# ChenFengYe/motion-latent-diffusion

Hardware: NVIDIA H100
Metric: motions/sec @ 50-step DDIM text-to-motion, batch 256 (higher is better)
Workload: dtype f16x2-split (fp32-equivalent, fp32 accumulate)

## Files before the change

### include/mldb.h

```cpp
#ifndef MLDB_H_
#define MLDB_H_

#include <stdint.h>

#ifdef __cplusplus
extern "C" {
#endif

#define MLDB_OK 0
#define MLDB_ERR_INVALID 1
#define MLDB_ERR_CUDA 2
#define MLDB_ERR_STATE 3
#define MLDB_ERR_UNSUPPORTED 4

#define MLDB_ABI_VERSION 4

typedef struct mldb_handle mldb_handle;

#define MLDB_COND_TEXT 0
#define MLDB_COND_ACTION 1
#define MLDB_ARCH_TRANS_ENC 0
#define MLDB_ARCH_TRANS_DEC 1
#define MLDB_VAE_NONE 0
#define MLDB_VAE_MLD 1
#define MLDB_VAE_ACTOR 2
#define MLDB_SCHED_DDIM 0
#define MLDB_SCHED_DDPM 1
#define MLDB_BETA_SCALED_LINEAR 0
#define MLDB_BETA_LINEAR 1
#define MLDB_BETA_SQUAREDCOS_CAP_V2 2
#define MLDB_DTYPE_F32 0

typedef struct mldb_config {
  int32_t abi_version;
  int32_t cond_kind;
  int32_t arch;
  int32_t latent_dim;
  int32_t n_lat;
  int32_t num_heads;
  int32_t ff_size;
  int32_t num_layers;
  int32_t text_dim;
  int32_t nclasses;
  int32_t nfeats;
  int32_t diffusion_only;
  int32_t flip_sin_to_cos;
  float   freq_shift;
  float   guidance_scale;
  int32_t vae_kind;
  int32_t vae_layers;
  int32_t vae_heads;
  int32_t vae_ff;
  int32_t vae_nfeats;
  int32_t sched_kind;
  int32_t num_train_timesteps;
  double  beta_start;
  double  beta_end;
  int32_t steps_offset;
  int32_t set_alpha_to_one;
  float   eta;
  int32_t njoints;
  int32_t beta_schedule;
  int32_t clip_sample;
} mldb_config;

void mldb_default_config(mldb_config* cfg);

int mldb_create(const mldb_config* cfg, int device, mldb_handle** out);
void mldb_destroy(mldb_handle* h);

int mldb_load_tensor(mldb_handle* h, const char* key, const void* data,
                     const int64_t* shape, int32_t ndim, int32_t dtype);

int mldb_finalize_weights(mldb_handle* h, void* stream);

int mldb_set_mean_std(mldb_handle* h, const float* mean, const float* std, int32_t nfeats);

int mldb_scheduler_table(const mldb_config* cfg, float* alphas_cumprod_out);
int mldb_scheduler_timesteps(const mldb_config* cfg, int32_t n, int64_t* out);

int mldb_scheduler_set_timesteps(mldb_handle* h, int32_t n, int64_t* timesteps_out);

int mldb_scheduler_step(mldb_handle* h, const float* model_output, int64_t timestep,
                        const float* sample, const float* noise, int64_t count,
                        float* prev_sample, void* stream);

int mldb_denoise(mldb_handle* h, const float* sample, int64_t timestep, const void* cond,
                 const int32_t* lengths, int32_t Bx, int32_t S_ctx, int32_t T,
                 float* out, void* stream);

int mldb_diffusion_reverse(mldb_handle* h, const void* cond, const float* init_noise,
                           const float* step_noise, const int32_t* lengths, int32_t B,
                           int32_t S_ctx, int32_t T, float* latents_out, void* stream);

int mldb_vae_decode(mldb_handle* h, const float* z, const int32_t* lengths, int32_t B,
                    int32_t T, float* feats_out, void* stream);

int mldb_vae_encode(mldb_handle* h, const float* feats, const int32_t* lengths, int32_t B,
                    int32_t T, float* mu, float* logvar, void* stream);

int mldb_feats2joints(mldb_handle* h, const float* feats, int32_t B, int32_t T,
                      float* joints_out, void* stream);

int mldb_sample(mldb_handle* h, const void* cond, const float* init_noise,
                const int32_t* lengths, int32_t B, int32_t S_ctx, int32_t T,
                float* latents_out, float* feats_out, float* joints_out, void* stream,
                const float* step_noise);

int mldb_sample_host(mldb_handle* h, const void* cond_host, const float* init_noise_host,
                     const int32_t* lengths_host, int32_t B, int32_t S_ctx, int32_t T,
                     float* joints_host, void* stream, const float* step_noise_host);

int mldb_comm_unique_id(void* out128 );
int mldb_comm_init(mldb_handle* h, const void* unique_id128, int32_t nranks, int32_t rank);
int mldb_comm_attach(mldb_handle* h, void* nccl_comm, int32_t nranks, int32_t rank);
int mldb_comm_info(const mldb_handle* h, int32_t* nranks, int32_t* rank);
int mldb_allgather(mldb_handle* h, const float* local, float* global, int64_t count, void* stream);
int mldb_sample_gather(mldb_handle* h, const void* cond, const float* init_noise, const int32_t* lengths,
                       int32_t B, int32_t S_ctx, int32_t T, float* joints_global, void* stream,
                       const float* step_noise);
int mldb_gather_wait(mldb_handle* h, void* stream);

int mldb_profile_op(mldb_handle* h, const char* op, int32_t B, int32_t S_ctx, int32_t iters,
                    float* avg_ms_out);

int mldb_profile_steps(mldb_handle* h, const void* cond, const float* init_noise, int32_t B, int32_t S_ctx,
                       float* ms_out);

int mldb_debug_timeline(int32_t enable, int64_t* out, int32_t cap, int32_t* count);

int mldb_debug_gemm(mldb_handle* h, const float* A, const float* W, const float* bias, const float* gamma,
                    const float* beta, const float* R, int32_t M, int32_t N, int32_t K, int32_t K1,
                    int32_t act, int32_t use_tc, int32_t split_out, float* out, void* stream);

int mldb_debug_ffn(mldb_handle* h, const float* X, const float* W1, const float* b1, const float* W2,
                   const float* b2, const float* gamma, const float* beta, int32_t M, int32_t d, int32_t ff,
                   int32_t mode, float* out, void* stream);

int mldb_debug_attention(mldb_handle* h, const float* Q, const float* KV, const int32_t* lengths, int32_t kv_prefix,
                         int32_t nseq, int32_t Lq, int32_t Lk, int32_t heads, int32_t hd, int32_t mode, float* out,
                         void* stream);

int mldb_debug_attention_causal(mldb_handle* h, const float* Q, const float* KV, const int32_t* lengths,
                                int32_t kv_prefix, int32_t nseq, int32_t Lq, int32_t Lk, int32_t heads, int32_t hd,
                                int32_t mode, float* out, void* stream);

#define MLDB_TEXT_ABI_VERSION 1
#define MLDB_TEXT_HIDDEN 0
#define MLDB_TEXT_POOLED 1
typedef struct mldb_text_config {
  int32_t abi_version;
  int32_t vocab_size;
  int32_t max_positions;
  int32_t hidden;
  int32_t heads;
  int32_t layers;
  int32_t ff;
  int32_t projection_dim;
  int32_t eos_token_id;
  float   ln_eps;
} mldb_text_config;
void mldb_default_text_config(mldb_text_config* cfg);
int mldb_text_configure(mldb_handle* h, const mldb_text_config* cfg);
int mldb_text_encode(mldb_handle* h, const int64_t* ids, int32_t n, int32_t L, int32_t mode, float* out, void* stream);

#define MLDB_T2M_ABI_VERSION 1
#define MLDB_T2M_TEXT 1
#define MLDB_T2M_MOVEMENT 2
#define MLDB_T2M_MOTION 4
typedef struct mldb_t2m_config {
  int32_t abi_version;
  int32_t parts;
  int32_t dim_word;
  int32_t dim_pos_ohot;
  int32_t dim_text_hidden;
  int32_t dim_coemb_hidden;
  int32_t dim_pose;
  int32_t dim_move_hidden;
  int32_t dim_move_latent;
  int32_t dim_motion_hidden;
  int32_t dim_motion_latent;
} mldb_t2m_config;
void mldb_default_t2m_config(mldb_t2m_config* cfg);
int mldb_t2m_configure(mldb_handle* h, const mldb_t2m_config* cfg);
int mldb_t2m_movement(mldb_handle* h, const float* x, int32_t ld, int32_t B, int32_t T, float* out, void* stream);
int mldb_t2m_motion(mldb_handle* h, const float* x, const int32_t* lengths, int32_t B, int32_t L, float* out,
                    void* stream);
int mldb_t2m_text(mldb_handle* h, const float* word_embs, const float* pos_ohot, const int32_t* lengths, int32_t B,
                  int32_t L, float* out, void* stream);

const char* mldb_last_error(void);
int mldb_abi_version(void);
int64_t mldb_launch_count(const mldb_handle* h);
#define MLDB_KSTAT_GEMM_TC 0
#define MLDB_KSTAT_GEMM_LN_TC 1
#define MLDB_KSTAT_FFN_TC 2
#define MLDB_KSTAT_ATTN_TC 3
#define MLDB_KSTAT_ATTN_MMA 4
#define MLDB_KSTAT_ATTN_SIMT 5
#define MLDB_KSTAT_GEMM_SIMT 6
#define MLDB_KSTAT_LN_SIMT 7
#define MLDB_KSTAT_LN_UNFUSED 8
#define MLDB_KSTAT_MISC 9
#define MLDB_KSTAT_TEXT_LN 10
#define MLDB_KSTAT_GRU_TC 11
#define MLDB_KSTAT_COUNT 12
int mldb_kernel_stats(const mldb_handle* h, int64_t* out, int32_t n);
int mldb_reset_kernel_stats(mldb_handle* h);

int mldb_set_option(mldb_handle* h, const char* name, const char* value);

#ifdef __cplusplus
}
#endif
#endif
```

### mld_b200/_lib.py

```python
from __future__ import annotations

import ctypes as C
import os

_HERE = os.path.dirname(os.path.abspath(__file__))
LIB_PATH = os.path.join(_HERE, "libmldb200.so")

MLDB_ABI_VERSION = 4
COND_TEXT, COND_ACTION = 0, 1
ARCH_TRANS_ENC, ARCH_TRANS_DEC = 0, 1
VAE_NONE, VAE_MLD, VAE_ACTOR = 0, 1, 2
SCHED_DDIM, SCHED_DDPM = 0, 1
BETA_SCHEDULES = {"scaled_linear": 0, "linear": 1, "squaredcos_cap_v2": 2}
DTYPE_F32 = 0
KSTAT_NAMES = ("gemm_tc", "gemm_ln_tc", "ffn_tc", "attn_tc", "attn_mma", "attn_simt", "gemm_simt", "ln_simt",
               "ln_unfused", "misc", "text_ln", "gru_tc")
MLDB_TEXT_ABI_VERSION = 1
TEXT_HIDDEN, TEXT_POOLED = 0, 1
MLDB_T2M_ABI_VERSION = 1
T2M_TEXT, T2M_MOVEMENT, T2M_MOTION = 1, 2, 4


class MldbConfig(C.Structure):
    _fields_ = [
        ("abi_version", C.c_int32),
        ("cond_kind", C.c_int32), ("arch", C.c_int32), ("latent_dim", C.c_int32),
        ("n_lat", C.c_int32), ("num_heads", C.c_int32), ("ff_size", C.c_int32),
        ("num_layers", C.c_int32), ("text_dim", C.c_int32), ("nclasses", C.c_int32),
        ("nfeats", C.c_int32), ("diffusion_only", C.c_int32), ("flip_sin_to_cos", C.c_int32),
        ("freq_shift", C.c_float), ("guidance_scale", C.c_float),
        ("vae_kind", C.c_int32), ("vae_layers", C.c_int32), ("vae_heads", C.c_int32),
        ("vae_ff", C.c_int32), ("vae_nfeats", C.c_int32),
        ("sched_kind", C.c_int32), ("num_train_timesteps", C.c_int32),
        ("beta_start", C.c_double), ("beta_end", C.c_double), ("steps_offset", C.c_int32),
        ("set_alpha_to_one", C.c_int32), ("eta", C.c_float), ("njoints", C.c_int32),
        ("beta_schedule", C.c_int32), ("clip_sample", C.c_int32),
    ]


class MldbTextConfig(C.Structure):
    _fields_ = [
        ("abi_version", C.c_int32), ("vocab_size", C.c_int32), ("max_positions", C.c_int32),
        ("hidden", C.c_int32), ("heads", C.c_int32), ("layers", C.c_int32), ("ff", C.c_int32),
        ("projection_dim", C.c_int32), ("eos_token_id", C.c_int32), ("ln_eps", C.c_float),
    ]


class MldbT2mConfig(C.Structure):
    _fields_ = [
        ("abi_version", C.c_int32), ("parts", C.c_int32), ("dim_word", C.c_int32), ("dim_pos_ohot", C.c_int32),
        ("dim_text_hidden", C.c_int32), ("dim_coemb_hidden", C.c_int32), ("dim_pose", C.c_int32),
        ("dim_move_hidden", C.c_int32), ("dim_move_latent", C.c_int32), ("dim_motion_hidden", C.c_int32),
        ("dim_motion_latent", C.c_int32),
    ]


_P = C.c_void_p
_SIGNATURES = {
    "mldb_default_config": (None, [C.POINTER(MldbConfig)]),
    "mldb_create": (C.c_int, [C.POINTER(MldbConfig), C.c_int, C.POINTER(_P)]),
    "mldb_destroy": (None, [_P]),
    "mldb_load_tensor": (C.c_int, [_P, C.c_char_p, _P, C.POINTER(C.c_int64), C.c_int32, C.c_int32]),
    "mldb_finalize_weights": (C.c_int, [_P, _P]),
    "mldb_set_mean_std": (C.c_int, [_P, _P, _P, C.c_int32]),
    "mldb_scheduler_table": (C.c_int, [C.POINTER(MldbConfig), _P]),
    "mldb_scheduler_timesteps": (C.c_int, [C.POINTER(MldbConfig), C.c_int32, _P]),
    "mldb_scheduler_set_timesteps": (C.c_int, [_P, C.c_int32, _P]),
    "mldb_scheduler_step": (C.c_int, [_P, _P, C.c_int64, _P, _P, C.c_int64, _P, _P]),
    "mldb_denoise": (C.c_int, [_P, _P, C.c_int64, _P, _P, C.c_int32, C.c_int32, C.c_int32, _P, _P]),
    "mldb_diffusion_reverse": (C.c_int, [_P, _P, _P, _P, _P, C.c_int32, C.c_int32, C.c_int32, _P, _P]),
    "mldb_vae_decode": (C.c_int, [_P, _P, _P, C.c_int32, C.c_int32, _P, _P]),
    "mldb_vae_encode": (C.c_int, [_P, _P, _P, C.c_int32, C.c_int32, _P, _P, _P]),
    "mldb_feats2joints": (C.c_int, [_P, _P, C.c_int32, C.c_int32, _P, _P]),
    "mldb_sample": (C.c_int, [_P, _P, _P, _P, C.c_int32, C.c_int32, C.c_int32, _P, _P, _P, _P, _P]),
    "mldb_sample_host": (C.c_int, [_P, _P, _P, _P, C.c_int32, C.c_int32, C.c_int32, _P, _P, _P]),
    "mldb_profile_op": (C.c_int, [_P, C.c_char_p, C.c_int32, C.c_int32, C.c_int32, C.POINTER(C.c_float)]),
    "mldb_profile_steps": (C.c_int, [_P, _P, _P, C.c_int32, C.c_int32, _P]),
    "mldb_debug_timeline": (C.c_int, [C.c_int32, _P, C.c_int32, C.POINTER(C.c_int32)]),
    "mldb_debug_gemm": (C.c_int, [_P, _P, _P, _P, _P, _P, _P, C.c_int32, C.c_int32, C.c_int32, C.c_int32,
                                  C.c_int32, C.c_int32, C.c_int32, _P, _P]),
    "mldb_debug_ffn": (C.c_int, [_P, _P, _P, _P, _P, _P, _P, _P, C.c_int32, C.c_int32, C.c_int32, C.c_int32, _P, _P]),
    "mldb_debug_attention": (C.c_int, [_P, _P, _P, _P, C.c_int32, C.c_int32, C.c_int32, C.c_int32, C.c_int32, C.c_int32,
                                       C.c_int32, _P, _P]),
    "mldb_debug_attention_causal": (C.c_int, [_P, _P, _P, _P, C.c_int32, C.c_int32, C.c_int32, C.c_int32, C.c_int32,
                                              C.c_int32, C.c_int32, _P, _P]),
    "mldb_default_text_config": (None, [C.POINTER(MldbTextConfig)]),
    "mldb_text_configure": (C.c_int, [_P, C.POINTER(MldbTextConfig)]),
    "mldb_text_encode": (C.c_int, [_P, _P, C.c_int32, C.c_int32, C.c_int32, _P, _P]),
    "mldb_default_t2m_config": (None, [C.POINTER(MldbT2mConfig)]),
    "mldb_t2m_configure": (C.c_int, [_P, C.POINTER(MldbT2mConfig)]),
    "mldb_t2m_movement": (C.c_int, [_P, _P, C.c_int32, C.c_int32, C.c_int32, _P, _P]),
    "mldb_t2m_motion": (C.c_int, [_P, _P, _P, C.c_int32, C.c_int32, _P, _P]),
    "mldb_t2m_text": (C.c_int, [_P, _P, _P, _P, C.c_int32, C.c_int32, _P, _P]),
    "mldb_comm_unique_id": (C.c_int, [_P]),
    "mldb_comm_init": (C.c_int, [_P, _P, C.c_int32, C.c_int32]),
    "mldb_comm_attach": (C.c_int, [_P, _P, C.c_int32, C.c_int32]),
    "mldb_comm_info": (C.c_int, [_P, C.POINTER(C.c_int32), C.POINTER(C.c_int32)]),
    "mldb_allgather": (C.c_int, [_P, _P, _P, C.c_int64, _P]),
    "mldb_sample_gather": (C.c_int, [_P, _P, _P, _P, C.c_int32, C.c_int32, C.c_int32, _P, _P, _P]),
    "mldb_gather_wait": (C.c_int, [_P, _P]),
    "mldb_kernel_stats": (C.c_int, [_P, _P, C.c_int32]),
    "mldb_reset_kernel_stats": (C.c_int, [_P]),
    "mldb_last_error": (C.c_char_p, []),
    "mldb_abi_version": (C.c_int, []),
    "mldb_launch_count": (C.c_int64, [_P]),
    "mldb_set_option": (C.c_int, [_P, C.c_char_p, C.c_char_p]),
}

_lib = None


def lib():
    global _lib
    if _lib is None:
        if not os.path.exists(LIB_PATH):
            raise ImportError(
                f"{LIB_PATH} is missing: build it with `python -c 'import __graft_entry__ as g; "
                "g.build()'` (nvcc, sm_90a). mld_b200 has no CPU or PyTorch fallback.")
        l = C.CDLL(LIB_PATH)
        for name, (res, args) in _SIGNATURES.items():
            fn = getattr(l, name)
            fn.restype = res
            fn.argtypes = args
        if l.mldb_abi_version() != MLDB_ABI_VERSION:
            raise ImportError("libmldb200.so ABI version mismatch; rebuild")
        _lib = l
    return _lib


def check(status: int, what: str = "mldb"):
    if status != 0:
        msg = lib().mldb_last_error()
        raise RuntimeError(f"{what} failed (status {status}): {msg.decode() if msg else '?'}")


def default_config() -> MldbConfig:
    cfg = MldbConfig()
    lib().mldb_default_config(C.byref(cfg))
    return cfg


def default_text_config() -> MldbTextConfig:
    cfg = MldbTextConfig()
    lib().mldb_default_text_config(C.byref(cfg))
    return cfg


def default_t2m_config() -> MldbT2mConfig:
    cfg = MldbT2mConfig()
    lib().mldb_default_t2m_config(C.byref(cfg))
    return cfg
```

### mld_b200/csrc/engine.cu

```cuda
#include "engine.h"

#include <math.h>
#include <stdio.h>
#include <string.h>

#include <algorithm>

#include "gemm_tc.h"

static thread_local std::string g_err;
void mldb_set_err(const std::string& s) { g_err = s; }
extern "C" const char* mldb_last_error(void) { return g_err.c_str(); }
extern "C" int mldb_abi_version(void) { return MLDB_ABI_VERSION; }

#define CK(call)                                                                      \
  do {                                                                                \
    cudaError_t e__ = (call);                                                         \
    if (e__ != cudaSuccess) {                                                         \
      char buf__[512];                                                                \
      snprintf(buf__, sizeof buf__, "%s:%d: %s failed: %s", __FILE__, __LINE__, #call, \
               cudaGetErrorString(e__));                                              \
      mldb_set_err(buf__);                                                            \
      return MLDB_ERR_CUDA;                                                           \
    }                                                                                 \
// ... 242 lines not shown
  for (int i = 0; i < nb; ++i) {
    s->skip.emplace_back();
    const std::string lp = p + "linear_blocks." + std::to_string(i) + ".";
    TRY(pack_named(h, lp + "weight", lp + "bias", &s->skip.back()));
  }
  TRY(pack_ln(h, p + "norm.", d, &s->norm));
  return MLDB_OK;
}
static int upload_pe(mldb_handle* h, const std::string& key, float** out, int* rows = nullptr) {
  const RawTensor& t = rt(h, key);
  if (rows) *rows = (int)t.shape[0];
  return upload_f32(h, t.host.data(), t.host.size(), out);
}
static int pack_actor_encoder(mldb_handle* h) {
  const mldb_config& c = h->cfg;
  const int d = c.latent_dim;
  const std::string E = "vae.encoder.";
  StackW* s = &h->venc;
  s->kind = STACK_PLAIN_ENC; s->d = d; s->ff = c.vae_ff; s->heads = c.vae_heads; s->layers = c.vae_layers;
  for (int i = 0; i < c.vae_layers; ++i) {
    const std::string n = E + "seqTransEncoder.layers." + std::to_string(i) + ".";
    s->enc.emplace_back();
    TRY(pack_enc_layer(h, n, d, &s->enc.back()));
    if (i == c.vae_layers - 1) TRY(pack_trimmed_qkv(h, n, d, &s->enc.back()));
  }
  std::vector<float> tok(rt(h, E + "mu_token").host);
  const std::vector<float>& lv = rt(h, E + "logvar_token").host;
  tok.insert(tok.end(), lv.begin(), lv.end());
  TRY(upload_f32(h, tok.data(), tok.size(), &h->global_token));
  TRY(pack_named(h, E + "skel_embedding.weight", E + "skel_embedding.bias", &h->skel_emb, 0, -1, true));
  return upload_pe(h, E + "sequence_pos_encoding.pe", &h->vae_enc_pe, &h->vae_enc_pe_rows);
}

static int check_sched_cfg(const mldb_config& c) {
  if (c.sched_kind != MLDB_SCHED_DDIM && c.sched_kind != MLDB_SCHED_DDPM) FAIL(MLDB_ERR_INVALID, "unknown sched_kind %d", c.sched_kind);
  if (c.beta_schedule != MLDB_BETA_SCALED_LINEAR && c.beta_schedule != MLDB_BETA_LINEAR &&
      c.beta_schedule != MLDB_BETA_SQUAREDCOS_CAP_V2)
    FAIL(MLDB_ERR_INVALID, "unknown beta_schedule %d", c.beta_schedule);
  if (!(c.eta >= 0.0f && c.eta <= 1.0f)) FAIL(MLDB_ERR_INVALID, "eta must lie in [0, 1], got %g", (double)c.eta);
  if (c.num_train_timesteps < 2) FAIL(MLDB_ERR_INVALID, "num_train_timesteps must be >= 2");
  return MLDB_OK;
}

static void build_alphas(const mldb_config& c, std::vector<float>* out) {
  const int T = c.num_train_timesteps;
  out->resize(T);
  const bool scaled = c.beta_schedule == MLDB_BETA_SCALED_LINEAR;
  const float s0 = scaled ? (float)sqrt(c.beta_start) : (float)c.beta_start;
  const float s1 = scaled ? (float)sqrt(c.beta_end) : (float)c.beta_end;
  const float step = (s1 - s0) / (float)(T - 1);
  auto alpha_bar = [](double t) { return pow(cos((t + 0.008) / 1.008 * M_PI / 2), 2.0); };
  double prod = 1.0;
  for (int i = 0; i < T; ++i) {
    float beta;
    if (c.beta_schedule == MLDB_BETA_SQUAREDCOS_CAP_V2) {
      const double t1 = (double)i / T, t2 = (double)(i + 1) / T;
      beta = (float)std::min(1.0 - alpha_bar(t2) / alpha_bar(t1), 0.999);
    } else {
      const float v = (i < T / 2) ? fmaf(step, (float)i, s0) : fmaf(-step, (float)(T - 1 - i), s1);
      beta = scaled ? v * v : v;
    }
    const float alpha = 1.0f - beta;
    prod *= (double)alpha;
    (*out)[i] = (float)prod;
  }
}
extern "C" int mldb_scheduler_table(const mldb_config* cfg, float* alphas_cumprod_out) {
  if (!cfg || !alphas_cumprod_out) FAIL(MLDB_ERR_INVALID, "null argument");
  TRY(check_sched_cfg(*cfg));
  std::vector<float> a;
  build_alphas(*cfg, &a);
  memcpy(alphas_cumprod_out, a.data(), a.size() * sizeof(float));
  return MLDB_OK;
}
extern "C" int mldb_scheduler_timesteps(const mldb_config* cfg, int32_t n, int64_t* out) {
  if (!cfg || !out || n <= 0 || n > cfg->num_train_timesteps) FAIL(MLDB_ERR_INVALID, "bad n");
  const int64_t ratio = cfg->num_train_timesteps / n;
  const int64_t off = cfg->sched_kind == MLDB_SCHED_DDIM ? cfg->steps_offset : 0;
  for (int i = 0; i < n; ++i) out[i] = (int64_t)(n - 1 - i) * ratio + off;
  return MLDB_OK;
}
static StepCoef make_coef(const mldb_handle* h, int64_t t, int n_inference) {
  const mldb_config& c = h->cfg;
  const std::vector<float>& ac = h->alphas_cumprod;
  StepCoef k{};
  const int64_t prev_t = t - c.num_train_timesteps / n_inference;
  const float a_t = ac[t];
  k.c0 = sqrtf(a_t);
  k.c1 = sqrtf(1.0f - a_t);
  k.clip = c.clip_sample ? 1 : 0;
  if (c.sched_kind == MLDB_SCHED_DDIM) {
    const float a_prev = prev_t >= 0 ? ac[prev_t] : (c.set_alpha_to_one ? 1.0f : ac[0]);
    const float variance = ((1.0f - a_prev) / (1.0f - a_t)) * (1.0f - a_t / a_prev);
    const float std_dev = c.eta * sqrtf(variance);
    k.kind = 0;
    k.c2 = sqrtf(a_prev);
    k.c3 = sqrtf(1.0f - a_prev - std_dev * std_dev);
    k.sigma = std_dev;
  } else {
    const float a_prev = prev_t >= 0 ? ac[prev_t] : 1.0f;
    const float bpt = 1.0f - a_t, bpp = 1.0f - a_prev;
    const float cur_alpha = a_t / a_prev, cur_beta = 1.0f - cur_alpha;
    k.kind = 1;
    k.c2 = (sqrtf(a_prev) * cur_beta) / bpt;
    k.c3 = sqrtf(cur_alpha) * bpp / bpt;
    k.sigma = t > 0 ? sqrtf(std::max(bpp / bpt * cur_beta, 1e-20f)) : 0.0f;
  }
  return k;
}

static inline unsigned nblk(int64_t n, int t = 256) { return (unsigned)((n + t - 1) / t); }

static inline ActBuf rows_of(ActBuf b, int64_t row0, int rows) {
  b.hi += row0 * b.cols; b.rows = rows; return b;
}
static inline void kcount(mldb_handle* h, int kind) { h->kstat[kind]++; count_launch(h); }
static void op_gemm(mldb_handle* h, const GemmArgs& g, cudaStream_t st) {
  if (h->use_tc && tc_gemm_supported(h->tc, g)) {
    if (!tc_gemm(h->tc, g, nullptr, st)) h->op_failed = true;
    kcount(h, MLDB_KSTAT_GEMM_TC);
    return;
  }
  simt_gemm(g, st);
  kcount(h, MLDB_KSTAT_GEMM_SIMT);
}
static void op_gemm_ln(mldb_handle* h, GemmArgs g, LnArgs l, float* cf32, cudaStream_t st) {
  if (h->use_tc && tc_gemm_ln_supported(h->tc, g, l)) {
    if (!tc_gemm(h->tc, g, &l, st)) h->op_failed = true;
    kcount(h, MLDB_KSTAT_GEMM_LN_TC);
    return;
  }
  g.out = ActBuf{}; g.out_f32 = cf32; g.ldc = g.w.N;
  op_gemm(h, g, st);
  l.c = cf32; l.ldc = g.w.N;
  simt_ln(l, st);
  kcount(h, h->use_tc ? MLDB_KSTAT_LN_UNFUSED : MLDB_KSTAT_LN_SIMT);
}
static void op_ln(mldb_handle* h, const LnArgs& l, cudaStream_t st) { simt_ln(l, st); kcount(h, MLDB_KSTAT_LN_SIMT); }
static void op_attn(mldb_handle* h, const AttnArgs& a, cudaStream_t st) {
  if (h->use_tc && h->attn_kind == 0 && tc_attention_supported(a)) {
    if (!tc_attention(a, st)) h->op_failed = true;
    kcount(h, MLDB_KSTAT_ATTN_TC);
  } else if (h->use_tc && h->attn_kind <= 1 && mma_attention_supported(a)) {
    mma_attention(a, st);
    kcount(h, MLDB_KSTAT_ATTN_MMA);
  } else {
    if (!simt_attention(a, st)) {
      mldb_set_err("CUDA-core attention: head_dim " + std::to_string(a.hd) + " does not fit shared memory");
      h->op_failed = true;
    }
    kcount(h, MLDB_KSTAT_ATTN_SIMT);
  }
}
static void op_ffn(mldb_handle* h, const GemmArgs& g1, const GemmArgs& g2, const LnArgs& l2, float* cf32, cudaStream_t st) {
  if (h->use_tc && tc_ffn_supported(h->tc, g1, g2, l2)) {
    int k = 0;
    for (int i = 0; i < mldb_handle::MAX_BRANCHES - 1; ++i) if (st == h->br_stream[i]) k = i + 1;
    if (!tc_ffn(h->tc, g1, g2, l2, h->ffn_scratch[k], h->ffn_flags[k], st)) h->op_failed = true;
    kcount(h, MLDB_KSTAT_FFN_TC);
    return;
  }
  op_gemm(h, g1, st);
  op_gemm_ln(h, g2, l2, cf32, st);
}

static int alloc_act(mldb_handle* h, int rows, int cols, ActBuf* out) {
  const int64_t rp = ((int64_t)rows + 127) / 128 * 128;
  __half* p = nullptr;
  TRY(dev_alloc(h, (void**)&p, (size_t)2 * rp * cols * sizeof(__half)));
  CK(cudaMemset(p, 0, (size_t)2 * rp * cols * sizeof(__half)));
  out->hi = p; out->plane_stride = rp * cols; out->rows = rows; out->cols = cols;
  return MLDB_OK;
}
static int alloc_stack_ws(mldb_handle* h, const StackW& sw, int nseq, int L, int Lmem, StackWs* ws,
                          int n_sel = 0) {
  ws->nseq = nseq; ws->L = L; ws->M = nseq * L; ws->d = sw.d; ws->ff = sw.ff; ws->Lmem = Lmem;
  const int M = ws->M, d = sw.d;
  TRY(alloc_act(h, M, d, &ws->x0));
  TRY(alloc_act(h, M, d, &ws->cur[0]));
  TRY(alloc_act(h, M, d, &ws->cur[1]));
  TRY(alloc_act(h, M, d, &ws->x1));
  TRY(alloc_act(h, M, d, &ws->att));
  TRY(alloc_act(h, M, 3 * d, &ws->qkv));
  TRY(alloc_act(h, M, sw.ff, &ws->h));
  const bool enc = sw.kind == STACK_SKIP_ENC || sw.kind == STACK_PLAIN_ENC;
  if (!enc) {
    TRY(alloc_act(h, M, d, &ws->x2));
    TRY(alloc_act(h, M, d, &ws->qc));
    TRY(alloc_act(h, nseq * Lmem, 2 * d, &ws->kvm));
    TRY(alloc_act(h, nseq, d, &ws->vrow));
    TRY(dev_alloc(h, (void**)&ws->cvec, (size_t)nseq * d * sizeof(float)));
  }
  if (sw.kind == STACK_SKIP_ENC || sw.kind == STACK_SKIP_DEC) {
    TRY(alloc_act(h, M, d, &ws->cat));
    const int nb = (sw.layers - 1) / 2;
    ws->ys.resize(nb);
    for (int i = 0; i < nb; ++i) TRY(alloc_act(h, M, d, &ws->ys[i]));
  }
  TRY(dev_alloc(h, (void**)&ws->cf32, (size_t)M * d * sizeof(float)));
  if (enc && n_sel > 0) {
    ws->n_sel = n_sel;
    const int R = nseq * n_sel;
    TRY(alloc_act(h, R, d, &ws->sx));
    TRY(alloc_act(h, R, d, &ws->sq));
    TRY(alloc_act(h, R, d, &ws->satt));
    TRY(alloc_act(h, R, d, &ws->sx1));
    TRY(alloc_act(h, R, sw.ff, &ws->sh));
    TRY(alloc_act(h, R, d, &ws->sout));
  }
  return MLDB_OK;
}

struct SeqInfo {
  const int32_t* lengths = nullptr;
  int kv_prefix = 0;
  int len_mod = 0;
};

static StackWs ws_slice(const StackWs& ws, int s0, int n) {
  StackWs w = ws;
  w.nseq = n; w.M = n * ws.L;
  auto tok = [&](ActBuf b) { return b.hi ? rows_of(b, (int64_t)s0 * ws.L, n * ws.L) : b; };
  auto sel = [&](ActBuf b) { return b.hi ? rows_of(b, (int64_t)s0 * ws.n_sel, n * ws.n_sel) : b; };
  w.x0 = tok(ws.x0); w.cur[0] = tok(ws.cur[0]); w.cur[1] = tok(ws.cur[1]); w.x1 = tok(ws.x1); w.x2 = tok(ws.x2);
  w.att = tok(ws.att); w.qkv = tok(ws.qkv); w.qc = tok(ws.qc); w.h = tok(ws.h); w.cat = tok(ws.cat);
  for (auto& y : w.ys) y = tok(y);
  if (ws.kvm.hi) w.kvm = rows_of(ws.kvm, (int64_t)s0 * ws.Lmem, n * ws.Lmem);
  if (ws.vrow.hi) w.vrow = rows_of(ws.vrow, s0, n);
  if (ws.cvec) w.cvec = ws.cvec + (size_t)s0 * ws.d;
  if (ws.cf32) w.cf32 = ws.cf32 + (size_t)s0 * ws.L * ws.d;
  w.sx = sel(ws.sx); w.sq = sel(ws.sq); w.satt = sel(ws.satt); w.sx1 = sel(ws.sx1); w.sh = sel(ws.sh); w.sout = sel(ws.sout);
  return w;
}
static void out_proj_ln(mldb_handle* h, const LinW& w, const LnW& n, ActBuf att, ActBuf res, ActBuf xout, int M, int d,
                        float* cf32, cudaStream_t st) {
  GemmArgs g; g.a1 = att; g.K1 = d; g.M = M; g.w = w;
  LnArgs l; l.res = res; l.gamma = n.g; l.beta = n.b; l.M = M; l.d = d; l.out = xout;
  op_gemm_ln(h, g, l, cf32, st);
}
static void self_attn_block(mldb_handle* h, const LinW& in_proj, const LinW& out_proj, const LnW& n,
                            ActBuf xin, ActBuf xout, StackWs& ws, const SeqInfo& si, int heads,
                            cudaStream_t st) {
  const int d = ws.d;
  GemmArgs g; g.a1 = xin; g.K1 = d; g.M = ws.M; g.w = in_proj; g.out = ws.qkv;
  op_gemm(h, g, st);
  AttnArgs a; a.q = ws.qkv; a.q_col0 = 0; a.Lq = ws.L; a.kv = ws.qkv; a.k_col0 = d; a.v_col0 = 2 * d;
  a.Lk = ws.L; a.nseq = ws.nseq; a.heads = heads; a.hd = d / heads;
  a.lengths = si.lengths; a.kv_prefix = si.kv_prefix; a.len_mod = si.len_mod; a.seq0 = 0; a.out = ws.att;
  op_attn(h, a, st);
  out_proj_ln(h, out_proj, n, ws.att, xin, xout, ws.M, d, ws.cf32, st);
}
static void ffn_block(mldb_handle* h, const LinW& l1, const LinW& l2, const LnW& n, ActBuf xin,
                      ActBuf xout, StackWs& ws, int act, cudaStream_t st) {
  GemmArgs g; g.a1 = xin; g.K1 = ws.d; g.M = ws.M; g.w = l1; g.act = act; g.out = ws.h;
  GemmArgs g2; g2.a1 = ws.h; g2.K1 = ws.ff; g2.M = ws.M; g2.w = l2;
  LnArgs l; l.res = xin; l.gamma = n.g; l.beta = n.b; l.M = ws.M; l.d = ws.d; l.out = xout;
  op_ffn(h, g, g2, l, ws.cf32, st);
}
static void enc_layer(mldb_handle* h, const StackW& sw, const EncW& w, ActBuf xin, ActBuf xout,
                      StackWs& ws, const SeqInfo& si, cudaStream_t st) {
  self_attn_block(h, w.in_proj, w.out_proj, w.n1, xin, ws.x1, ws, si, sw.heads, st);
  ffn_block(h, w.l1, w.l2, w.n2, ws.x1, xout, ws, ACT_GELU, st);
}
static void dec_layer(mldb_handle* h, const StackW& sw, const DecW& w, ActBuf xin, ActBuf xout,
                      ActBuf mem, StackWs& ws, const SeqInfo& si, cudaStream_t st) {
  const int d = ws.d;
  self_attn_block(h, w.sa_in, w.sa_out, w.n1, xin, ws.x1, ws, si, sw.heads, st);
  if (ws.Lmem == 1) {
    GemmArgs gv; gv.a1 = mem; gv.K1 = d; gv.M = ws.nseq; gv.w = w.ca_v; gv.out = ws.vrow;
    op_gemm(h, gv, st);
    GemmArgs gc; gc.a1 = ws.vrow; gc.K1 = d; gc.M = ws.nseq; gc.w = w.ca_out; gc.out_f32 = ws.cvec; gc.ldc = d;
    op_gemm(h, gc, st);
    LnArgs lc; lc.res = ws.x1; lc.rowvec = ws.cvec; lc.rv_group = ws.L; lc.gamma = w.n2.g; lc.beta = w.n2.b;
    lc.M = ws.M; lc.d = d; lc.out = ws.x2;
    op_ln(h, lc, st);
    ffn_block(h, w.l1, w.l2, w.n3, ws.x2, xout, ws, ACT_GELU, st);
    return;
  }
  GemmArgs gq; gq.a1 = ws.x1; gq.K1 = d; gq.M = ws.M; gq.w = w.ca_q; gq.out = ws.qc;
  op_gemm(h, gq, st);
  GemmArgs gk; gk.a1 = mem; gk.K1 = d; gk.M = ws.nseq * ws.Lmem; gk.w = w.ca_kv; gk.out = ws.kvm;
  op_gemm(h, gk, st);
  AttnArgs a; a.q = ws.qc; a.q_col0 = 0; a.Lq = ws.L; a.kv = ws.kvm; a.k_col0 = 0; a.v_col0 = d;
  a.Lk = ws.Lmem; a.nseq = ws.nseq; a.heads = sw.heads; a.hd = d / sw.heads; a.out = ws.att;
  op_attn(h, a, st);
  out_proj_ln(h, w.ca_out, w.n2, ws.att, ws.x1, ws.x2, ws.M, d, ws.cf32, st);
  ffn_block(h, w.l1, w.l2, w.n3, ws.x2, xout, ws, ACT_GELU, st);
}
static void any_layer(mldb_handle* h, const StackW& sw, int li, ActBuf xin, ActBuf xout, ActBuf mem,
                      StackWs& ws, const SeqInfo& si, cudaStream_t st) {
  if (sw.kind == STACK_SKIP_ENC) enc_layer(h, sw, sw.enc[li], xin, xout, ws, si, st);
  else dec_layer(h, sw, sw.dec[li], xin, xout, mem, ws, si, st);
}
__global__ void k_gather_rows(ActBuf src, ActBuf dst, int L, int n_sel, int nrows_out, int d) {
  pdl_trigger();
  pdl_wait();
  const int64_t idx = (int64_t)blockIdx.x * blockDim.x + threadIdx.x;
  if (idx >= (int64_t)nrows_out * (d / 8)) return;
  const int c = (int)(idx % (d / 8));
  const int r = (int)(idx / (d / 8));
  const int64_t srow = (int64_t)(r / n_sel) * L + r % n_sel;
  const uint4* sh = reinterpret_cast<const uint4*>(src.hi + srow * src.cols) + c;
  const uint4* sl = reinterpret_cast<const uint4*>(src.lo() + srow * src.cols) + c;
  reinterpret_cast<uint4*>(dst.hi + (int64_t)r * dst.cols)[c] = *sh;
  reinterpret_cast<uint4*>(dst.lo() + (int64_t)r * dst.cols)[c] = *sl;
}

static ActBuf enc_layer_selected(mldb_handle* h, const StackW& sw, const EncW& w, ActBuf xin, StackWs& ws,
                                 const SeqInfo& si, cudaStream_t st) {
  const int d = ws.d, R = ws.nseq * ws.n_sel;
  GemmArgs gk; gk.a1 = xin; gk.K1 = d; gk.M = ws.M; gk.w = w.kv_only; gk.out = ws.qkv;
  op_gemm(h, gk, st);
  launch_pdl(k_gather_rows, dim3(nblk((int64_t)R * (d / 8))), dim3(256), 0, st, xin, ws.sx, ws.L, ws.n_sel, R, d);
  kcount(h, MLDB_KSTAT_MISC);
  GemmArgs gq; gq.a1 = ws.sx; gq.K1 = d; gq.M = R; gq.w = w.q_only; gq.out = ws.sq;
  op_gemm(h, gq, st);
  AttnArgs a; a.q = ws.sq; a.q_col0 = 0; a.Lq = ws.n_sel; a.kv = ws.qkv; a.k_col0 = 0; a.v_col0 = d;
  a.Lk = ws.L; a.nseq = ws.nseq; a.heads = sw.heads; a.hd = d / sw.heads; a.lengths = si.lengths;
  a.kv_prefix = si.kv_prefix; a.len_mod = si.len_mod; a.out = ws.satt;
  op_attn(h, a, st);
  out_proj_ln(h, w.out_proj, w.n1, ws.satt, ws.sx, ws.sx1, R, d, ws.cf32, st);
  GemmArgs g1; g1.a1 = ws.sx1; g1.K1 = d; g1.M = R; g1.w = w.l1; g1.act = ACT_GELU; g1.out = ws.sh;
  GemmArgs g2; g2.a1 = ws.sh; g2.K1 = ws.ff; g2.M = R; g2.w = w.l2;
  LnArgs l2; l2.res = ws.sx1; l2.gamma = w.n2.g; l2.beta = w.n2.b; l2.M = R; l2.d = d; l2.out = ws.sout;
  op_ffn(h, g1, g2, l2, ws.cf32, st);
  return ws.sout;
}

static ActBuf run_stack(mldb_handle* h, const StackW& sw, ActBuf x0, ActBuf mem, StackWs& ws,
                        const SeqInfo& si, cudaStream_t st) {
  if (sw.kind == STACK_PLAIN_ENC) {
    ActBuf x = x0;
    for (int i = 0; i + 1 < sw.layers; ++i) {
      enc_layer(h, sw, sw.enc[i], x, ws.cur[i & 1], ws, si, st);
      x = ws.cur[i & 1];
    }
    return enc_layer_selected(h, sw, sw.enc.back(), x, ws, si, st);
  }
  if (sw.kind == STACK_PLAIN_DEC) {
    ActBuf x = x0;
    for (int i = 0; i < sw.layers; ++i) {
      any_layer(h, sw, i, x, ws.cur[i & 1], mem, ws, si, st);
      x = ws.cur[i & 1];
    }
    return x;
  }
  const int nb = (sw.layers - 1) / 2;
  ActBuf x = x0;
  for (int i = 0; i < nb; ++i) {
    any_layer(h, sw, i, x, ws.ys[i], mem, ws, si, st);
    x = ws.ys[i];
  }
  any_layer(h, sw, nb, x, ws.cur[0], mem, ws, si, st);
  x = ws.cur[0];
  for (int i = 0; i < nb; ++i) {
    GemmArgs g; g.a1 = x; g.K1 = sw.d; g.a2 = ws.ys[nb - 1 - i]; g.K2 = sw.d; g.M = ws.M;
    g.w = sw.skip[i]; g.out = ws.cat;
    op_gemm(h, g, st);
    if (i == nb - 1 && sw.kind == STACK_SKIP_ENC && ws.n_sel > 0)
      return enc_layer_selected(h, sw, sw.enc[nb + 1 + i], ws.cat, ws, si, st);
    any_layer(h, sw, nb + 1 + i, ws.cat, ws.cur[(i + 1) & 1], mem, ws, si, st);
    x = ws.cur[(i + 1) & 1];
  }
  return x;
}

extern "C" int mldb_create(const mldb_config* cfg, int device, mldb_handle** out) {
  if (!cfg || !out) FAIL(MLDB_ERR_INVALID, "null argument");
  if (cfg->abi_version != MLDB_ABI_VERSION) FAIL(MLDB_ERR_INVALID, "abi_version mismatch");
  if (cfg->latent_dim % cfg->num_heads || cfg->latent_dim % 32) FAIL(MLDB_ERR_INVALID, "latent_dim must be a multiple of 32 and of num_heads");
  if (cfg->latent_dim > 1024) FAIL(MLDB_ERR_UNSUPPORTED, "latent_dim > 1024");
  for (int heads : {cfg->num_heads, cfg->vae_heads})
    if (heads > 0 && !simt_attention_supported(cfg->latent_dim / heads))
      FAIL(MLDB_ERR_UNSUPPORTED, "head_dim %d is too wide for the attention kernels", cfg->latent_dim / heads);
  if (cfg->arch == MLDB_ARCH_TRANS_ENC && cfg->num_layers > 0 && cfg->num_layers % 2 != 1) FAIL(MLDB_ERR_INVALID, "skip encoder needs an odd layer count");
  if (cfg->arch == MLDB_ARCH_TRANS_ENC && cfg->diffusion_only) FAIL(MLDB_ERR_UNSUPPORTED, "diffusion_only requires arch trans_dec");
  if (cfg->vae_kind == MLDB_VAE_MLD && cfg->vae_layers % 2 != 1) FAIL(MLDB_ERR_INVALID, "MldVae needs an odd layer count");
  TRY(check_sched_cfg(*cfg));
  int ndev = 0;
  CK(cudaGetDeviceCount(&ndev));
  if (device < 0 || device >= ndev) FAIL(MLDB_ERR_INVALID, "no such CUDA device %d (no CPU fallback exists)", device);
  cudaDeviceProp prop;
  CK(cudaGetDeviceProperties(&prop, device));
  if (prop.major != 9) FAIL(MLDB_ERR_UNSUPPORTED, "device %d is sm_%d%d; libmldb200 is sm_90a only", device, prop.major, prop.minor);
  DeviceGuard guard(device);
  mldb_handle* h = new mldb_handle();
  h->cfg = *cfg; h->device = device; h->sm_count = prop.multiProcessorCount;
  build_spec(h);
  build_alphas(h->cfg, &h->alphas_cumprod);
  cudaError_t e = cudaStreamCreateWithFlags(&h->cap_stream, cudaStreamNonBlocking);
  if (e != cudaSuccess) { delete h; FAIL(MLDB_ERR_CUDA, "cudaStreamCreate: %s", cudaGetErrorString(e)); }
  if (!simt_init() || !mma_attention_init()) { delete h; return MLDB_ERR_CUDA; }
  h->tc = tc_create(device);
  if (!h->tc) { delete h; return MLDB_ERR_CUDA; }
  if (!tc_attention_init(device) || !gru_tc_init()) { tc_destroy(h->tc); delete h; return MLDB_ERR_CUDA; }
  const char* env = getenv("MLDB_GEMM");
  if (env && !strcmp(env, "simt")) h->use_tc = false;
  env = getenv("MLDB_GRAPH");
  if (env && !strcmp(env, "0")) h->use_graph = false;
  env = getenv("MLDB_ATTN");
  if (env) h->attn_kind = !strcmp(env, "mma") ? 1 : (!strcmp(env, "simt") ? 2 : 0);
  env = getenv("MLDB_BRANCHES");
  if (env) h->branches = std::min(std::max(atoi(env), 1), (int)mldb_handle::MAX_BRANCHES);
  e = cudaEventCreateWithFlags(&h->ev_fork, cudaEventDisableTiming);
  for (int i = 0; i < mldb_handle::MAX_BRANCHES - 1 && e == cudaSuccess; ++i) {
    e = cudaStreamCreateWithFlags(&h->br_stream[i], cudaStreamNonBlocking);
    if (e == cudaSuccess) e = cudaEventCreateWithFlags(&h->ev_join[i], cudaEventDisableTiming);
  }
  if (e != cudaSuccess) { mldb_destroy(h); FAIL(MLDB_ERR_CUDA, "branch streams: %s", cudaGetErrorString(e)); }
  for (int i = 0; i < mldb_handle::MAX_BRANCHES && e == cudaSuccess; ++i) {
    e = cudaMalloc((void**)&h->ffn_scratch[i], TC_FFN_SCRATCH_BYTES);
    if (e == cudaSuccess) e = cudaMalloc((void**)&h->ffn_flags[i], TC_FFN_FLAG_BYTES);
    if (e == cudaSuccess) e = cudaMemset(h->ffn_flags[i], 0, TC_FFN_FLAG_BYTES);
  }
  if (e != cudaSuccess) { mldb_destroy(h); FAIL(MLDB_ERR_CUDA, "ffn scratch: %s", cudaGetErrorString(e)); }
  env = getenv("MLDB_FFN_SPLIT");
  if (env) tc_set_ffn_split(h->tc, atoi(env) != 0);
  env = getenv("MLDB_FFN_FUSED");
  if (env) tc_set_ffn_fused(h->tc, atoi(env) != 0);
  *out = h;
  return MLDB_OK;
}

extern "C" void mldb_destroy(mldb_handle* h) {
  if (!h) return;
  DeviceGuard guard(h->device);
  cudaDeviceSynchronize();
  for (auto& kv : h->plans) {
    if (kv.second->exec) cudaGraphExecDestroy(kv.second->exec);
    delete kv.second;
  }
  for (void* p : h->allocs) cudaFree(p);
  for (void* p : h->text.ws_allocs) cudaFree(p);
  for (void* p : h->t2m.buf) cudaFree(p);
  if (h->cap_stream) cudaStreamDestroy(h->cap_stream);
  for (int i = 0; i < mldb_handle::MAX_BRANCHES - 1; ++i) {
    if (h->br_stream[i]) cudaStreamDestroy(h->br_stream[i]);
    if (h->ev_join[i]) cudaEventDestroy(h->ev_join[i]);
  }
  if (h->ev_fork) cudaEventDestroy(h->ev_fork);
  for (int i = 0; i < mldb_handle::MAX_BRANCHES; ++i) { cudaFree(h->ffn_scratch[i]); cudaFree(h->ffn_flags[i]); }
  mldb_comm_release(h);
  tc_destroy(h->tc);
  delete h;
}

extern "C" int mldb_set_option(mldb_handle* h, const char* name, const char* value) {
  if (!h || !name || !value) FAIL(MLDB_ERR_INVALID, "null argument");
  if (!strcmp(name, "gemm")) {
    if (!strcmp(value, "tc")) h->use_tc = true;
    else if (!strcmp(value, "simt")) h->use_tc = false;
    else FAIL(MLDB_ERR_INVALID, "gemm must be tc|simt");
  } else if (!strcmp(name, "ffn_fused")) {
    tc_set_ffn_fused(h->tc, atoi(value) != 0);
  } else if (!strcmp(name, "ffn_split")) {
    tc_set_ffn_split(h->tc, atoi(value) != 0);
  } else if (!strcmp(name, "attn")) {
    if (!strcmp(value, "tc")) h->attn_kind = 0;
    else if (!strcmp(value, "mma")) h->attn_kind = 1;
    else if (!strcmp(value, "simt")) h->attn_kind = 2;
    else FAIL(MLDB_ERR_INVALID, "attn must be tc|mma|simt");
  } else if (!strcmp(name, "branches")) {
    h->branches = std::min(std::max(atoi(value), 1), (int)mldb_handle::MAX_BRANCHES);
  } else if (!strcmp(name, "graph")) {
    h->use_graph = strcmp(value, "0") != 0;
  } else if (!strcmp(name, "t2m_chunk")) {
    h->t2m.chunk = std::max(atoi(value), 0);
  } else {
    FAIL(MLDB_ERR_INVALID, "unknown option %s", name);
  }
  for (auto& kv : h->plans) {
    if (kv.second->exec) { cudaGraphExecDestroy(kv.second->exec); kv.second->exec = nullptr; }
  }
  return MLDB_OK;
}

extern "C" int64_t mldb_launch_count(const mldb_handle* h) { return h ? h->launches : 0; }

// ... 911 lines not shown
    return check_ops(h);
  }
  LnArgs l; l.res = x; l.gamma = h->venc.norm.g; l.beta = h->venc.norm.b; l.M = B * G; l.d = d;
  if (p->ws.n_sel == 0) { l.sel_group = G; l.in_group = L; }
  l.out_f32 = p->stage_f32; l.ld_out = d;
  op_ln(h, l, st);
  k_rows_out_permuted<<<nblk((int64_t)B * G * d), 256, 0, st>>>(p->stage_f32, mu, logvar, B, c.n_lat, d);
  kcount(h, MLDB_KSTAT_MISC);
  CK(cudaGetLastError());
  return MLDB_OK;
}

static int run_f2j(mldb_handle* h, const float* feats, int B, int T, float* joints, cudaStream_t st) {
  const mldb_config& c = h->cfg;
  const int F = c.vae_kind != MLDB_VAE_NONE ? c.vae_nfeats : c.nfeats;
  if (!h->mean || h->nstat != F) FAIL(MLDB_ERR_STATE, "call mldb_set_mean_std with %d features first", F);
  if (F < 4 + (c.njoints - 1) * 3) FAIL(MLDB_ERR_UNSUPPORTED, "feats2joints needs the HumanML3D/KIT layout");
  k_feats2joints<<<B, 256, 0, st>>>(feats, h->mean, h->stdv, T, F, c.njoints, joints);
  kcount(h, MLDB_KSTAT_MISC);
  CK(cudaGetLastError());
  return MLDB_OK;
}
extern "C" int mldb_feats2joints(mldb_handle* h, const float* feats, int32_t B, int32_t T,
                                 float* joints_out, void* stream) {
  TRY(check_ready(h, false));
  DeviceGuard guard(h->device);
  if (!feats || !joints_out || B <= 0 || T <= 0) FAIL(MLDB_ERR_INVALID, "bad argument");
  return run_f2j(h, feats, B, T, joints_out, (cudaStream_t)stream);
}

extern "C" int mldb_sample(mldb_handle* h, const void* cond, const float* init_noise,
                           const int32_t* lengths, int32_t B, int32_t S_ctx, int32_t T,
                           float* latents_out, float* feats_out, float* joints_out, void* stream,
                           const float* step_noise) {
  TRY(check_ready(h, true));
  DeviceGuard guard(h->device);
  if (!cond || !init_noise || !lengths || B <= 0 || T <= 0) FAIL(MLDB_ERR_INVALID, "bad argument");
  cudaStream_t st = (cudaStream_t)stream;
  Plan *rp = nullptr, *dp = nullptr;
  TRY(dec_plan(h, B, T, &dp));
  const mldb_config& c = h->cfg;
  float* z = latents_out;
  if (!z) {
    if (!dp->stage_f32) TRY(dev_alloc(h, (void**)&dp->stage_f32, (size_t)B * c.n_lat * c.latent_dim * sizeof(float)));
    z = dp->stage_f32;
  }
  if (c.arch != MLDB_ARCH_TRANS_ENC) FAIL(MLDB_ERR_UNSUPPORTED, "mldb_sample is built for the latent (VAE) models");
  TRY(run_reverse(h, cond, init_noise, step_noise, lengths, B, S_ctx, T, z, st, &rp));
  TRY(run_decode(h, z, lengths, B, T, feats_out, st, &dp));
  if (joints_out) TRY(run_f2j(h, feats_out ? feats_out : dp->feats, B, T, joints_out, st));
  return MLDB_OK;
}

extern "C" int mldb_sample_gather(mldb_handle* h, const void* cond, const float* init_noise,
                                  const int32_t* lengths, int32_t B, int32_t S_ctx, int32_t T,
                                  float* joints_global, void* stream, const float* step_noise) {
  TRY(check_ready(h, true));
  DeviceGuard guard(h->device);
  if (!joints_global) FAIL(MLDB_ERR_INVALID, "bad argument");
  const int64_t count = (int64_t)B * T * h->cfg.njoints * 3;
  cudaStream_t st = (cudaStream_t)stream;
  if (!h->nccl_comm) {
    return mldb_sample(h, cond, init_noise, lengths, B, S_ctx, T, nullptr, nullptr, joints_global, stream, step_noise);
  }
  TRY(mldb_gather_begin(h, st));
  TRY(mldb_sample(h, cond, init_noise, lengths, B, S_ctx, T, nullptr, nullptr, joints_global + h->comm_rank * count, stream,
                  step_noise));
  return mldb_gather_async(h, joints_global, count, st);
}

extern "C" int mldb_sample_host(mldb_handle* h, const void* cond_host, const float* init_noise_host,
                                const int32_t* lengths_host, int32_t B, int32_t S_ctx, int32_t T,
                                float* joints_host, void* stream, const float* step_noise_host) {
  TRY(check_ready(h, true));
  DeviceGuard guard(h->device);
  if (!cond_host || !init_noise_host || !lengths_host || !joints_host || B <= 0 || T <= 0) FAIL(MLDB_ERR_INVALID, "bad argument");
  cudaStream_t st = (cudaStream_t)stream;
  const mldb_config& c = h->cfg;
  Plan* dp = nullptr;
  TRY(dec_plan(h, B, T, &dp));
  const bool cfg_on = c.guidance_scale > 1.0f;
  const int Bx = cfg_on ? 2 * B : B;
  const size_t cond_bytes = c.cond_kind == MLDB_COND_TEXT ? (size_t)Bx * S_ctx * c.text_dim * sizeof(float)
                                                         : (size_t)Bx * sizeof(int64_t);
  const size_t noise_bytes = (size_t)B * c.n_lat * c.latent_dim * sizeof(float);
  if (dp->cond_cap < cond_bytes) {
    TRY(dev_alloc(h, (void**)&dp->cond_f, cond_bytes));
    dp->cond_cap = cond_bytes;
  }
  if (!dp->noise_in) {
    TRY(dev_alloc(h, (void**)&dp->noise_in, noise_bytes));
    TRY(dev_alloc(h, (void**)&dp->cond_i, (size_t)B * sizeof(int32_t)));
  }
  const int world = h->nccl_comm ? h->comm_world : 1;
  const size_t joints_elems = (size_t)B * T * c.njoints * 3;
  if (world > 1 && !dp->joints_all) TRY(dev_alloc(h, (void**)&dp->joints_all, world * joints_elems * sizeof(float)));
  CK(cudaMemcpyAsync(dp->cond_f, cond_host, cond_bytes, cudaMemcpyHostToDevice, st));
  CK(cudaMemcpyAsync(dp->noise_in, init_noise_host, noise_bytes, cudaMemcpyHostToDevice, st));
  CK(cudaMemcpyAsync(dp->cond_i, lengths_host, (size_t)B * sizeof(int32_t), cudaMemcpyHostToDevice, st));
  const float* step_noise = nullptr;
  if (step_noise_host) {
    const size_t n = h->timesteps.size() * (size_t)B * c.n_lat * c.latent_dim;
    if (dp->noise_cap < n) {
      TRY(dev_alloc(h, (void**)&dp->step_noise, n * sizeof(float)));
      dp->noise_cap = n;
    }
    CK(cudaMemcpyAsync(dp->step_noise, step_noise_host, n * sizeof(float), cudaMemcpyHostToDevice, st));
    step_noise = dp->step_noise;
  }
  if (world > 1) {
    TRY(mldb_sample_gather(h, dp->cond_f, dp->noise_in, (const int32_t*)dp->cond_i, B, S_ctx, T, dp->joints_all, stream,
                           step_noise));
    TRY(mldb_gather_wait(h, stream));
    CK(cudaMemcpyAsync(joints_host, dp->joints_all, world * joints_elems * sizeof(float), cudaMemcpyDeviceToHost, st));
    return MLDB_OK;
  }
  TRY(mldb_sample(h, dp->cond_f, dp->noise_in, (const int32_t*)dp->cond_i, B, S_ctx, T, nullptr, nullptr, dp->joints, stream,
                  step_noise));
  CK(cudaMemcpyAsync(joints_host, dp->joints, joints_elems * sizeof(float), cudaMemcpyDeviceToHost, st));
  return MLDB_OK;
}

extern "C" int mldb_profile_op(mldb_handle* h, const char* op, int32_t B, int32_t S_ctx, int32_t iters,
                               float* avg_ms_out) {
  TRY(check_ready(h, false));
  DeviceGuard guard(h->device);
  if (!op || !avg_ms_out || iters <= 0) FAIL(MLDB_ERR_INVALID, "bad argument");
  const mldb_config& c = h->cfg;
  if (c.num_layers == 0 || c.arch != MLDB_ARCH_TRANS_ENC) FAIL(MLDB_ERR_UNSUPPORTED, "needs the trans_enc denoiser");
  const bool cfg_on = c.guidance_scale > 1.0f;
  Plan* p = nullptr;
  TRY(enc_plan(h, 0, B, cfg_on ? 2 * B : B, S_ctx, &p));
  cudaStream_t st = h->cap_stream;
  StackWs& ws = p->ws;
  const EncW& w = h->den.enc[0];
  const int d = ws.d;
  SeqInfo si;
  auto run = [&]() -> int {
    if (!strcmp(op, "qkv")) {
      GemmArgs g; g.a1 = ws.x0; g.K1 = d; g.M = ws.M; g.w = w.in_proj; g.out = ws.qkv; op_gemm(h, g, st);
    } else if (!strcmp(op, "attn")) {
      AttnArgs a; a.q = ws.qkv; a.Lq = ws.L; a.kv = ws.qkv; a.k_col0 = d; a.v_col0 = 2 * d; a.Lk = ws.L;
      a.nseq = ws.nseq; a.heads = c.num_heads; a.hd = d / c.num_heads; a.out = ws.att; op_attn(h, a, st);
    } else if (!strcmp(op, "outproj_ln")) {
      out_proj_ln(h, w.out_proj, w.n1, ws.att, ws.x0, ws.x1, ws.M, d, ws.cf32, st);
    } else if (!strcmp(op, "ffn1")) {
      GemmArgs g; g.a1 = ws.x1; g.K1 = d; g.M = ws.M; g.w = w.l1; g.act = ACT_GELU; g.out = ws.h; op_gemm(h, g, st);
    } else if (!strcmp(op, "ffn2_ln")) {
      GemmArgs g; g.a1 = ws.h; g.K1 = ws.ff; g.M = ws.M; g.w = w.l2;
      LnArgs l; l.res = ws.x1; l.gamma = w.n2.g; l.beta = w.n2.b; l.M = ws.M; l.d = d; l.out = ws.cur[0];
      op_gemm_ln(h, g, l, ws.cf32, st);
    } else if (!strcmp(op, "ffn")) {
      ffn_block(h, w.l1, w.l2, w.n2, ws.x1, ws.cur[0], ws, ACT_GELU, st);
    } else if (!strcmp(op, "layer")) {
      enc_layer(h, h->den, w, ws.x0, ws.cur[0], ws, si, st);
    } else {
      FAIL(MLDB_ERR_INVALID, "unknown op %s", op);
    }
    return MLDB_OK;
  };
  cudaEvent_t e0, e1;
  CK(cudaEventCreate(&e0)); CK(cudaEventCreate(&e1));
  for (int i = 0; i < 3; ++i) TRY(run());
  CK(cudaEventRecord(e0, st));
  for (int i = 0; i < iters; ++i) TRY(run());
  CK(cudaEventRecord(e1, st));
  CK(cudaStreamSynchronize(st));
  float ms = 0.0f;
  CK(cudaEventElapsedTime(&ms, e0, e1));
  cudaEventDestroy(e0); cudaEventDestroy(e1);
  CK(cudaGetLastError());
  *avg_ms_out = ms / (float)iters;
  return MLDB_OK;
}

extern "C" int mldb_profile_steps(mldb_handle* h, const void* cond, const float* init_noise, int32_t B, int32_t S_ctx,
                                  float* ms_out) {
  TRY(check_ready(h, true));
  DeviceGuard guard(h->device);
  if (!cond || !init_noise || !ms_out || B <= 0) FAIL(MLDB_ERR_INVALID, "bad argument");
  const mldb_config& c = h->cfg;
  if (c.num_layers == 0 || c.arch != MLDB_ARCH_TRANS_ENC) FAIL(MLDB_ERR_UNSUPPORTED, "needs the trans_enc denoiser");
  if (c.sched_kind != MLDB_SCHED_DDIM) FAIL(MLDB_ERR_UNSUPPORTED, "step profiling is built for the DDIM loop");
  const bool cfg_on = c.guidance_scale > 1.0f;
  Plan* p = nullptr;
  TRY(enc_plan(h, 0, B, cfg_on ? 2 * B : B, S_ctx, &p));
  cudaStream_t st = h->cap_stream;
  const int d = c.latent_dim, nsteps = (int)h->timesteps.size();
  const int64_t per = (int64_t)c.n_lat * d;
  TRY(place_condition(h, p, cond, st));
  CK(cudaMemcpyAsync(p->latents, init_noise, (size_t)B * per * sizeof(float), cudaMemcpyDeviceToDevice, st));
  std::vector<cudaEvent_t> ev(nsteps + 1);
  for (auto& e : ev) CK(cudaEventCreate(&e));
  CK(cudaEventRecord(ev[0], st));
  for (int i = 0; i < nsteps; ++i) {
    denoiser_pass(h, p, p->latents, B, h->d_tt + (size_t)i * d, p->eps, st);
    launch_pdl(k_cfg_sched, dim3(nblk(B * per)), dim3(256), 0, st, (const float*)p->eps, p->latents, (const float*)nullptr,
               (int64_t)(B * per), cfg_on ? 1 : 0, c.guidance_scale, (const StepCoef*)h->d_coefs, i, (const int*)nullptr);
    kcount(h, MLDB_KSTAT_MISC);
    CK(cudaEventRecord(ev[i + 1], st));
  }
  CK(cudaStreamSynchronize(st));
  for (int i = 0; i < nsteps; ++i) CK(cudaEventElapsedTime(&ms_out[i], ev[i], ev[i + 1]));
  for (auto& e : ev) cudaEventDestroy(e);
  CK(cudaGetLastError());
  return check_ops(h);
}


static void op_text_ln(mldb_handle* h, const TextLnArgs& a, cudaStream_t st) { text_ln(a, st); kcount(h, MLDB_KSTAT_TEXT_LN); }

static int text_workspace(mldb_handle* h, int rows, int seqs) {
  TextW& tw = h->text;
  if (rows <= tw.rows && seqs <= tw.seqs) return MLDB_OK;
  rows = std::max(rows, tw.rows); seqs = std::max(seqs, tw.seqs);
  CK(cudaDeviceSynchronize());
  for (void* p : tw.ws_allocs) cudaFree(p);
  tw.ws_allocs.clear();
  tw.rows = tw.seqs = 0;
  auto alloc = [&](size_t bytes, void** p) -> int {
    CK(cudaMalloc(p, bytes ? bytes : 16));
    tw.ws_allocs.push_back(*p);
    CK(cudaMemset(*p, 0, bytes));
    return MLDB_OK;
  };
  auto act = [&](int r, int cols, ActBuf* out) -> int {
    const int64_t rp = ((int64_t)r + 127) / 128 * 128;
    TRY(alloc((size_t)2 * rp * cols * sizeof(__half), (void**)&out->hi));
    out->plane_stride = rp * cols; out->rows = r; out->cols = cols;
    return MLDB_OK;
  };
  const mldb_text_config& c = tw.cfg;
  TRY(alloc((size_t)rows * c.hidden * sizeof(float), (void**)&tw.x));
  TRY(act(rows, c.hidden, &tw.a));
  TRY(act(rows, 3 * c.hidden, &tw.qkv));
  TRY(act(rows, c.hidden, &tw.att));
  TRY(act(rows, c.ff, &tw.h));
  TRY(act(seqs, c.hidden, &tw.pooled));
  tw.rows = rows; tw.seqs = seqs;
  return MLDB_OK;
}

extern "C" int mldb_text_encode(mldb_handle* h, const int64_t* ids, int32_t n, int32_t L, int32_t mode, float* out,
                                void* stream) {
  if (!h || !ids || !out) FAIL(MLDB_ERR_INVALID, "null argument");
  TextW& tw = h->text;
  if (!tw.on) FAIL(MLDB_ERR_STATE, "the text tower is not configured (mldb_text_configure)");
  if (!h->finalized) FAIL(MLDB_ERR_STATE, "finalize weights first");
  const mldb_text_config& c = tw.cfg;
  if (n < 1 || L < 1 || L > c.max_positions) FAIL(MLDB_ERR_INVALID, "ids must be [n >= 1, 1 <= L <= %d]", c.max_positions);
  if ((int64_t)n * L > (1 << 30)) FAIL(MLDB_ERR_INVALID, "too many tokens");
  if (mode != MLDB_TEXT_HIDDEN && mode != MLDB_TEXT_POOLED) FAIL(MLDB_ERR_INVALID, "mode must be MLDB_TEXT_HIDDEN or MLDB_TEXT_POOLED");
  DeviceGuard guard(h->device);
  cudaStream_t st = (cudaStream_t)stream;
  const int M = n * L, d = c.hidden;
  TRY(text_workspace(h, M, n));
  auto rows = [&](ActBuf b, int r) { b.rows = r; return b; };
  const ActBuf a = rows(tw.a, M), qkv = rows(tw.qkv, M), att = rows(tw.att, M), hid = rows(tw.h, M);
  auto ln = [&](int m, const LnW& w) {
    TextLnArgs l; l.mode = m; l.x = tw.x; l.ids = ids; l.L = L; l.tok = tw.tok; l.pos = tw.pos; l.vocab = c.vocab_size;
    l.eos_id = c.eos_token_id; l.gamma = w.g; l.beta = w.b; l.eps = c.ln_eps; l.M = M; l.d = d; l.out = a;
    return l;
  };
  op_text_ln(h, ln(TEXT_LN_EMBED, tw.layers[0].ln1), st);
  for (int i = 0; i < c.layers; ++i) {
    const TextLayerW& w = tw.layers[i];
    GemmArgs g; g.a1 = a; g.K1 = d; g.M = M; g.w = w.qkv; g.out = qkv; g.wide_n = 1;
    op_gemm(h, g, st);
    AttnArgs at; at.q = qkv; at.q_col0 = 0; at.Lq = L; at.kv = qkv; at.k_col0 = d; at.v_col0 = 2 * d; at.Lk = L;
    at.nseq = n; at.heads = c.heads; at.hd = d / c.heads; at.causal = 1; at.out = att;
    op_attn(h, at, st);
    GemmArgs go; go.a1 = att; go.K1 = d; go.M = M; go.w = w.out; go.out_f32 = tw.x; go.ldc = d; go.res_f32 = tw.x;
    op_gemm(h, go, st);
    op_text_ln(h, ln(TEXT_LN_ROWS, w.ln2), st);
    GemmArgs g1; g1.a1 = a; g1.K1 = d; g1.M = M; g1.w = w.fc1; g1.act = ACT_QUICKGELU; g1.out = hid; g1.wide_n = 1;
    op_gemm(h, g1, st);
    GemmArgs g2; g2.a1 = hid; g2.K1 = c.ff; g2.M = M; g2.w = w.fc2; g2.out_f32 = tw.x; g2.ldc = d; g2.res_f32 = tw.x;
    op_gemm(h, g2, st);
    if (i + 1 < c.layers) op_text_ln(h, ln(TEXT_LN_ROWS, tw.layers[i + 1].ln1), st);
  }
  if (mode == MLDB_TEXT_HIDDEN) {
    TextLnArgs l = ln(TEXT_LN_ROWS, tw.final_ln);
    l.out = ActBuf{}; l.out_f32 = out;
    op_text_ln(h, l, st);
  } else {
    TextLnArgs l = ln(TEXT_LN_EOS, tw.final_ln);
    l.M = n; l.out = rows(tw.pooled, n);
    op_text_ln(h, l, st);
    GemmArgs gp; gp.a1 = l.out; gp.K1 = d; gp.M = n; gp.w = tw.proj; gp.out_f32 = out; gp.ldc = c.projection_dim;
    gp.wide_n = 1;
    op_gemm(h, gp, st);
  }
  CK(cudaGetLastError());
  return check_ops(h);
}

static int t2m_slot(mldb_handle* h, int i, size_t bytes, void** out) {
  T2mW& t = h->t2m;
  if (bytes > t.cap[i]) {
    CK(cudaDeviceSynchronize());
    cudaFree(t.buf[i]);
    t.buf[i] = nullptr; t.cap[i] = 0;
    CK(cudaMalloc(&t.buf[i], bytes));
    CK(cudaMemset(t.buf[i], 0, bytes));
    t.cap[i] = bytes;
  }
// ... 124 lines not shown
}

extern "C" int mldb_t2m_motion(mldb_handle* h, const float* x, const int32_t* lengths, int32_t B, int32_t L, float* out,
                               void* stream) {
  if (!h || !x || !lengths || !out) FAIL(MLDB_ERR_INVALID, "null argument");
  TRY(t2m_ready(h, MLDB_T2M_MOTION, "motion"));
  const mldb_t2m_config& c = h->t2m.cfg;
  if (B < 1 || L < 1 || (int64_t)B * L > (1 << 26)) FAIL(MLDB_ERR_INVALID, "motion encoder input must be [B >= 1, L >= 1, %d], got B=%d L=%d", c.dim_move_latent, B, L);
  DeviceGuard guard(h->device);
  cudaStream_t st = (cudaStream_t)stream;
  const int In = c.dim_move_latent, H = c.dim_motion_hidden;
  const int Bc = t2m_chunk(h, B, gru_bytes_per_seq(L, In + H, H));
  for (int b0 = 0; b0 < B; b0 += Bc) {
    const int n = std::min(Bc, B - b0);
    ActBuf xs, e;
    TRY(t2m_act(h, 0, n * L, In, &xs));
    TRY(t2m_act(h, 2, n * L, H, &e));
    k_f32_to_split_pad<<<nblk((int64_t)n * L * In), 256, 0, st>>>(xs, x + (int64_t)b0 * L * In, In, n * L, In, 1);
    kcount(h, MLDB_KSTAT_MISC);
    GemmArgs g; g.a1 = xs; g.K1 = In; g.M = n * L; g.w = h->t2m.motion_in; g.out = e; g.wide_n = 1;
    op_gemm(h, g, st);
    TRY(gru_forward(h, h->t2m.motion_gru, e, lengths + b0, n, L, out + (int64_t)b0 * c.dim_motion_latent,
                    c.dim_motion_latent, st));
  }
  CK(cudaGetLastError());
  return check_ops(h);
}

extern "C" int mldb_t2m_text(mldb_handle* h, const float* word_embs, const float* pos_ohot, const int32_t* lengths,
                             int32_t B, int32_t L, float* out, void* stream) {
  if (!h || !word_embs || !pos_ohot || !lengths || !out) FAIL(MLDB_ERR_INVALID, "null argument");
  TRY(t2m_ready(h, MLDB_T2M_TEXT, "text"));
  const mldb_t2m_config& c = h->t2m.cfg;
  if (B < 1 || L < 1 || (int64_t)B * L > (1 << 26)) FAIL(MLDB_ERR_INVALID, "text encoder input must be [B >= 1, L >= 1, *], got B=%d L=%d", B, L);
  DeviceGuard guard(h->device);
  cudaStream_t st = (cudaStream_t)stream;
  const int W = c.dim_word, P = c.dim_pos_ohot, H = c.dim_text_hidden;
  const int Bc = t2m_chunk(h, B, gru_bytes_per_seq(L, pad64(P) + 2 * W + pad64(W) + H, H));
  for (int b0 = 0; b0 < B; b0 += Bc) {
    const int n = std::min(Bc, B - b0), M = n * L;
    ActBuf ps, xs, e;
    float* xw = nullptr;
    TRY(t2m_act(h, 0, M, pad64(P), &ps));
    TRY(t2m_slot(h, 7, (size_t)M * W * sizeof(float), (void**)&xw));
    TRY(t2m_act(h, 8, M, pad64(W), &xs));
    TRY(t2m_act(h, 2, M, H, &e));
    k_f32_to_split_pad<<<nblk((int64_t)M * ps.cols), 256, 0, st>>>(ps, pos_ohot + (int64_t)b0 * L * P, P, M, P, 1);
    kcount(h, MLDB_KSTAT_MISC);
    GemmArgs gp; gp.a1 = ps; gp.K1 = ps.cols; gp.M = M; gp.w = h->t2m.pos_emb; gp.out_f32 = xw; gp.ldc = W;
    gp.res_f32 = word_embs + (int64_t)b0 * L * W; gp.wide_n = 1;
    op_gemm(h, gp, st);
    k_f32_to_split_pad<<<nblk((int64_t)M * xs.cols), 256, 0, st>>>(xs, xw, W, M, W, 1);
    kcount(h, MLDB_KSTAT_MISC);
    GemmArgs g; g.a1 = xs; g.K1 = xs.cols; g.M = M; g.w = h->t2m.text_in; g.out = e; g.wide_n = 1;
    op_gemm(h, g, st);
    TRY(gru_forward(h, h->t2m.text_gru, e, lengths + b0, n, L, out + (int64_t)b0 * c.dim_coemb_hidden,
                    c.dim_coemb_hidden, st));
  }
  CK(cudaGetLastError());
  return check_ops(h);
}

extern "C" int mldb_debug_gemm(mldb_handle* h, const float* A, const float* W, const float* bias,
                               const float* gamma, const float* beta, const float* R, int32_t M, int32_t N,
                               int32_t K, int32_t K1, int32_t act, int32_t use_tc, int32_t split_out, float* out,
                               void* stream) {
  if (!h || !A || !W || !out || M <= 0 || N <= 0 || K <= 0) FAIL(MLDB_ERR_INVALID, "bad argument");
  DeviceGuard guard(h->device);
  cudaStream_t st = (cudaStream_t)stream;
  const size_t n_alloc0 = h->allocs.size();
  LinW w;
  TRY(pack_linear(h, W, N, K, bias, &w));
  if (K1 <= 0 || K1 >= K) K1 = K;
  ActBuf a1, a2{}, res{}, o{};
  TRY(alloc_act(h, M, K1, &a1));
  k_rows_to_split<<<nblk((int64_t)M * K1), 256, 0, st>>>(a1, A, K, M, K1, 1 << 30, 0, 0, 0, nullptr);
  if (K1 < K) {
    TRY(alloc_act(h, M, K - K1, &a2));
    k_rows_to_split<<<nblk((int64_t)M * (K - K1)), 256, 0, st>>>(a2, A + K1, K, M, K - K1, 1 << 30, 0, 0, 0, nullptr);
  }
  float *g = nullptr, *b = nullptr, *cf32 = nullptr;
  const bool saved = h->use_tc;
  h->use_tc = use_tc != 0;
  GemmArgs ga; ga.a1 = a1; ga.K1 = K1; ga.a2 = a2; ga.K2 = K - K1; ga.M = M; ga.w = w; ga.act = act; ga.wide_n = 1;
  int rc = MLDB_OK;
  if (gamma) {
    TRY(upload_f32(h, gamma, N, &g));
    TRY(upload_f32(h, beta, N, &b));
    TRY(dev_alloc(h, (void**)&cf32, (size_t)M * N * sizeof(float)));
    TRY(alloc_act(h, M, N, &o));
    if (R) {
      TRY(alloc_act(h, M, N, &res));
      k_rows_to_split<<<nblk((int64_t)M * N), 256, 0, st>>>(res, R, N, M, N, 1 << 30, 0, 0, 0, nullptr);
    }
    LnArgs l; l.res = res; l.gamma = g; l.beta = b; l.M = M; l.d = N; l.out = o;
    op_gemm_ln(h, ga, l, cf32, st);
    k_split_to_f32<<<nblk((int64_t)M * N), 256, 0, st>>>(o, out, (int64_t)M * N);
  } else if (R) {
    ga.res_f32 = R; ga.out_f32 = out; ga.ldc = N;
    op_gemm(h, ga, st);
  } else if (split_out && N % 8 == 0) {
    TRY(alloc_act(h, M, N, &o));
    ga.out = o;
    op_gemm(h, ga, st);
    k_split_to_f32<<<nblk((int64_t)M * N), 256, 0, st>>>(o, out, (int64_t)M * N);
  } else {
    ga.out_f32 = out; ga.ldc = N;
    op_gemm(h, ga, st);
  }
  h->use_tc = saved;
  cudaError_t e = cudaStreamSynchronize(st);
  if (e == cudaSuccess) e = cudaGetLastError();
  while (h->allocs.size() > n_alloc0) { cudaFree(h->allocs.back()); h->allocs.pop_back(); }
  if (e != cudaSuccess) FAIL(MLDB_ERR_CUDA, "debug gemm: %s", cudaGetErrorString(e));
  return rc;
}

extern "C" int mldb_debug_ffn(mldb_handle* h, const float* X, const float* W1, const float* b1, const float* W2,
                              const float* b2, const float* gamma, const float* beta, int32_t M, int32_t d,
                              int32_t ff, int32_t mode, float* out, void* stream) {
  if (!h || !X || !W1 || !W2 || !gamma || !beta || !out || M <= 0 || d <= 0 || ff <= 0)
    FAIL(MLDB_ERR_INVALID, "bad argument");
  DeviceGuard guard(h->device);
  cudaStream_t st = (cudaStream_t)stream;
  const size_t n_alloc0 = h->allocs.size();
  LinW l1, l2;
  LnW n;
  TRY(pack_linear(h, W1, ff, d, b1, &l1));
  TRY(pack_linear(h, W2, d, ff, b2, &l2));
  TRY(upload_f32(h, gamma, d, &n.g));
  TRY(upload_f32(h, beta, d, &n.b));
  StackWs ws;
  ws.M = M; ws.d = d; ws.ff = ff;
  ActBuf x, o;
  TRY(alloc_act(h, M, d, &x));
  TRY(alloc_act(h, M, d, &o));
  TRY(alloc_act(h, M, ff, &ws.h));
  TRY(dev_alloc(h, (void**)&ws.cf32, (size_t)M * d * sizeof(float)));
  k_rows_to_split<<<nblk((int64_t)M * d), 256, 0, st>>>(x, X, d, M, d, 1 << 30, 0, 0, 0, nullptr);
  const bool saved = h->use_tc;
  h->use_tc = mode != 0;
  const int saved_fused = tc_set_ffn_fused(h->tc, mode == 2);
  ffn_block(h, l1, l2, n, x, o, ws, ACT_GELU, st);
  h->use_tc = saved;
  tc_set_ffn_fused(h->tc, saved_fused);
  k_split_to_f32<<<nblk((int64_t)M * d), 256, 0, st>>>(o, out, (int64_t)M * d);
  cudaError_t e = cudaStreamSynchronize(st);
  if (e == cudaSuccess) e = cudaGetLastError();
  while (h->allocs.size() > n_alloc0) { cudaFree(h->allocs.back()); h->allocs.pop_back(); }
  if (e != cudaSuccess) FAIL(MLDB_ERR_CUDA, "debug ffn: %s", cudaGetErrorString(e));
  return MLDB_OK;
}

static int debug_attention(mldb_handle* h, const float* Q, const float* KV, const int32_t* lengths, int32_t kv_prefix,
                           int32_t nseq, int32_t Lq, int32_t Lk, int32_t heads, int32_t hd, int32_t mode, int causal,
                           float* out, void* stream) {
  if (!h || !Q || !out || nseq <= 0 || Lq <= 0 || Lk <= 0 || heads <= 0 || hd <= 0) FAIL(MLDB_ERR_INVALID, "bad argument");
  if (!KV && Lq != Lk) FAIL(MLDB_ERR_INVALID, "a packed QKV input is self-attention: Lq must equal Lk");
  if (causal && KV) FAIL(MLDB_ERR_INVALID, "causal attention is self-attention: pass a packed QKV input (KV == NULL)");
  DeviceGuard guard(h->device);
  cudaStream_t st = (cudaStream_t)stream;
  const size_t n_alloc0 = h->allocs.size();
  const int d = heads * hd, Mq = nseq * Lq, Mk = nseq * Lk;
  ActBuf qb, kvb, o;
  TRY(alloc_act(h, Mq, KV ? d : 3 * d, &qb));
  TRY(alloc_act(h, Mq, d, &o));
  rows_to_split(h, qb, Q, qb.cols, Mq, qb.cols, 1 << 30, 0, 0, 0, nullptr, 0, st);
  AttnArgs a; a.q = qb; a.q_col0 = 0; a.Lq = Lq; a.Lk = Lk;
  if (KV) {
    TRY(alloc_act(h, Mk, 2 * d, &kvb));
    rows_to_split(h, kvb, KV, 2 * d, Mk, 2 * d, 1 << 30, 0, 0, 0, nullptr, 0, st);
    a.kv = kvb; a.k_col0 = 0; a.v_col0 = d;
  } else {
    a.kv = qb; a.k_col0 = d; a.v_col0 = 2 * d;
  }
  a.nseq = nseq; a.heads = heads; a.hd = hd; a.lengths = lengths; a.kv_prefix = kv_prefix; a.out = o;
  a.causal = causal;
  int rc = MLDB_OK;
  if (mode == 0 && simt_attention_supported(hd)) { if (!simt_attention(a, st)) rc = MLDB_ERR_UNSUPPORTED; }
  else if (mode == 1 && mma_attention_supported(a)) mma_attention(a, st);
  else if (mode == 2 && tc_attention_supported(a)) { if (!tc_attention(a, st)) rc = MLDB_ERR_CUDA; }
  else rc = MLDB_ERR_UNSUPPORTED;
  if (rc == MLDB_OK) k_split_to_f32<<<nblk((int64_t)Mq * d), 256, 0, st>>>(o, out, (int64_t)Mq * d);
  cudaError_t e = cudaStreamSynchronize(st);
  if (e == cudaSuccess) e = cudaGetLastError();
  while (h->allocs.size() > n_alloc0) { cudaFree(h->allocs.back()); h->allocs.pop_back(); }
  if (e != cudaSuccess) FAIL(MLDB_ERR_CUDA, "debug attention: %s", cudaGetErrorString(e));
  if (rc == MLDB_ERR_UNSUPPORTED) FAIL(rc, "attention mode %d does not support this shape", mode);
  return rc;
}
extern "C" int mldb_debug_attention(mldb_handle* h, const float* Q, const float* KV, const int32_t* lengths,
                                    int32_t kv_prefix, int32_t nseq, int32_t Lq, int32_t Lk, int32_t heads, int32_t hd,
                                    int32_t mode, float* out, void* stream) {
  return debug_attention(h, Q, KV, lengths, kv_prefix, nseq, Lq, Lk, heads, hd, mode, 0, out, stream);
}
extern "C" int mldb_debug_attention_causal(mldb_handle* h, const float* Q, const float* KV, const int32_t* lengths,
                                           int32_t kv_prefix, int32_t nseq, int32_t Lq, int32_t Lk, int32_t heads,
                                           int32_t hd, int32_t mode, float* out, void* stream) {
  return debug_attention(h, Q, KV, lengths, kv_prefix, nseq, Lq, Lk, heads, hd, mode, 1, out, stream);
}

static long long* g_timeline = nullptr;
namespace tc { long long* mldb_timeline_buffer() { return g_timeline; } }
extern "C" int mldb_debug_timeline(int32_t enable, int64_t* out, int32_t cap, int32_t* count) {
  constexpr int WARPS = 32, CAPW = 512;
  constexpr size_t BYTES = (size_t)WARPS * CAPW * 2 * sizeof(long long);
  if (enable) {
    if (!g_timeline && cudaMalloc((void**)&g_timeline, BYTES) != cudaSuccess) FAIL(MLDB_ERR_CUDA, "timeline buffer");
    CK(cudaMemset(g_timeline, 0, BYTES));
    return MLDB_OK;
  }
  if (!g_timeline) FAIL(MLDB_ERR_STATE, "no timeline is being recorded");
  if (!out || !count || cap <= 0) FAIL(MLDB_ERR_INVALID, "bad argument");
  CK(cudaDeviceSynchronize());
  std::vector<long long> hbuf((size_t)WARPS * CAPW * 2);
  CK(cudaMemcpy(hbuf.data(), g_timeline, BYTES, cudaMemcpyDeviceToHost));
  int n = 0;
  for (int w = 0; w < WARPS; ++w)
    for (int i = 0; i < CAPW && n < cap; ++i) {
      const long long tag = hbuf[((size_t)w * CAPW + i) * 2], clk = hbuf[((size_t)w * CAPW + i) * 2 + 1];
      if (clk == 0) break;
      out[2 * n] = tag | ((long long)w << 16);
      out[2 * n + 1] = clk;
      ++n;
    }
  *count = n;
  cudaFree(g_timeline);
  g_timeline = nullptr;
  return MLDB_OK;
}

extern "C" int mldb_kernel_stats(const mldb_handle* h, int64_t* out, int32_t n) {
  if (!h || !out || n <= 0) FAIL(MLDB_ERR_INVALID, "bad argument");
  for (int i = 0; i < n; ++i) out[i] = i < MLDB_KSTAT_COUNT ? h->kstat[i] : 0;
  return MLDB_OK;
}
extern "C" int mldb_reset_kernel_stats(mldb_handle* h) {
  if (!h) FAIL(MLDB_ERR_INVALID, "null handle");
  for (int i = 0; i < MLDB_KSTAT_COUNT; ++i) h->kstat[i] = 0;
  return MLDB_OK;
}
```

### mld_b200/csrc/gemm_tc.cu

```cuda
#include "gemm_tc.h"

#include <algorithm>

#include "tc_common.cuh"

namespace {
using namespace tc;

constexpr int BM = 128, BK = 64;
constexpr int NUM_THREADS = 384;
constexpr int MMA_THREADS = 256;
constexpr int CONSUMER_WARPS = 8;
constexpr int MAX_N = 1024;
constexpr int MAX_N_WIDE = 4096;

struct TcParams {
  int M, N, kblocks, kb1;
  int m_tiles, n_tiles;
  float inv_scale;
  const float* bias;
  const float* addtab;
  int act;
  __half* out_hi; __half* out_lo; int ld_out, out_col0;
  float* out_f32; int ldc;
  const float* res_f32;
  int in_group, out_group, out_off;
  const int32_t* zero_lengths;
  const __half* res_hi; const __half* res_lo; int ld_res;
  const float* gamma; const float* beta;
  long long* tl;
};

enum { EPI_FAST = 0, EPI_LN = 1, EPI_GENERIC = 2, EPI_RES = 3, EPI_F32 = 4 };

template <int BN>
struct TileCfg {
  static constexpr int A_BYTES = BM * BK * 2;
  static constexpr int W_BYTES = BN * BK * 2;
  static constexpr int STAGE_BYTES = 2 * A_BYTES + 2 * W_BYTES;
  static constexpr int STAGES = BN == 256 ? 2 : 3;
  static constexpr int SMEM_BYTES = STAGES * STAGE_BYTES + 256 + 1024;
  static_assert(SMEM_BYTES <= 232448, "shared memory budget");
};

__device__ __forceinline__ void store_split2(__half* hi, __half* lo, int64_t o, float x0, float x1) {
  uint32_t h, l;
  split2(x0, x1, h, l);
  *reinterpret_cast<uint32_t*>(hi + o) = h;
  *reinterpret_cast<uint32_t*>(lo + o) = l;
}

template <int ACT, int N>
__device__ __forceinline__ void fast_group(const float (&d)[N], int j, float sc, float2 b, float (&x)[4]) {
  x[0] = fmaf(d[4 * j], sc, b.x); x[1] = fmaf(d[4 * j + 1], sc, b.y);
  x[2] = fmaf(d[4 * j + 2], sc, b.x); x[3] = fmaf(d[4 * j + 3], sc, b.y);
#pragma unroll
  for (int e = 0; e < 4; ++e) {
    if (ACT == ACT_GELU) x[e] = gelu_fast(x[e]);
    if (ACT == ACT_QUICKGELU) x[e] = quick_gelu_f(x[e]);
    if (ACT == ACT_LEAKY) x[e] = apply_act(x[e], ACT_LEAKY);
  }
}

__device__ __forceinline__ void quad_transpose(uint32_t (&v)[4], int l) {
  const bool b2 = l & 2, b1 = l & 1;
  uint32_t r0 = __shfl_xor_sync(0xffffffffu, b2 ? v[0] : v[2], 2), r1 = __shfl_xor_sync(0xffffffffu, b2 ? v[1] : v[3], 2);
  if (b2) { v[0] = r0; v[1] = r1; } else { v[2] = r0; v[3] = r1; }
  r0 = __shfl_xor_sync(0xffffffffu, b1 ? v[0] : v[1], 1); r1 = __shfl_xor_sync(0xffffffffu, b1 ? v[2] : v[3], 1);
  if (b1) { v[0] = r0; v[2] = r1; } else { v[1] = r0; v[3] = r1; }
}

template <class Load>
__device__ __forceinline__ void ring_produce(int& q_next, int total, int need, const uint64_t* bar_empty, int stages,
                                             Load&& load) {
  while (q_next < total) {
    const uint32_t bar = smem_u32(&bar_empty[q_next % stages]), par = (((uint32_t)(q_next / stages)) & 1u) ^ 1u;
    if (q_next <= need) mbar_wait(bar, par);
    else if (!__shfl_sync(0xffffffffu, (int)mbar_test(bar, par), 0)) break;
    load(q_next++);
  }
}

__device__ __forceinline__ void ln_epilogue(float (&d)[128], float sc, const float* bias, const __half* res_hi,
                                            const __half* res_lo, int ld_res, const float* gamma, const float* beta,
                                            __half* out_hi, __half* out_lo, int ld_out, int r_lo, int M, int cp) {
  const bool ok0 = r_lo < M, ok1 = r_lo + 8 < M;
  float s0 = 0.0f, s1 = 0.0f;
#pragma unroll
  for (int j = 0; j < 32; ++j) {
    const int n = 8 * j + cp;
    const float2 b = bias ? __ldg(reinterpret_cast<const float2*>(bias + n)) : make_float2(0.0f, 0.0f);
    float x0 = fmaf(d[4 * j], sc, b.x), x1 = fmaf(d[4 * j + 1], sc, b.y);
    float x2 = fmaf(d[4 * j + 2], sc, b.x), x3 = fmaf(d[4 * j + 3], sc, b.y);
    if (res_hi) {
      if (ok0) {
        const int64_t o = (int64_t)r_lo * ld_res + n;
        const float2 h = __half22float2(*reinterpret_cast<const __half2*>(res_hi + o));
        const float2 l = __half22float2(*reinterpret_cast<const __half2*>(res_lo + o));
        x0 = (x0 + h.x) + l.x; x1 = (x1 + h.y) + l.y;
      }
      if (ok1) {
        const int64_t o = (int64_t)(r_lo + 8) * ld_res + n;
        const float2 h = __half22float2(*reinterpret_cast<const __half2*>(res_hi + o));
        const float2 l = __half22float2(*reinterpret_cast<const __half2*>(res_lo + o));
        x2 = (x2 + h.x) + l.x; x3 = (x3 + h.y) + l.y;
      }
    }
    d[4 * j] = x0; d[4 * j + 1] = x1; d[4 * j + 2] = x2; d[4 * j + 3] = x3;
    s0 += x0 + x1; s1 += x2 + x3;
  }
  const float mean0 = quad_sum(s0) * (1.0f / 256), mean1 = quad_sum(s1) * (1.0f / 256);
  float q0 = 0.0f, q1 = 0.0f;
#pragma unroll
  for (int j = 0; j < 32; ++j) {
    const float a0 = d[4 * j] - mean0, a1 = d[4 * j + 1] - mean0, a2 = d[4 * j + 2] - mean1, a3 = d[4 * j + 3] - mean1;
    d[4 * j] = a0; d[4 * j + 1] = a1; d[4 * j + 2] = a2; d[4 * j + 3] = a3;
    q0 = fmaf(a0, a0, fmaf(a1, a1, q0));
    q1 = fmaf(a2, a2, fmaf(a3, a3, q1));
  }
  const float rstd0 = rsqrtf(quad_sum(q0) * (1.0f / 256) + 1e-5f), rstd1 = rsqrtf(quad_sum(q1) * (1.0f / 256) + 1e-5f);
#pragma unroll
  for (int j = 0; j < 32; ++j) {
    const int n = 8 * j + cp;
    const float2 g = __ldg(reinterpret_cast<const float2*>(gamma + n)), be = __ldg(reinterpret_cast<const float2*>(beta + n));
    if (ok0)
      store_split2(out_hi, out_lo, (int64_t)r_lo * ld_out + n, fmaf(d[4 * j] * rstd0, g.x, be.x),
                   fmaf(d[4 * j + 1] * rstd0, g.y, be.y));
    if (ok1)
      store_split2(out_hi, out_lo, (int64_t)(r_lo + 8) * ld_out + n, fmaf(d[4 * j + 2] * rstd1, g.x, be.x),
                   fmaf(d[4 * j + 3] * rstd1, g.y, be.y));
  }
}

template <int BN, int EPI, int ACT = ACT_NONE>
__global__ void __launch_bounds__(NUM_THREADS, 1)
k_gemm_tc(const __grid_constant__ CUtensorMap tmA1h, const __grid_constant__ CUtensorMap tmA1l,
          const __grid_constant__ CUtensorMap tmA2h, const __grid_constant__ CUtensorMap tmA2l,
          const __grid_constant__ CUtensorMap tmWh, const __grid_constant__ CUtensorMap tmWl, const TcParams p) {
  static_assert(EPI != EPI_LN || BN == 256, "the LayerNorm epilogue covers a full 256-wide row");
  using Cfg = TileCfg<BN>;
  constexpr int STAGES = Cfg::STAGES;
  extern __shared__ uint8_t smem_raw[];
  uint8_t* smem = smem_raw + smem_pad1024(smem_raw);
  uint64_t* bar_full = reinterpret_cast<uint64_t*>(smem + STAGES * Cfg::STAGE_BYTES);
  uint64_t* bar_empty = bar_full + STAGES;

  const int warp = __shfl_sync(0xffffffffu, (int)(threadIdx.x >> 5), 0), lane = threadIdx.x & 31;
  int tl_n = 0;
  tl_event(p.tl, tl_n, 40);
  const int ntiles = p.m_tiles * p.n_tiles;
  const int nlocal = (ntiles - (int)blockIdx.x + (int)gridDim.x - 1) / (int)gridDim.x;
  auto decode = [&](int j, int& m0, int& n0) {
    const int t = (int)blockIdx.x + j * (int)gridDim.x;
    m0 = (t / p.n_tiles) * BM;
    n0 = (t % p.n_tiles) * BN;
  };

  if (threadIdx.x == 0) {
    for (int s = 0; s < STAGES; ++s) {
      mbar_init(smem_u32(&bar_full[s]), 1);
      mbar_init(smem_u32(&bar_empty[s]), CONSUMER_WARPS);
    }
    asm volatile("fence.mbarrier_init.release.cluster;" ::: "memory");
    tma_prefetch_desc(&tmA1h); tma_prefetch_desc(&tmA1l); tma_prefetch_desc(&tmWh); tma_prefetch_desc(&tmWl);
  }
  pdl_trigger();
  __syncthreads();
  pdl_wait();
  tl_event(p.tl, tl_n, 41);

  if (warp < 4) {
    reg_dec<40>();
    if (warp != 0) return;
    int kbg = 0;
    for (int j = 0; j < nlocal; ++j) {
      int m0, n0;
      decode(j, m0, n0);
      tl_event(p.tl, tl_n, 1, j);
      for (int kb = 0; kb < p.kblocks; ++kb, ++kbg) {
        const int s = kbg % STAGES;
        mbar_wait(smem_u32(&bar_empty[s]), (((uint32_t)(kbg / STAGES)) & 1u) ^ 1u);
        if (elect_one()) {
          if (kb == 0 && j + 1 < nlocal) {
            int m1, n1;
            decode(j + 1, m1, n1);
            if (m1 != m0) {
              for (int k2 = 0; k2 < p.kblocks; ++k2) {
                if (k2 < p.kb1) { tma_prefetch_2d(&tmA1h, k2 * BK, m1); tma_prefetch_2d(&tmA1l, k2 * BK, m1); }
                else { tma_prefetch_2d(&tmA2h, (k2 - p.kb1) * BK, m1); tma_prefetch_2d(&tmA2l, (k2 - p.kb1) * BK, m1); }
              }
            }
          }
          const uint32_t full = smem_u32(&bar_full[s]);
          mbar_expect_tx(full, Cfg::STAGE_BYTES);
          const uint32_t sAh = smem_u32(smem + s * Cfg::STAGE_BYTES), sAl = sAh + Cfg::A_BYTES;
          const uint32_t sWh = sAl + Cfg::A_BYTES, sWl = sWh + Cfg::W_BYTES;
          if (kb < p.kb1) {
            tma_load_2d(sAh, &tmA1h, full, kb * BK, m0);
            tma_load_2d(sAl, &tmA1l, full, kb * BK, m0);
          } else {
            tma_load_2d(sAh, &tmA2h, full, (kb - p.kb1) * BK, m0);
            tma_load_2d(sAl, &tmA2l, full, (kb - p.kb1) * BK, m0);
          }
          tma_load_2d(sWh, &tmWh, full, kb * BK, n0);
          tma_load_2d(sWl, &tmWl, full, kb * BK, n0);
        }
        __syncwarp();
      }
    }
    return;
  }
  reg_inc<232>();
  const int cw = (warp >> 2) - 1;
  const int cp = 2 * (lane & 3);
  float d[BN / 2];
  int kbg = 0;
  for (int it = 0; it < nlocal; ++it) {
    int m0, n0;
    decode(it, m0, n0);
    tl_event(p.tl, tl_n, 2, it);
    for (int kb = 0; kb < p.kblocks; ++kb, ++kbg) {
      const int s = kbg % STAGES;
      mbar_wait(smem_u32(&bar_full[s]), ((uint32_t)(kbg / STAGES)) & 1u);
      const uint32_t sAh = smem_u32(smem + s * Cfg::STAGE_BYTES) + cw * (64 * 128), sAl = sAh + Cfg::A_BYTES;
      const uint32_t sWh = smem_u32(smem + s * Cfg::STAGE_BYTES) + 2 * Cfg::A_BYTES, sWl = sWh + Cfg::W_BYTES;
      wg_fence();
      kblock_ss<BN>(d, sAh, sAl, sWh, sWl, kb == 0);
      wg_commit();
      if (kb > 0) {
        wg_wait<1>();
        if (lane == 0) mbar_arrive(smem_u32(&bar_empty[(kbg - 1) % STAGES]));
      }
    }
    wg_wait<0>();
    acc_fence(d);
    if (lane == 0) mbar_arrive(smem_u32(&bar_empty[(kbg - 1) % STAGES]));
    tl_event(p.tl, tl_n, 4, it);

    const int r_lo = m0 + cw * 64 + (warp & 3) * 16 + (lane >> 2);
    if constexpr (EPI == EPI_LN) {
      ln_epilogue(d, p.inv_scale, p.bias, p.res_hi, p.res_lo, p.ld_res, p.gamma, p.beta, p.out_hi, p.out_lo, p.ld_out,
                  r_lo, p.M, cp);
    } else if constexpr (EPI == EPI_FAST) {
      const bool ok0 = r_lo < p.M, ok1 = r_lo + 8 < p.M;
      const int64_t o0 = (int64_t)r_lo * p.ld_out + p.out_col0 + n0 + cp, o1 = o0 + (int64_t)8 * p.ld_out;
#pragma unroll
      for (int j = 0; j < BN / 8; ++j) {
        float x[4];
        fast_group<ACT>(d, j, p.inv_scale, __ldg(reinterpret_cast<const float2*>(p.bias + n0 + 8 * j + cp)), x);
        if (ok0) store_split2(p.out_hi, p.out_lo, o0 + 8 * j, x[0], x[1]);
        if (ok1) store_split2(p.out_hi, p.out_lo, o1 + 8 * j, x[2], x[3]);
      }
    } else if constexpr (EPI == EPI_RES) {
      const float sc = p.inv_scale;
#pragma unroll
      for (int j = 0; j < BN / 8; ++j) {
        const int n = n0 + 8 * j + cp;
        if (n >= p.N) continue;
        const float2 b = p.bias ? __ldg(reinterpret_cast<const float2*>(p.bias + n)) : make_float2(0.0f, 0.0f);
#pragma unroll
        for (int h = 0; h < 2; ++h) {
          if (r_lo + 8 * h >= p.M) continue;
          const int64_t o = (int64_t)(r_lo + 8 * h) * p.ldc + n;
          const float2 r = *reinterpret_cast<const float2*>(p.res_f32 + o);
          *reinterpret_cast<float2*>(p.out_f32 + o) =
              make_float2(fmaf(d[4 * j + 2 * h], sc, b.x) + r.x, fmaf(d[4 * j + 2 * h + 1], sc, b.y) + r.y);
        }
      }
    } else if constexpr (EPI == EPI_F32) {
      const float sc = p.inv_scale;
#pragma unroll
      for (int j = 0; j < BN / 8; ++j) {
        const int n = n0 + 8 * j + cp;
        if (n >= p.N) continue;
        const float2 b = p.bias ? __ldg(reinterpret_cast<const float2*>(p.bias + n)) : make_float2(0.0f, 0.0f);
#pragma unroll
        for (int h = 0; h < 2; ++h) {
          if (r_lo + 8 * h >= p.M) continue;
          const float x0 = apply_act(fmaf(d[4 * j + 2 * h], sc, b.x), ACT), x1 = apply_act(fmaf(d[4 * j + 2 * h + 1], sc, b.y), ACT);
          *reinterpret_cast<float2*>(p.out_f32 + (int64_t)(r_lo + 8 * h) * p.ldc + n) = make_float2(x0, x1);
        }
      }
    } else {
#pragma unroll
      for (int h = 0; h < 2; ++h) {
        const int m = r_lo + 8 * h;
        if (m >= p.M) continue;
        int seq = 0, pos = m;
        if (p.in_group < p.M) { seq = m / p.in_group; pos = m - seq * p.in_group; }
        const int64_t orow = (int64_t)seq * p.out_group + p.out_off + pos;
        const bool zero = p.zero_lengths != nullptr && pos >= p.zero_lengths[seq];
        const float* tab = p.addtab ? p.addtab + (int64_t)(p.out_off + pos) * p.N : nullptr;
#pragma unroll
        for (int j = 0; j < BN / 8; ++j) {
#pragma unroll
          for (int e = 0; e < 2; ++e) {
            const int n = n0 + 8 * j + cp + e;
            if (n >= p.N) continue;
            float x = d[4 * j + 2 * h + e] * p.inv_scale + (p.bias ? p.bias[n] : 0.0f);
            if (tab) x += tab[n];
            x = zero ? 0.0f : apply_act(x, p.act);
            if (p.out_hi) {
              __half hh, ll;
              split_f32(x, hh, ll);
              const int64_t o = orow * p.ld_out + p.out_col0 + n;
              p.out_hi[o] = hh; p.out_lo[o] = ll;
            }
            if (p.out_f32) p.out_f32[orow * p.ldc + n] = x;
          }
        }
      }
    }
    tl_event(p.tl, tl_n, 5, it);
  }
  tl_event(p.tl, tl_n, 42);
}

struct FfnParams {
  int M, m_tiles, n_chunks;
  int full, left, parts;
  float* scratch;
  int* flags;
  int reverse;
  long long* tl;
  float inv_s1, inv_s2;
  const float* b1; const float* b2; const float* gamma; const float* beta;
  const __half* res_hi; const __half* res_lo; int ld_res;
  __half* out_hi; __half* out_lo; int ld_out;
};
struct FfnCfg {
  static constexpr int CHUNK = 64;
  static constexpr int X_BYTES = 2 * 4 * BM * 128;
  static constexpr int STAGE_BYTES = 32768, STAGES = 3;
  static constexpr int SMEM_BYTES = X_BYTES + STAGES * STAGE_BYTES + 256 + 1024;
  static_assert(SMEM_BYTES <= 232448, "shared memory budget");
};

__global__ void __launch_bounds__(MMA_THREADS, 1)
k_ffn_tc(const __grid_constant__ CUtensorMap tmXh, const __grid_constant__ CUtensorMap tmXl,
         const __grid_constant__ CUtensorMap tmW1h, const __grid_constant__ CUtensorMap tmW1l,
         const __grid_constant__ CUtensorMap tmW2h, const __grid_constant__ CUtensorMap tmW2l, const FfnParams p) {
  using Cfg = FfnCfg;
  constexpr int STAGES = Cfg::STAGES;
  extern __shared__ uint8_t smem_raw[];
  uint8_t* smem = smem_raw + smem_pad1024(smem_raw);
  uint8_t* ring = smem + Cfg::X_BYTES;
  uint64_t* bar_full = reinterpret_cast<uint64_t*>(ring + STAGES * Cfg::STAGE_BYTES);
  uint64_t* bar_empty = bar_full + STAGES;
  uint64_t* bar_xfull = bar_empty + STAGES;
  uint64_t* bar_xempty = bar_xfull + 1;

  const int warp = __shfl_sync(0xffffffffu, (int)(threadIdx.x >> 5), 0), lane = threadIdx.x & 31;
  int tl_n = 0;
  tl_event(p.tl, tl_n, 40);
  const int ncta = (int)gridDim.x, cid = (int)blockIdx.x;
  const int NC = p.n_chunks;
  struct Item { int mt, c0, c1, mode, piece0; };
  auto rev = [&](int t) { return p.reverse ? p.m_tiles - 1 - t : t; };
  const int nlocal = p.full + (cid < p.left * p.parts ? 1 : 0);
  auto item = [&](int j) -> Item {
    if (j < p.full) return Item{rev(cid + j * ncta), 0, NC, 0, 0};
    const int t = cid / p.parts, part = cid - t * p.parts;
    const int c0 = (part * NC + p.parts - 1) / p.parts, c1 = ((part + 1) * NC + p.parts - 1) / p.parts;
    const int slot0 = t * (p.parts - 1);
    return Item{rev(p.full * ncta + t), c0, c1, p.parts == 1 ? 0 : (part == p.parts - 1 ? 2 : 1),
                p.parts == 1 ? 0 : slot0 + (part == p.parts - 1 ? 0 : part)};
  };
  const int per_tile = 4 * NC;
  int total = p.full * per_tile;
  if (nlocal > p.full) {
    const Item it = item(p.full);
    total += 4 * (it.c1 - it.c0);
  }

  if (threadIdx.x == 0) {
    for (int s = 0; s < STAGES; ++s) {
      mbar_init(smem_u32(&bar_full[s]), 1);
      mbar_init(smem_u32(&bar_empty[s]), CONSUMER_WARPS);
    }
    mbar_init(smem_u32(bar_xfull), 1);
    mbar_init(smem_u32(bar_xempty), CONSUMER_WARPS);
    asm volatile("fence.mbarrier_init.release.cluster;" ::: "memory");
    tma_prefetch_desc(&tmXh); tma_prefetch_desc(&tmXl); tma_prefetch_desc(&tmW1h);
    tma_prefetch_desc(&tmW1l); tma_prefetch_desc(&tmW2h); tma_prefetch_desc(&tmW2l);
  }
  pdl_trigger();
  __syncthreads();
  pdl_wait();
  tl_event(p.tl, tl_n, 41);

  int q_next = 0, x_next = 0;
  auto load_slot = [&](int q) {
    const int j = min(q / per_tile, p.full);
    const Item it = item(j);
    const int r = q - j * per_tile, c = it.c0 + (r >> 2), k = r & 3;
    if (elect_one()) {
      const uint32_t full = smem_u32(&bar_full[q % STAGES]);
      const uint32_t dst = smem_u32(ring + (q % STAGES) * Cfg::STAGE_BYTES);
      mbar_expect_tx(full, Cfg::STAGE_BYTES);
      if (k < 2) {
        for (int kk = 0; kk < 2; ++kk) {
          tma_load_2d(dst + kk * 8192, &tmW1h, full, (2 * k + kk) * BK, c * Cfg::CHUNK);
          tma_load_2d(dst + 16384 + kk * 8192, &tmW1l, full, (2 * k + kk) * BK, c * Cfg::CHUNK);
        }
      } else {
        tma_load_2d(dst, k == 3 ? &tmW2l : &tmW2h, full, c * Cfg::CHUNK, 0);
      }
    }
    __syncwarp();
  };
  auto load_x = [&](int j) {
    if (elect_one()) {
      const int m0 = item(j).mt * BM;
      const uint32_t full = smem_u32(bar_xfull);
      mbar_expect_tx(full, Cfg::X_BYTES);
      for (int kb = 0; kb < 4; ++kb) {
        tma_load_2d(smem_u32(smem + kb * 16384), &tmXh, full, kb * BK, m0);
        tma_load_2d(smem_u32(smem + 65536 + kb * 16384), &tmXl, full, kb * BK, m0);
      }
      if (j + 1 < nlocal) {
        const int m1 = item(j + 1).mt * BM;
        for (int k2 = 0; k2 < 4; ++k2) { tma_prefetch_2d(&tmXh, k2 * BK, m1); tma_prefetch_2d(&tmXl, k2 * BK, m1); }
      }
    }
    __syncwarp();
  };
  auto produce = [&](int need) {
    ring_produce(q_next, total, need, bar_empty, STAGES, load_slot);
    if (x_next < nlocal && __shfl_sync(0xffffffffu, (int)mbar_test(smem_u32(bar_xempty), ((uint32_t)x_next & 1u) ^ 1u), 0))
      load_x(x_next++);
  };
  auto produce_x = [&](int j) {
    while (x_next <= j) {
      mbar_wait(smem_u32(bar_xempty), ((uint32_t)x_next & 1u) ^ 1u);
      load_x(x_next++);
    }
  };

  const int cw = warp >> 2;
  const int cp = 2 * (lane & 3);
  const uint32_t sX = smem_u32(smem) + cw * (64 * 128);
  float acc2[128];
  float acc1[32];
  uint32_t hh[4][4], hl[4][4];
  int rc = 0;
  auto slot_full = [&](int r) { mbar_wait(smem_u32(&bar_full[r % STAGES]), ((uint32_t)(r / STAGES)) & 1u); };
  auto slot_free = [&](int r) { if (lane == 0) mbar_arrive(smem_u32(&bar_empty[r % STAGES])); };
  for (int j = 0; j < nlocal; ++j) {
    const Item it = item(j);
    const int m0 = it.mt * BM;
    if (warp == 0) produce_x(j);
    mbar_wait(smem_u32(bar_xfull), (uint32_t)j & 1u);
    tl_event(p.tl, tl_n, 2, j);
    int pend = -1;
    for (int c = it.c0; c < it.c1; ++c) {
#pragma unroll
      for (int half = 0; half < 2; ++half) {
        if (warp == 0) produce(rc + half);
        slot_full(rc + half);
        tl_event(p.tl, tl_n, 10 + half, c);
        const uint32_t w = smem_u32(ring + ((rc + half) % STAGES) * Cfg::STAGE_BYTES);
        wg_fence();
#pragma unroll
        for (int k = 0; k < 2; ++k) {
          const uint32_t xh = sX + (2 * half + k) * 16384;
          kblock_ss<64>(acc1, xh, xh + 65536, w + k * 8192, w + 16384 + k * 8192, half == 0 && k == 0);
        }
        wg_commit();
      }
      wg_wait<0>();
      acc_fence(acc1);
      tl_event(p.tl, tl_n, 13, c);
      if (pend >= 0) slot_free(pend);
      slot_free(rc); slot_free(rc + 1);
      rc += 2;
      if (c == it.c1 - 1 && lane == 0) mbar_arrive(smem_u32(bar_xempty));
      if (warp == 0) produce(-1);
#pragma unroll
      for (int ks = 0; ks < 4; ++ks) {
#pragma unroll
        for (int g = 0; g < 2; ++g) {
          const int jj = 2 * ks + g, n = c * Cfg::CHUNK + 8 * jj + cp;
          const float2 b = p.b1 ? __ldg(reinterpret_cast<const float2*>(p.b1 + n)) : make_float2(0.0f, 0.0f);
          split2(gelu_fast(fmaf(acc1[4 * jj], p.inv_s1, b.x)), gelu_fast(fmaf(acc1[4 * jj + 1], p.inv_s1, b.y)),
                 hh[ks][2 * g], hl[ks][2 * g]);
          split2(gelu_fast(fmaf(acc1[4 * jj + 2], p.inv_s1, b.x)), gelu_fast(fmaf(acc1[4 * jj + 3], p.inv_s1, b.y)),
                 hh[ks][2 * g + 1], hl[ks][2 * g + 1]);
        }
      }
      tl_event(p.tl, tl_n, 14, c);
      if (warp == 0) produce(rc);
      slot_full(rc);
      tl_event(p.tl, tl_n, 12, c);
      wg_fence();
      {
        const uint64_t wd = make_desc(smem_u32(ring + (rc % STAGES) * Cfg::STAGE_BYTES));
#pragma unroll
        for (int ks = 0; ks < 4; ++ks) {
          wgmma_rs_n256(acc2, hl[ks], wd + 2 * ks, (c == it.c0 && ks == 0) ? 0u : 1u);
          wgmma_rs_n256(acc2, hh[ks], wd + 2 * ks, 1u);
        }
      }
      wg_commit();
      if (warp == 0) produce(rc + 1);
      slot_full(rc + 1);
      {
        const uint64_t wd = make_desc(smem_u32(ring + ((rc + 1) % STAGES) * Cfg::STAGE_BYTES));
#pragma unroll
        for (int ks = 0; ks < 4; ++ks) wgmma_rs_n256(acc2, hh[ks], wd + 2 * ks, 1u);
      }
      wg_commit();
      wg_wait<1>();
      slot_free(rc);
      pend = rc + 1;
      rc += 2;
      if (warp == 0) produce(-1);
    }
    wg_wait<0>();
    acc_fence(acc2);
    if (pend >= 0) slot_free(pend);
    if (warp == 0) produce(-1);
    tl_event(p.tl, tl_n, 4, j);
    const int rl = cw * 64 + (warp & 3) * 16 + (lane >> 2);
    if (it.mode == 1) {
      float* const dst = p.scratch + (size_t)it.piece0 * (BM * 256);
#pragma unroll
      for (int jj = 0; jj < 32; ++jj) {
        *reinterpret_cast<float2*>(dst + rl * 256 + 8 * jj + cp) = make_float2(acc2[4 * jj], acc2[4 * jj + 1]);
        *reinterpret_cast<float2*>(dst + (rl + 8) * 256 + 8 * jj + cp) = make_float2(acc2[4 * jj + 2], acc2[4 * jj + 3]);
      }
      __threadfence();
      named_bar_sync(1, MMA_THREADS);
      if (threadIdx.x == 0) asm volatile("st.release.gpu.global.u32 [%0], %1;" ::"l"(p.flags + it.piece0), "r"(1) : "memory");
      continue;
    }
    const int nparts = it.mode == 2 ? p.parts - 1 : 0;
    if (nparts > 0) {
      if (lane == 0) {
        for (int pp = 0; pp < nparts; ++pp) {
          const int* f = p.flags + it.piece0 + pp;
          uint32_t v = 0;
          long long t_end = clock64() + 4000000000ll;
          do {
            asm volatile("ld.acquire.gpu.global.u32 %0, [%1];" : "=r"(v) : "l"(f) : "memory");
            if (v == 0 && clock64() > t_end) __trap();
          } while (v == 0);
        }
      }
      __syncwarp();
      for (int pp = 0; pp < nparts; ++pp) {
        const float* src = p.scratch + (size_t)(it.piece0 + pp) * (BM * 256);
#pragma unroll
        for (int jj = 0; jj < 32; ++jj) {
          const float2 a = __ldcg(reinterpret_cast<const float2*>(src + rl * 256 + 8 * jj + cp));
          const float2 b = __ldcg(reinterpret_cast<const float2*>(src + (rl + 8) * 256 + 8 * jj + cp));
          acc2[4 * jj] += a.x; acc2[4 * jj + 1] += a.y; acc2[4 * jj + 2] += b.x; acc2[4 * jj + 3] += b.y;
        }
      }
      named_bar_sync(1, MMA_THREADS);
      if (threadIdx.x == 0)
        for (int pp = 0; pp < nparts; ++pp) p.flags[it.piece0 + pp] = 0;
    }
    ln_epilogue(acc2, p.inv_s2, p.b2, p.res_hi, p.res_lo, p.ld_res, p.gamma, p.beta, p.out_hi, p.out_lo, p.ld_out,
                m0 + rl, p.M, cp);
    tl_event(p.tl, tl_n, 5, j);
  }
  tl_event(p.tl, tl_n, 42);
}

struct ProjParams {
  int M, n_chunks, items;
  float inv_scale;
  const float* bias;
  __half* out_hi; __half* out_lo; int ld_out, out_col0;
  long long* tl;
};
struct ProjCfg {
  static constexpr int CHUNK = 128;
  static constexpr int A_BYTES = 2 * 4 * BM * 128;
  static constexpr int STAGE_BYTES = 2 * CHUNK * 128, STAGES = 3;
  static constexpr int SMEM_BYTES = A_BYTES + STAGES * STAGE_BYTES + 256 + 1024;
  static_assert(SMEM_BYTES <= 232448, "shared memory budget");
};

template <int ACT>
__global__ void __launch_bounds__(MMA_THREADS, 1)
k_proj_tc(const __grid_constant__ CUtensorMap tmAh, const __grid_constant__ CUtensorMap tmAl,
          const __grid_constant__ CUtensorMap tmWh, const __grid_constant__ CUtensorMap tmWl, const ProjParams p) {
  using Cfg = ProjCfg;
  constexpr int STAGES = Cfg::STAGES;
  extern __shared__ uint8_t smem_raw[];
  uint8_t* smem = smem_raw + smem_pad1024(smem_raw);
  uint8_t* ring = smem + Cfg::A_BYTES;
  uint64_t* bar_full = reinterpret_cast<uint64_t*>(ring + STAGES * Cfg::STAGE_BYTES);
  uint64_t* bar_empty = bar_full + STAGES;
  uint64_t* bar_afull = bar_empty + STAGES;
  uint64_t* bar_aempty = bar_afull + 4;

  const int warp = __shfl_sync(0xffffffffu, (int)(threadIdx.x >> 5), 0), lane = threadIdx.x & 31;
  int tl_n = 0;
  tl_event(p.tl, tl_n, 40);
  const int NC = p.n_chunks;
  const int t0 = (int)((long long)blockIdx.x * p.items / gridDim.x);
  const int n = (int)((long long)(blockIdx.x + 1) * p.items / gridDim.x) - t0;
  const int mt0 = t0 / NC, ntiles = (t0 + n - 1) / NC - mt0 + 1;
  auto tile_of = [&](int i) { return (t0 + i) / NC - mt0; };
  auto first_of_tile = [&](int i) { return i == 0 || (t0 + i) % NC == 0; };
  auto last_of_tile = [&](int i) { return i == n - 1 || (t0 + i + 1) % NC == 0; };

  if (threadIdx.x == 0) {
    for (int s = 0; s < STAGES; ++s) {
      mbar_init(smem_u32(&bar_full[s]), 1);
      mbar_init(smem_u32(&bar_empty[s]), CONSUMER_WARPS);
    }
    for (int k = 0; k < 4; ++k) {
      mbar_init(smem_u32(&bar_afull[k]), 1);
      mbar_init(smem_u32(&bar_aempty[k]), CONSUMER_WARPS);
    }
    asm volatile("fence.mbarrier_init.release.cluster;" ::: "memory");
    tma_prefetch_desc(&tmAh); tma_prefetch_desc(&tmAl); tma_prefetch_desc(&tmWh); tma_prefetch_desc(&tmWl);
  }
  pdl_trigger();
  __syncthreads();
  pdl_wait();
  tl_event(p.tl, tl_n, 41);

  int q_next = 0, a_next = 0;
  auto load_w = [&](int q) {
    if (elect_one()) {
      const int c = (t0 + (q >> 2)) % NC, k = q & 3;
      const uint32_t full = smem_u32(&bar_full[q % STAGES]);
      const uint32_t dst = smem_u32(ring + (q % STAGES) * Cfg::STAGE_BYTES);
      mbar_expect_tx(full, Cfg::STAGE_BYTES);
      tma_load_2d(dst, &tmWh, full, k * BK, c * Cfg::CHUNK);
      tma_load_2d(dst + Cfg::STAGE_BYTES / 2, &tmWl, full, k * BK, c * Cfg::CHUNK);
    }
    __syncwarp();
  };
  auto load_a = [&](int a) {
    if (elect_one()) {
      const int j = a >> 2, k = a & 3, m0 = (mt0 + j) * BM;
      const uint32_t full = smem_u32(&bar_afull[k]);
      mbar_expect_tx(full, 2 * BM * 128);
      tma_load_2d(smem_u32(smem + k * 16384), &tmAh, full, k * BK, m0);
      tma_load_2d(smem_u32(smem + 65536 + k * 16384), &tmAl, full, k * BK, m0);
      if (k == 0 && j + 1 < ntiles)
        for (int k2 = 0; k2 < 4; ++k2) { tma_prefetch_2d(&tmAh, k2 * BK, m0 + BM); tma_prefetch_2d(&tmAl, k2 * BK, m0 + BM); }
    }
    __syncwarp();
  };
  auto produce = [&](int need_w, int need_a) {
    ring_produce(a_next, 4 * ntiles, need_a, bar_aempty, 4, load_a);
    ring_produce(q_next, 4 * n, need_w, bar_empty, STAGES, load_w);
  };

  const int cw = warp >> 2;
  const int cp = 2 * (lane & 3);
  const uint32_t sA = smem_u32(smem) + cw * (64 * 128);
  float acc0[64], acc1[64];
  auto retire = [&](int q) {
    if (lane == 0) {
      mbar_arrive(smem_u32(&bar_empty[q % STAGES]));
      if (last_of_tile(q >> 2)) mbar_arrive(smem_u32(&bar_aempty[q & 3]));
    }
  };
  auto epilogue = [&](const float (&d)[64], int i) {
    const int t = t0 + i, r_lo = (t / NC) * BM + cw * 64 + (warp & 3) * 16 + (lane >> 2), n0 = (t % NC) * Cfg::CHUNK;
    const int l = lane & 3;
    const bool ok0 = r_lo < p.M, ok1 = r_lo + 8 < p.M;
    const int64_t o0 = (int64_t)r_lo * p.ld_out + p.out_col0 + n0 + 8 * l, o1 = o0 + (int64_t)8 * p.ld_out;
    tl_event(p.tl, tl_n, 52, i);
#pragma unroll
    for (int jb = 0; jb < Cfg::CHUNK / 32; ++jb) {
      uint32_t h0[4], l0[4], h1[4], l1[4];
#pragma unroll
      for (int g = 0; g < 4; ++g) {
        const int j = 4 * jb + g;
        float x[4];
        fast_group<ACT>(d, j, p.inv_scale, __ldg(reinterpret_cast<const float2*>(p.bias + n0 + 8 * j + cp)), x);
        split2(x[0], x[1], h0[g], l0[g]);
        split2(x[2], x[3], h1[g], l1[g]);
      }
      quad_transpose(h0, l); quad_transpose(l0, l); quad_transpose(h1, l); quad_transpose(l1, l);
      if (ok0) {
        *reinterpret_cast<uint4*>(p.out_hi + o0 + 32 * jb) = make_uint4(h0[0], h0[1], h0[2], h0[3]);
        *reinterpret_cast<uint4*>(p.out_lo + o0 + 32 * jb) = make_uint4(l0[0], l0[1], l0[2], l0[3]);
      }
      if (ok1) {
        *reinterpret_cast<uint4*>(p.out_hi + o1 + 32 * jb) = make_uint4(h1[0], h1[1], h1[2], h1[3]);
        *reinterpret_cast<uint4*>(p.out_lo + o1 + 32 * jb) = make_uint4(l1[0], l1[1], l1[2], l1[3]);
      }
    }
    tl_event(p.tl, tl_n, 53, i);
  };
  auto step = [&](int i, float (&cur)[64], float (&prev)[64]) {
    const bool fresh = first_of_tile(i);
    const int j = tile_of(i);
    tl_event(p.tl, tl_n, 50, i);
#pragma unroll
    for (int k = 0; k < 4; ++k) {
      const int q = 4 * i + k;
      if (warp == 0) produce(q, fresh ? 4 * j + k : -1);
      if (fresh) {
        mbar_wait(smem_u32(&bar_afull[k]), (uint32_t)j & 1u);
        if (k == 0) tl_event(p.tl, tl_n, 51, j);
      }
      mbar_wait(smem_u32(&bar_full[q % STAGES]), ((uint32_t)(q / STAGES)) & 1u);
      const uint32_t w = smem_u32(ring + (q % STAGES) * Cfg::STAGE_BYTES), a = sA + k * 16384;
      wg_fence();
      kblock_ss<128>(cur, a, a + 65536, w, w + Cfg::STAGE_BYTES / 2, k == 0);
      wg_commit();
      if (k == 2) {
        if (warp == 0) produce(q + 1, -1);
        if (i > 0) epilogue(prev, i - 1);
      }
      if (q > 0) {
        wg_wait<1>();
        retire(q - 1);
// ... 24 lines not shown
  int sm_count = 132;
  int ffn_fused = 1;
  int ffn_split = 1;
};

TcCtx* tc_create(int device) {
  if (!tc::tmap_encoder()) return nullptr;
  TcCtx* c = new TcCtx();
  c->device = device;
  cudaDeviceGetAttribute(&c->sm_count, cudaDevAttrMultiProcessorCount, device);
  bool ok = true;
  auto opt_in = [&](auto kernel, int bytes) { ok = ok && smem_opt_in(kernel, bytes, "k_gemm_tc"); };
  opt_in(k_gemm_tc<256, EPI_FAST>, TileCfg<256>::SMEM_BYTES); opt_in(k_gemm_tc<128, EPI_FAST>, TileCfg<128>::SMEM_BYTES);
  opt_in(k_gemm_tc<256, EPI_FAST, ACT_GELU>, TileCfg<256>::SMEM_BYTES); opt_in(k_gemm_tc<128, EPI_FAST, ACT_GELU>, TileCfg<128>::SMEM_BYTES);
  opt_in(k_gemm_tc<256, EPI_GENERIC>, TileCfg<256>::SMEM_BYTES); opt_in(k_gemm_tc<128, EPI_GENERIC>, TileCfg<128>::SMEM_BYTES);
  opt_in(k_gemm_tc<256, EPI_FAST, ACT_QUICKGELU>, TileCfg<256>::SMEM_BYTES);
  opt_in(k_gemm_tc<128, EPI_FAST, ACT_QUICKGELU>, TileCfg<128>::SMEM_BYTES);
  opt_in(k_gemm_tc<256, EPI_RES>, TileCfg<256>::SMEM_BYTES); opt_in(k_gemm_tc<128, EPI_RES>, TileCfg<128>::SMEM_BYTES);
  opt_in(k_gemm_tc<256, EPI_LN>, TileCfg<256>::SMEM_BYTES);
  opt_in(k_gemm_tc<256, EPI_FAST, ACT_LEAKY>, TileCfg<256>::SMEM_BYTES); opt_in(k_gemm_tc<128, EPI_FAST, ACT_LEAKY>, TileCfg<128>::SMEM_BYTES);
  opt_in(k_gemm_tc<256, EPI_F32>, TileCfg<256>::SMEM_BYTES); opt_in(k_gemm_tc<128, EPI_F32>, TileCfg<128>::SMEM_BYTES);
  opt_in(k_gemm_tc<256, EPI_F32, ACT_LEAKY>, TileCfg<256>::SMEM_BYTES); opt_in(k_gemm_tc<128, EPI_F32, ACT_LEAKY>, TileCfg<128>::SMEM_BYTES);
  opt_in(k_ffn_tc, FfnCfg::SMEM_BYTES);
  opt_in(k_proj_tc<ACT_NONE>, ProjCfg::SMEM_BYTES); opt_in(k_proj_tc<ACT_GELU>, ProjCfg::SMEM_BYTES);
  opt_in(k_proj_tc<ACT_QUICKGELU>, ProjCfg::SMEM_BYTES); opt_in(k_proj_tc<ACT_LEAKY>, ProjCfg::SMEM_BYTES);
  if (!ok) {
    delete c;
    return nullptr;
  }
  return c;
}
void tc_destroy(TcCtx* c) { delete c; }

static int pick_bn(const GemmArgs& g) { return (g.w.N % 256 == 0) ? 256 : 128; }

bool tc_gemm_supported(const TcCtx* c, const GemmArgs& g) {
  if (!c) return false;
  if (g.a_kind != A_SPLIT || g.M < 1 || g.w.N > (g.wide_n ? MAX_N_WIDE : MAX_N)) return false;
  if (g.K1 <= 0 || g.K1 % BK || g.K2 % BK || g.a1.cols != g.K1) return false;
  if (g.K2 > 0 && g.a2.cols != g.K2) return false;
  if (g.w.K != g.K1 + g.K2) return false;
  if (((uintptr_t)g.a1.hi & 15) || ((uintptr_t)g.w.w & 15)) return false;
  if (g.out.hi && ((g.out.cols % 8) || (g.out_col0 % 8))) return false;
  if (g.res_f32 && (!g.out_f32 || g.out.hi || g.act != ACT_NONE || g.addtab || g.zero_lengths || g.in_group < g.M ||
                    g.out_group != 0 || g.out_off != 0 || (g.w.N % 2) || (g.ldc % 2) || ((uintptr_t)g.out_f32 & 7) ||
                    ((uintptr_t)g.res_f32 & 7)))
    return false;
  return true;
}

bool tc_gemm_ln_supported(const TcCtx* c, const GemmArgs& g, const LnArgs& l) {
  if (!tc_gemm_supported(c, g)) return false;
  if (g.w.N != 256 || l.d != 256 || g.act != ACT_NONE) return false;
  if (l.in_group != 0 || l.c != nullptr || l.out_f32 != nullptr || !l.out.hi) return false;
  if (l.out.cols != 256 || (l.res.hi && l.res.cols != 256)) return false;
  if (l.gamma2 || l.rowvec) return false;
  if (g.addtab || g.zero_lengths || g.in_group < g.M || g.out_group != 0 || g.out_off != 0) return false;
  return true;
}

static void fill_params(const GemmArgs& g, const LnArgs* ln, int bn, TcParams* out) {
  TcParams p{};
  p.M = g.M; p.N = g.w.N; p.kblocks = g.w.K / BK; p.kb1 = g.K1 / BK;
  p.inv_scale = g.w.inv_scale; p.bias = g.w.bias; p.addtab = g.addtab; p.act = g.act;
  p.in_group = g.in_group; p.out_group = g.out_group; p.out_off = g.out_off; p.zero_lengths = g.zero_lengths;
  if (ln) {
    p.out_hi = ln->out.hi; p.out_lo = ln->out.lo(); p.ld_out = ln->out.cols; p.out_col0 = 0;
    p.res_hi = ln->res.hi; p.res_lo = ln->res.hi ? ln->res.lo() : nullptr; p.ld_res = ln->res.cols;
    p.gamma = ln->gamma; p.beta = ln->beta;
  } else {
    p.out_hi = g.out.hi; p.out_lo = g.out.hi ? g.out.lo() : nullptr; p.ld_out = g.out.cols; p.out_col0 = g.out_col0;
    p.out_f32 = g.out_f32; p.ldc = g.ldc; p.res_f32 = g.res_f32;
  }
  p.m_tiles = (g.M + BM - 1) / BM;
  p.n_tiles = (g.w.N + bn - 1) / bn;
  p.tl = tc::mldb_timeline_buffer();
  *out = p;
}

static bool tc_proj(TcCtx* c, const GemmArgs& g, cudaStream_t st) {
  CUtensorMap mAh, mAl, mWh, mWl;
  const bool ok = make_map(&mAh, g.a1.hi, g.M, g.K1, BM) && make_map(&mAl, g.a1.lo(), g.M, g.K1, BM) &&
                  make_map(&mWh, g.w.w, g.w.N, g.w.K, ProjCfg::CHUNK) &&
                  make_map(&mWl, g.w.w + g.w.plane_stride, g.w.N, g.w.K, ProjCfg::CHUNK);
  if (!ok) return false;
  ProjParams p{};
  p.M = g.M; p.n_chunks = g.w.N / ProjCfg::CHUNK; p.items = (g.M + BM - 1) / BM * p.n_chunks;
  p.inv_scale = g.w.inv_scale; p.bias = g.w.bias;
  p.out_hi = g.out.hi; p.out_lo = g.out.lo(); p.ld_out = g.out.cols; p.out_col0 = g.out_col0;
  p.tl = tc::mldb_timeline_buffer();
  const dim3 grid(p.items < c->sm_count ? p.items : c->sm_count);
  switch (g.act) {
    case ACT_GELU: launch_pdl(k_proj_tc<ACT_GELU>, grid, dim3(MMA_THREADS), ProjCfg::SMEM_BYTES, st, mAh, mAl, mWh, mWl, p); break;
    case ACT_QUICKGELU: launch_pdl(k_proj_tc<ACT_QUICKGELU>, grid, dim3(MMA_THREADS), ProjCfg::SMEM_BYTES, st, mAh, mAl, mWh, mWl, p); break;
    case ACT_LEAKY: launch_pdl(k_proj_tc<ACT_LEAKY>, grid, dim3(MMA_THREADS), ProjCfg::SMEM_BYTES, st, mAh, mAl, mWh, mWl, p); break;
    default: launch_pdl(k_proj_tc<ACT_NONE>, grid, dim3(MMA_THREADS), ProjCfg::SMEM_BYTES, st, mAh, mAl, mWh, mWl, p); break;
  }
  return true;
}

bool tc_gemm(TcCtx* c, const GemmArgs& g, const LnArgs* ln, cudaStream_t st) {
  const int bn = ln ? 256 : pick_bn(g);
  const bool fast = !ln && g.out.hi && !g.out_f32 && !g.addtab && !g.zero_lengths && g.in_group >= g.M &&
                    g.out_group == 0 && g.out_off == 0 && g.w.N % bn == 0 && g.w.bias != nullptr &&
                    (g.act == ACT_NONE || g.act == ACT_GELU || g.act == ACT_QUICKGELU || g.act == ACT_LEAKY);
  if (fast && g.K1 == 256 && g.K2 == 0 && ((uintptr_t)g.out.hi & 15) == 0 && ((uintptr_t)g.out.lo() & 15) == 0)
    return tc_proj(c, g, st);
  CUtensorMap mA1h, mA1l, mA2h, mA2l, mWh, mWl;
  bool ok = make_map(&mA1h, g.a1.hi, g.M, g.K1, BM) && make_map(&mA1l, g.a1.lo(), g.M, g.K1, BM);
  if (g.K2 > 0) ok = ok && make_map(&mA2h, g.a2.hi, g.M, g.K2, BM) && make_map(&mA2l, g.a2.lo(), g.M, g.K2, BM);
  else { mA2h = mA1h; mA2l = mA1l; }
  ok = ok && make_map(&mWh, g.w.w, g.w.N, g.w.K, bn) && make_map(&mWl, g.w.w + g.w.plane_stride, g.w.N, g.w.K, bn);
  if (!ok) return false;
  TcParams p;
  fill_params(g, ln, bn, &p);
  const bool f32 = !ln && g.vec_f32 && !g.out.hi && g.out_f32 && !g.res_f32 && !g.addtab && !g.zero_lengths &&
                   g.in_group >= g.M && g.out_group == 0 && g.out_off == 0 && g.w.N % 2 == 0 && g.ldc % 2 == 0 &&
                   ((uintptr_t)g.out_f32 & 7) == 0 && (g.act == ACT_NONE || g.act == ACT_LEAKY);
  const int ntiles = p.m_tiles * p.n_tiles;
  dim3 grid(ntiles < c->sm_count ? ntiles : c->sm_count);
#define MLDB_LAUNCH(BN_, ...)                                                                                      \
  launch_pdl(k_gemm_tc<BN_, __VA_ARGS__>, grid, dim3(NUM_THREADS), TileCfg<BN_>::SMEM_BYTES, st, mA1h, mA1l, mA2h, \
             mA2l, mWh, mWl, p)
#define MLDB_LAUNCH_SHAPE(...)                                                       \
  do {                                                                               \
    if (bn == 256) MLDB_LAUNCH(256, __VA_ARGS__); else MLDB_LAUNCH(128, __VA_ARGS__); \
  } while (0)
  if (ln)                             MLDB_LAUNCH(256, EPI_LN);
  else if (g.res_f32)                 MLDB_LAUNCH_SHAPE(EPI_RES);
  else if (fast && g.act == ACT_GELU) MLDB_LAUNCH_SHAPE(EPI_FAST, ACT_GELU);
  else if (fast && g.act == ACT_QUICKGELU) MLDB_LAUNCH_SHAPE(EPI_FAST, ACT_QUICKGELU);
  else if (fast && g.act == ACT_LEAKY) MLDB_LAUNCH_SHAPE(EPI_FAST, ACT_LEAKY);
  else if (f32 && g.act == ACT_LEAKY) MLDB_LAUNCH_SHAPE(EPI_F32, ACT_LEAKY);
  else if (f32)                       MLDB_LAUNCH_SHAPE(EPI_F32);
  else if (fast)                      MLDB_LAUNCH_SHAPE(EPI_FAST);
  else                                MLDB_LAUNCH_SHAPE(EPI_GENERIC);
#undef MLDB_LAUNCH_SHAPE
#undef MLDB_LAUNCH
  return true;
}

int tc_set_ffn_split(TcCtx* c, int on) {
  if (!c) return 0;
  const int old = c->ffn_split;
  c->ffn_split = on;
  return old;
}
int tc_set_ffn_fused(TcCtx* c, int on) {
  if (!c) return 0;
  const int old = c->ffn_fused;
  c->ffn_fused = on;
  return old;
}
bool tc_ffn_supported(const TcCtx* c, const GemmArgs& g1, const GemmArgs& g2, const LnArgs& l2) {
  if (!c || !c->ffn_fused) return false;
  if (!tc_gemm_supported(c, g1) || !tc_gemm_ln_supported(c, g2, l2)) return false;
  if (g1.K1 != 256 || g1.K2 > 0 || g2.K2 > 0 || g1.M != g2.M) return false;
  if (g1.w.N % FfnCfg::CHUNK || g1.w.N > MAX_N || g1.w.N != g2.K1) return false;
  if (g1.act != ACT_GELU || g1.out_f32 || g1.addtab || g1.zero_lengths) return false;
  if (g1.in_group < g1.M || g1.out_group != 0 || g1.out_off != 0) return false;
  return true;
}
bool tc_ffn(TcCtx* c, const GemmArgs& g1, const GemmArgs& g2, const LnArgs& l2, float* scratch, int* flags, cudaStream_t st) {
  CUtensorMap mXh, mXl, mW1h, mW1l, mW2h, mW2l;
  const int m_tiles = (g1.M + BM - 1) / BM;
  const bool ok = make_map(&mXh, g1.a1.hi, g1.M, g1.K1, BM) && make_map(&mXl, g1.a1.lo(), g1.M, g1.K1, BM) &&
                  make_map(&mW1h, g1.w.w, g1.w.N, g1.w.K, FfnCfg::CHUNK) &&
                  make_map(&mW1l, g1.w.w + g1.w.plane_stride, g1.w.N, g1.w.K, FfnCfg::CHUNK) &&
                  make_map(&mW2h, g2.w.w, g2.w.N, g2.w.K, 256) &&
                  make_map(&mW2l, g2.w.w + g2.w.plane_stride, g2.w.N, g2.w.K, 256);
  if (!ok) return false;
  FfnParams p{};
  p.M = g1.M; p.m_tiles = m_tiles; p.n_chunks = g1.w.N / FfnCfg::CHUNK;
  p.tl = tc::mldb_timeline_buffer();
  p.inv_s1 = g1.w.inv_scale; p.inv_s2 = g2.w.inv_scale;
  p.b1 = g1.w.bias; p.b2 = g2.w.bias; p.gamma = l2.gamma; p.beta = l2.beta;
  p.res_hi = l2.res.hi; p.res_lo = l2.res.hi ? l2.res.lo() : nullptr; p.ld_res = l2.res.cols;
  p.out_hi = l2.out.hi; p.out_lo = l2.out.lo(); p.ld_out = l2.out.cols;
  const int ncta_max = c->sm_count;
  p.full = m_tiles / ncta_max; p.left = m_tiles % ncta_max; p.parts = 1;
  p.scratch = scratch; p.flags = flags;
  if (p.left > 0 && scratch && flags && c->ffn_split) {
    const int parts = std::min(p.n_chunks, ncta_max / p.left);
    if (parts >= 2 && (size_t)p.left * (parts - 1) * (BM * 256 * 4) <= TC_FFN_SCRATCH_BYTES) p.parts = parts;
  }
  const int ncta = p.full > 0 ? ncta_max : p.left * p.parts;
  p.reverse = tc::snake_order();
  launch_pdl(k_ffn_tc, dim3(ncta), dim3(MMA_THREADS), FfnCfg::SMEM_BYTES, st, mXh, mXl, mW1h, mW1l, mW2h, mW2l, p);
  return true;
}
```

### mld_b200/csrc/gemm_tc.h

```cpp
#pragma once
#include "ops.cuh"

struct TcCtx;
TcCtx* tc_create(int device);
void tc_destroy(TcCtx* c);
bool tc_gemm_supported(const TcCtx* c, const GemmArgs& g);
bool tc_gemm_ln_supported(const TcCtx* c, const GemmArgs& g, const LnArgs& l);
bool tc_gemm(TcCtx* c, const GemmArgs& g, const LnArgs* ln, cudaStream_t st);
bool tc_ffn_supported(const TcCtx* c, const GemmArgs& g1, const GemmArgs& g2, const LnArgs& l2);
constexpr size_t TC_FFN_SCRATCH_BYTES = (size_t)160 * 128 * 256 * 4, TC_FFN_FLAG_BYTES = 160 * 4;
bool tc_ffn(TcCtx* c, const GemmArgs& g1, const GemmArgs& g2, const LnArgs& l2, float* scratch, int* flags, cudaStream_t st);
int tc_set_ffn_split(TcCtx* c, int on);
int tc_set_ffn_fused(TcCtx* c, int on);
```

### mld_b200/csrc/tc_common.cuh

```cuda
#pragma once
#include <cuda.h>
#include <stdio.h>
#include <stdlib.h>
#include <string.h>

#include <string>

#include "common.cuh"

namespace tc {

__device__ __forceinline__ uint32_t smem_u32(const void* p) { return (uint32_t)__cvta_generic_to_shared(p); }
__device__ __forceinline__ uint32_t smem_pad1024(const void* raw) { return (1024u - (smem_u32(raw) & 1023u)) & 1023u; }

__device__ __forceinline__ void mbar_init(uint32_t bar, uint32_t count) {
  asm volatile("mbarrier.init.shared::cta.b64 [%0], %1;" ::"r"(bar), "r"(count) : "memory");
}
__device__ __forceinline__ void mbar_expect_tx(uint32_t bar, uint32_t bytes) {
  asm volatile("mbarrier.arrive.expect_tx.shared::cta.b64 _, [%0], %1;" ::"r"(bar), "r"(bytes) : "memory");
}
__device__ __forceinline__ void mbar_arrive(uint32_t bar) {
  asm volatile("mbarrier.arrive.shared::cta.b64 _, [%0];" ::"r"(bar) : "memory");
}
__device__ __forceinline__ void mbar_wait(uint32_t bar, uint32_t parity) {
  uint32_t done = 0, spins = 0;
  long long t0 = 0;
  do {
    asm volatile(
        "{\n\t.reg .pred p;\n\t"
        "mbarrier.try_wait.parity.shared::cta.b64 p, [%1], %2;\n\t"
        "selp.u32 %0, 1, 0, p;\n\t}"
        : "=r"(done)
        : "r"(bar), "r"(parity)
        : "memory");
    if (!done && (++spins & 1023u) == 0) {
      const long long now = clock64();
      if (t0 == 0) t0 = now;
      else if (now - t0 > 4000000000ll) __trap();
    }
  } while (!done);
}
__device__ __forceinline__ bool mbar_test(uint32_t bar, uint32_t parity) {
  uint32_t done;
  asm volatile(
      "{\n\t.reg .pred p;\n\t"
      "mbarrier.test_wait.parity.shared::cta.b64 p, [%1], %2;\n\t"
      "selp.u32 %0, 1, 0, p;\n\t}"
      : "=r"(done)
      : "r"(bar), "r"(parity)
      : "memory");
  return done != 0;
}

__device__ __forceinline__ void tma_load_2d(uint32_t dst, const CUtensorMap* map, uint32_t bar, int c0, int c1) {
  asm volatile(
      "cp.async.bulk.tensor.2d.shared::cluster.global.mbarrier::complete_tx::bytes [%0], [%1, {%3, %4}], [%2];"
      ::"r"(dst), "l"(reinterpret_cast<uint64_t>(map)), "r"(bar), "r"(c0), "r"(c1)
      : "memory");
}
__device__ __forceinline__ void tma_load_3d(uint32_t dst, const CUtensorMap* map, uint32_t bar, int c0, int c1, int c2) {
  asm volatile(
      "cp.async.bulk.tensor.3d.shared::cluster.global.mbarrier::complete_tx::bytes [%0], [%1, {%3, %4, %5}], [%2];"
      ::"r"(dst), "l"(reinterpret_cast<uint64_t>(map)), "r"(bar), "r"(c0), "r"(c1), "r"(c2)
      : "memory");
}
__device__ __forceinline__ void tma_prefetch_2d(const CUtensorMap* map, int c0, int c1) {
  asm volatile("cp.async.bulk.prefetch.tensor.2d.L2.global.tile [%0, {%1, %2}];"
               ::"l"(reinterpret_cast<uint64_t>(map)), "r"(c0), "r"(c1) : "memory");
}
__device__ __forceinline__ void tma_prefetch_desc(const CUtensorMap* map) {
  asm volatile("prefetch.tensormap [%0];" ::"l"(reinterpret_cast<uint64_t>(map)) : "memory");
}

__device__ __forceinline__ bool elect_one() {
  uint32_t pred;
  asm volatile("{\n\t.reg .pred p;\n\telect.sync _|p, 0xffffffff;\n\tselp.u32 %0, 1, 0, p;\n\t}" : "=r"(pred));
  return pred != 0;
}

template <int N> __device__ __forceinline__ void reg_dec() { asm volatile("setmaxnreg.dec.sync.aligned.u32 %0;" ::"n"(N)); }
template <int N> __device__ __forceinline__ void reg_inc() { asm volatile("setmaxnreg.inc.sync.aligned.u32 %0;" ::"n"(N)); }
__device__ __forceinline__ void named_bar_sync(int id, int threads) {
  asm volatile("bar.sync %0, %1;" ::"r"(id), "r"(threads) : "memory");
}

__device__ __forceinline__ void wg_fence() { asm volatile("wgmma.fence.sync.aligned;" ::: "memory"); }
__device__ __forceinline__ void wg_commit() { asm volatile("wgmma.commit_group.sync.aligned;" ::: "memory"); }
template <int N> __device__ __forceinline__ void wg_wait() { asm volatile("wgmma.wait_group.sync.aligned %0;" ::"n"(N) : "memory"); }

template <int N> __device__ __forceinline__ void acc_fence(float (&d)[N]) {
#pragma unroll
  for (int i = 0; i < N; ++i) asm volatile("" : "+f"(d[i])::"memory");
}

__device__ __forceinline__ uint64_t make_desc(uint32_t saddr) {
  return (uint64_t)((saddr >> 4) & 0x3FFF) | ((uint64_t)1 << 16) | ((uint64_t)(1024 >> 4) << 32) | ((uint64_t)1 << 62);
}
__device__ __forceinline__ void wgmma_ss_n256(float (&d)[128], uint64_t adesc, uint64_t bdesc, uint32_t acc) {
  asm volatile(
      "{\n\t.reg .pred p;\n\t"
      "setp.ne.b32 p, %130, 0;\n\t"
      "wgmma.mma_async.sync.aligned.m64n256k16.f32.f16.f16 "
      "{%0, %1, %2, %3, %4, %5, %6, %7, %8, %9, %10, %11, %12, %13, %14, %15, "
      "%16, %17, %18, %19, %20, %21, %22, %23, %24, %25, %26, %27, %28, %29, %30, %31, "
      "%32, %33, %34, %35, %36, %37, %38, %39, %40, %41, %42, %43, %44, %45, %46, %47, "
      "%48, %49, %50, %51, %52, %53, %54, %55, %56, %57, %58, %59, %60, %61, %62, %63, "
      "%64, %65, %66, %67, %68, %69, %70, %71, %72, %73, %74, %75, %76, %77, %78, %79, "
      "%80, %81, %82, %83, %84, %85, %86, %87, %88, %89, %90, %91, %92, %93, %94, %95, "
      "%96, %97, %98, %99, %100, %101, %102, %103, %104, %105, %106, %107, %108, %109, %110, %111, "
      "%112, %113, %114, %115, %116, %117, %118, %119, %120, %121, %122, %123, %124, %125, %126, %127}, "
      "%128, %129, p, 1, 1, 0, 0;\n\t}"
      : "+f"(d[0]), "+f"(d[1]), "+f"(d[2]), "+f"(d[3]), "+f"(d[4]), "+f"(d[5]), "+f"(d[6]), "+f"(d[7]),
        "+f"(d[8]), "+f"(d[9]), "+f"(d[10]), "+f"(d[11]), "+f"(d[12]), "+f"(d[13]), "+f"(d[14]), "+f"(d[15]),
        "+f"(d[16]), "+f"(d[17]), "+f"(d[18]), "+f"(d[19]), "+f"(d[20]), "+f"(d[21]), "+f"(d[22]), "+f"(d[23]),
        "+f"(d[24]), "+f"(d[25]), "+f"(d[26]), "+f"(d[27]), "+f"(d[28]), "+f"(d[29]), "+f"(d[30]), "+f"(d[31]),
        "+f"(d[32]), "+f"(d[33]), "+f"(d[34]), "+f"(d[35]), "+f"(d[36]), "+f"(d[37]), "+f"(d[38]), "+f"(d[39]),
        "+f"(d[40]), "+f"(d[41]), "+f"(d[42]), "+f"(d[43]), "+f"(d[44]), "+f"(d[45]), "+f"(d[46]), "+f"(d[47]),
        "+f"(d[48]), "+f"(d[49]), "+f"(d[50]), "+f"(d[51]), "+f"(d[52]), "+f"(d[53]), "+f"(d[54]), "+f"(d[55]),
        "+f"(d[56]), "+f"(d[57]), "+f"(d[58]), "+f"(d[59]), "+f"(d[60]), "+f"(d[61]), "+f"(d[62]), "+f"(d[63]),
        "+f"(d[64]), "+f"(d[65]), "+f"(d[66]), "+f"(d[67]), "+f"(d[68]), "+f"(d[69]), "+f"(d[70]), "+f"(d[71]),
        "+f"(d[72]), "+f"(d[73]), "+f"(d[74]), "+f"(d[75]), "+f"(d[76]), "+f"(d[77]), "+f"(d[78]), "+f"(d[79]),
        "+f"(d[80]), "+f"(d[81]), "+f"(d[82]), "+f"(d[83]), "+f"(d[84]), "+f"(d[85]), "+f"(d[86]), "+f"(d[87]),
        "+f"(d[88]), "+f"(d[89]), "+f"(d[90]), "+f"(d[91]), "+f"(d[92]), "+f"(d[93]), "+f"(d[94]), "+f"(d[95]),
        "+f"(d[96]), "+f"(d[97]), "+f"(d[98]), "+f"(d[99]), "+f"(d[100]), "+f"(d[101]), "+f"(d[102]), "+f"(d[103]),
        "+f"(d[104]), "+f"(d[105]), "+f"(d[106]), "+f"(d[107]), "+f"(d[108]), "+f"(d[109]), "+f"(d[110]), "+f"(d[111]),
        "+f"(d[112]), "+f"(d[113]), "+f"(d[114]), "+f"(d[115]), "+f"(d[116]), "+f"(d[117]), "+f"(d[118]), "+f"(d[119]),
        "+f"(d[120]), "+f"(d[121]), "+f"(d[122]), "+f"(d[123]), "+f"(d[124]), "+f"(d[125]), "+f"(d[126]), "+f"(d[127])
      : "l"(adesc), "l"(bdesc), "r"(acc)
      : "memory");
}
__device__ __forceinline__ void wgmma_ss_n128(float (&d)[64], uint64_t adesc, uint64_t bdesc, uint32_t acc) {
  asm volatile(
      "{\n\t.reg .pred p;\n\t"
      "setp.ne.b32 p, %66, 0;\n\t"
      "wgmma.mma_async.sync.aligned.m64n128k16.f32.f16.f16 "
      "{%0, %1, %2, %3, %4, %5, %6, %7, %8, %9, %10, %11, %12, %13, %14, %15, "
      "%16, %17, %18, %19, %20, %21, %22, %23, %24, %25, %26, %27, %28, %29, %30, %31, "
      "%32, %33, %34, %35, %36, %37, %38, %39, %40, %41, %42, %43, %44, %45, %46, %47, "
      "%48, %49, %50, %51, %52, %53, %54, %55, %56, %57, %58, %59, %60, %61, %62, %63}, "
      "%64, %65, p, 1, 1, 0, 0;\n\t}"
      : "+f"(d[0]), "+f"(d[1]), "+f"(d[2]), "+f"(d[3]), "+f"(d[4]), "+f"(d[5]), "+f"(d[6]), "+f"(d[7]),
        "+f"(d[8]), "+f"(d[9]), "+f"(d[10]), "+f"(d[11]), "+f"(d[12]), "+f"(d[13]), "+f"(d[14]), "+f"(d[15]),
        "+f"(d[16]), "+f"(d[17]), "+f"(d[18]), "+f"(d[19]), "+f"(d[20]), "+f"(d[21]), "+f"(d[22]), "+f"(d[23]),
        "+f"(d[24]), "+f"(d[25]), "+f"(d[26]), "+f"(d[27]), "+f"(d[28]), "+f"(d[29]), "+f"(d[30]), "+f"(d[31]),
        "+f"(d[32]), "+f"(d[33]), "+f"(d[34]), "+f"(d[35]), "+f"(d[36]), "+f"(d[37]), "+f"(d[38]), "+f"(d[39]),
        "+f"(d[40]), "+f"(d[41]), "+f"(d[42]), "+f"(d[43]), "+f"(d[44]), "+f"(d[45]), "+f"(d[46]), "+f"(d[47]),
        "+f"(d[48]), "+f"(d[49]), "+f"(d[50]), "+f"(d[51]), "+f"(d[52]), "+f"(d[53]), "+f"(d[54]), "+f"(d[55]),
        "+f"(d[56]), "+f"(d[57]), "+f"(d[58]), "+f"(d[59]), "+f"(d[60]), "+f"(d[61]), "+f"(d[62]), "+f"(d[63])
      : "l"(adesc), "l"(bdesc), "r"(acc)
      : "memory");
}
__device__ __forceinline__ void wgmma_ss_n96(float (&d)[48], uint64_t adesc, uint64_t bdesc, uint32_t acc) {
  asm volatile(
      "{\n\t.reg .pred p;\n\t"
      "setp.ne.b32 p, %50, 0;\n\t"
      "wgmma.mma_async.sync.aligned.m64n96k16.f32.f16.f16 "
      "{%0, %1, %2, %3, %4, %5, %6, %7, %8, %9, %10, %11, %12, %13, %14, %15, "
      "%16, %17, %18, %19, %20, %21, %22, %23, %24, %25, %26, %27, %28, %29, %30, %31, "
      "%32, %33, %34, %35, %36, %37, %38, %39, %40, %41, %42, %43, %44, %45, %46, %47}, "
      "%48, %49, p, 1, 1, 0, 0;\n\t}"
      : "+f"(d[0]), "+f"(d[1]), "+f"(d[2]), "+f"(d[3]), "+f"(d[4]), "+f"(d[5]), "+f"(d[6]), "+f"(d[7]),
        "+f"(d[8]), "+f"(d[9]), "+f"(d[10]), "+f"(d[11]), "+f"(d[12]), "+f"(d[13]), "+f"(d[14]), "+f"(d[15]),
        "+f"(d[16]), "+f"(d[17]), "+f"(d[18]), "+f"(d[19]), "+f"(d[20]), "+f"(d[21]), "+f"(d[22]), "+f"(d[23]),
        "+f"(d[24]), "+f"(d[25]), "+f"(d[26]), "+f"(d[27]), "+f"(d[28]), "+f"(d[29]), "+f"(d[30]), "+f"(d[31]),
        "+f"(d[32]), "+f"(d[33]), "+f"(d[34]), "+f"(d[35]), "+f"(d[36]), "+f"(d[37]), "+f"(d[38]), "+f"(d[39]),
        "+f"(d[40]), "+f"(d[41]), "+f"(d[42]), "+f"(d[43]), "+f"(d[44]), "+f"(d[45]), "+f"(d[46]), "+f"(d[47])
      : "l"(adesc), "l"(bdesc), "r"(acc)
      : "memory");
}
__device__ __forceinline__ void wgmma_ss_n64(float (&d)[32], uint64_t adesc, uint64_t bdesc, uint32_t acc) {
  asm volatile(
      "{\n\t.reg .pred p;\n\t"
      "setp.ne.b32 p, %34, 0;\n\t"
      "wgmma.mma_async.sync.aligned.m64n64k16.f32.f16.f16 "
      "{%0, %1, %2, %3, %4, %5, %6, %7, %8, %9, %10, %11, %12, %13, %14, %15, "
      "%16, %17, %18, %19, %20, %21, %22, %23, %24, %25, %26, %27, %28, %29, %30, %31}, "
      "%32, %33, p, 1, 1, 0, 0;\n\t}"
      : "+f"(d[0]), "+f"(d[1]), "+f"(d[2]), "+f"(d[3]), "+f"(d[4]), "+f"(d[5]), "+f"(d[6]), "+f"(d[7]),
        "+f"(d[8]), "+f"(d[9]), "+f"(d[10]), "+f"(d[11]), "+f"(d[12]), "+f"(d[13]), "+f"(d[14]), "+f"(d[15]),
        "+f"(d[16]), "+f"(d[17]), "+f"(d[18]), "+f"(d[19]), "+f"(d[20]), "+f"(d[21]), "+f"(d[22]), "+f"(d[23]),
        "+f"(d[24]), "+f"(d[25]), "+f"(d[26]), "+f"(d[27]), "+f"(d[28]), "+f"(d[29]), "+f"(d[30]), "+f"(d[31])
      : "l"(adesc), "l"(bdesc), "r"(acc)
      : "memory");
}
__device__ __forceinline__ void wgmma_rs_n256(float (&d)[128], const uint32_t (&a)[4], uint64_t bdesc, uint32_t acc) {
  asm volatile(
      "{\n\t.reg .pred p;\n\t"
      "setp.ne.b32 p, %133, 0;\n\t"
      "wgmma.mma_async.sync.aligned.m64n256k16.f32.f16.f16 "
      "{%0, %1, %2, %3, %4, %5, %6, %7, %8, %9, %10, %11, %12, %13, %14, %15, "
      "%16, %17, %18, %19, %20, %21, %22, %23, %24, %25, %26, %27, %28, %29, %30, %31, "
      "%32, %33, %34, %35, %36, %37, %38, %39, %40, %41, %42, %43, %44, %45, %46, %47, "
      "%48, %49, %50, %51, %52, %53, %54, %55, %56, %57, %58, %59, %60, %61, %62, %63, "
      "%64, %65, %66, %67, %68, %69, %70, %71, %72, %73, %74, %75, %76, %77, %78, %79, "
      "%80, %81, %82, %83, %84, %85, %86, %87, %88, %89, %90, %91, %92, %93, %94, %95, "
      "%96, %97, %98, %99, %100, %101, %102, %103, %104, %105, %106, %107, %108, %109, %110, %111, "
      "%112, %113, %114, %115, %116, %117, %118, %119, %120, %121, %122, %123, %124, %125, %126, %127}, "
      "{%128, %129, %130, %131}, %132, p, 1, 1, 0;\n\t}"
      : "+f"(d[0]), "+f"(d[1]), "+f"(d[2]), "+f"(d[3]), "+f"(d[4]), "+f"(d[5]), "+f"(d[6]), "+f"(d[7]),
        "+f"(d[8]), "+f"(d[9]), "+f"(d[10]), "+f"(d[11]), "+f"(d[12]), "+f"(d[13]), "+f"(d[14]), "+f"(d[15]),
        "+f"(d[16]), "+f"(d[17]), "+f"(d[18]), "+f"(d[19]), "+f"(d[20]), "+f"(d[21]), "+f"(d[22]), "+f"(d[23]),
        "+f"(d[24]), "+f"(d[25]), "+f"(d[26]), "+f"(d[27]), "+f"(d[28]), "+f"(d[29]), "+f"(d[30]), "+f"(d[31]),
        "+f"(d[32]), "+f"(d[33]), "+f"(d[34]), "+f"(d[35]), "+f"(d[36]), "+f"(d[37]), "+f"(d[38]), "+f"(d[39]),
        "+f"(d[40]), "+f"(d[41]), "+f"(d[42]), "+f"(d[43]), "+f"(d[44]), "+f"(d[45]), "+f"(d[46]), "+f"(d[47]),
        "+f"(d[48]), "+f"(d[49]), "+f"(d[50]), "+f"(d[51]), "+f"(d[52]), "+f"(d[53]), "+f"(d[54]), "+f"(d[55]),
        "+f"(d[56]), "+f"(d[57]), "+f"(d[58]), "+f"(d[59]), "+f"(d[60]), "+f"(d[61]), "+f"(d[62]), "+f"(d[63]),
        "+f"(d[64]), "+f"(d[65]), "+f"(d[66]), "+f"(d[67]), "+f"(d[68]), "+f"(d[69]), "+f"(d[70]), "+f"(d[71]),
        "+f"(d[72]), "+f"(d[73]), "+f"(d[74]), "+f"(d[75]), "+f"(d[76]), "+f"(d[77]), "+f"(d[78]), "+f"(d[79]),
        "+f"(d[80]), "+f"(d[81]), "+f"(d[82]), "+f"(d[83]), "+f"(d[84]), "+f"(d[85]), "+f"(d[86]), "+f"(d[87]),
        "+f"(d[88]), "+f"(d[89]), "+f"(d[90]), "+f"(d[91]), "+f"(d[92]), "+f"(d[93]), "+f"(d[94]), "+f"(d[95]),
        "+f"(d[96]), "+f"(d[97]), "+f"(d[98]), "+f"(d[99]), "+f"(d[100]), "+f"(d[101]), "+f"(d[102]), "+f"(d[103]),
        "+f"(d[104]), "+f"(d[105]), "+f"(d[106]), "+f"(d[107]), "+f"(d[108]), "+f"(d[109]), "+f"(d[110]), "+f"(d[111]),
        "+f"(d[112]), "+f"(d[113]), "+f"(d[114]), "+f"(d[115]), "+f"(d[116]), "+f"(d[117]), "+f"(d[118]), "+f"(d[119]),
        "+f"(d[120]), "+f"(d[121]), "+f"(d[122]), "+f"(d[123]), "+f"(d[124]), "+f"(d[125]), "+f"(d[126]), "+f"(d[127])
      : "r"(a[0]), "r"(a[1]), "r"(a[2]), "r"(a[3]), "l"(bdesc), "r"(acc)
      : "memory");
}
__device__ __forceinline__ void wgmma_rs_n64_tb(float (&d)[32], const uint32_t (&a)[4], uint64_t bdesc, uint32_t acc) {
  asm volatile(
      "{\n\t.reg .pred p;\n\t"
      "setp.ne.b32 p, %37, 0;\n\t"
      "wgmma.mma_async.sync.aligned.m64n64k16.f32.f16.f16 "
      "{%0, %1, %2, %3, %4, %5, %6, %7, %8, %9, %10, %11, %12, %13, %14, %15, "
      "%16, %17, %18, %19, %20, %21, %22, %23, %24, %25, %26, %27, %28, %29, %30, %31}, "
      "{%32, %33, %34, %35}, %36, p, 1, 1, 1;\n\t}"
// ... 106 lines not shown
```

### mld_b200/engine.py

```python
from __future__ import annotations

import ctypes as C
from typing import Dict, Optional, Sequence

import torch

from . import _lib
from ._lib import MldbConfig, check


def _ptr(t: Optional[torch.Tensor]):
    return None if t is None else C.c_void_p(t.data_ptr())


def _f32c(t: torch.Tensor, device) -> torch.Tensor:
    return t.to(device=device, dtype=torch.float32).contiguous()


class Engine:

    def __init__(self, cfg: MldbConfig, device: int | torch.device = 0):
        self._h = None
        self.lib = _lib.lib()
        if not torch.cuda.is_available():
            raise RuntimeError("mld_b200 needs a CUDA device (sm_90a); there is no CPU fallback")
        dev = torch.device(device) if not isinstance(device, int) else torch.device("cuda", device)
        self.device = dev
        self.cfg = cfg
        h = C.c_void_p()
        check(self.lib.mldb_create(C.byref(cfg), dev.index or 0, C.byref(h)), "mldb_create")
        self._h = h
        self.timesteps: Optional[torch.Tensor] = None

    def __del__(self):
        try:
            if self._h is not None:
                self.lib.mldb_destroy(self._h)
                self._h = None
        except Exception:
            pass

    def load_state_dict(self, sd: Dict[str, torch.Tensor], prefix: str = ""):
        for k, v in sd.items():
            t = v.detach().to(dtype=torch.float32).contiguous()
            shape = (C.c_int64 * t.dim())(*t.shape)
            check(self.lib.mldb_load_tensor(self._h, (prefix + k).encode(), _ptr(t), shape, t.dim(),
                                            _lib.DTYPE_F32), f"mldb_load_tensor({prefix + k})")

    def finalize(self):
        check(self.lib.mldb_finalize_weights(self._h, None), "mldb_finalize_weights")

    def set_mean_std(self, mean: torch.Tensor, std: torch.Tensor):
        m = mean.detach().float().contiguous().cpu()
        s = std.detach().float().contiguous().cpu()
        check(self.lib.mldb_set_mean_std(self._h, _ptr(m), _ptr(s), m.numel()), "mldb_set_mean_std")

    def set_option(self, name: str, value: str):
        check(self.lib.mldb_set_option(self._h, name.encode(), value.encode()), "mldb_set_option")

    def profile_op(self, op: str, B: int, S_ctx: int, iters: int = 20) -> float:
        ms = C.c_float()
        check(self.lib.mldb_profile_op(self._h, op.encode(), B, S_ctx, iters, C.byref(ms)), "mldb_profile_op")
        return float(ms.value)

    def profile_steps(self, cond: torch.Tensor, init_noise: torch.Tensor):
        c, z0 = self._cond(cond), _f32c(init_noise, self.device)
        B = z0.shape[0]
        self._check_latent(z0, B, "init_noise")
        self._check_cond(c, 2 * B if self.cfg_on else B)
        S = c.shape[1] if c.dim() == 3 else 1
        n = 0 if self.timesteps is None else len(self.timesteps)
        ms = (C.c_float * n)()
        check(self.lib.mldb_profile_steps(self._h, _ptr(c), _ptr(z0), B, S, ms), "mldb_profile_steps")
        return [float(v) for v in ms]

    def debug_gemm(self, A, W, bias=None, gamma=None, beta=None, R=None, K1=0, act=0, use_tc=True, split_out=False,
                   in_place=False):
        A = _f32c(A, self.device)
        Wc = W.detach().float().contiguous().cpu()
        host = [None if t is None else t.detach().float().contiguous().cpu() for t in (bias, gamma, beta)]
        Rd = None if R is None else _f32c(R, self.device)
        M, K = A.shape
        N = Wc.shape[0]
        out = torch.empty((M, N), dtype=torch.float32, device=self.device)
        if in_place:
            if Rd is None or gamma is not None:
                raise ValueError("in_place needs R and no gamma (the residual-add epilogue)")
            out = Rd = Rd.clone()
        check(self.lib.mldb_debug_gemm(self._h, _ptr(A), _ptr(Wc), _ptr(host[0]), _ptr(host[1]), _ptr(host[2]),
                                       _ptr(Rd), M, N, K, K1, act, int(use_tc), int(split_out), _ptr(out), self._stream()),
              "mldb_debug_gemm")
        return out

    def debug_ffn(self, X, W1, b1, W2, b2, gamma, beta, mode=2):
        X = _f32c(X, self.device)
        host = [t.detach().float().contiguous().cpu() for t in (W1, b1, W2, b2, gamma, beta)]
        M, d = X.shape
        ff = host[0].shape[0]
        out = torch.empty((M, d), dtype=torch.float32, device=self.device)
        check(self.lib.mldb_debug_ffn(self._h, _ptr(X), *[_ptr(t) for t in host], M, d, ff, int(mode), _ptr(out),
                                      self._stream()), "mldb_debug_ffn")
        return out

    def debug_attention(self, q, nseq, Lq, heads, lengths=None, mode=2, kv=None, Lk=None, kv_prefix=0,
                        causal=False):
        q = _f32c(q, self.device)
        kvd = None if kv is None else _f32c(kv, self.device)
        d = q.shape[1] // 3 if kv is None else q.shape[1]
        Lk = Lq if Lk is None else Lk
        if q.shape[0] != nseq * Lq or (kvd is not None and tuple(kvd.shape) != (nseq * Lk, 2 * d)):
            raise ValueError("debug_attention: shape mismatch")
        ln = None if lengths is None else torch.as_tensor(lengths, dtype=torch.int32, device=self.device).contiguous()
        out = torch.empty((nseq * Lq, d), dtype=torch.float32, device=self.device)
        fn = self.lib.mldb_debug_attention_causal if causal else self.lib.mldb_debug_attention
        check(fn(self._h, _ptr(q), _ptr(kvd), _ptr(ln), int(kv_prefix), nseq, Lq, Lk, heads, d // heads, int(mode),
                 _ptr(out), self._stream()), "mldb_debug_attention")
        return out

    def text_configure(self, tcfg):
        check(self.lib.mldb_text_configure(self._h, C.byref(tcfg)), "mldb_text_configure")
        self.text_cfg = tcfg

    def text_encode(self, ids: torch.Tensor, mode: int = _lib.TEXT_POOLED) -> torch.Tensor:
        tc = getattr(self, "text_cfg", None)
        if tc is None:
            raise RuntimeError("text_configure() was not called before finalize()")
        if ids.dim() != 2 or ids.shape[0] < 1 or not 1 <= ids.shape[1] <= tc.max_positions:
            raise ValueError(f"ids must be [n, L] with 1 <= L <= {tc.max_positions}, got {tuple(ids.shape)}")
        if ids.numel() and (int(ids.min()) < 0 or int(ids.max()) >= tc.vocab_size):
            raise ValueError(f"token ids must lie in [0, {tc.vocab_size})")
        d_ids = ids.to(device=self.device, dtype=torch.int64).contiguous()
        n, L = d_ids.shape
        shape = (n, L, tc.hidden) if mode == _lib.TEXT_HIDDEN else (n, tc.projection_dim)
        out = torch.empty(shape, dtype=torch.float32, device=self.device)
        check(self.lib.mldb_text_encode(self._h, _ptr(d_ids), n, L, int(mode), _ptr(out), self._stream()),
              "mldb_text_encode")
        return out

    def t2m_configure(self, tcfg):
        check(self.lib.mldb_t2m_configure(self._h, C.byref(tcfg)), "mldb_t2m_configure")
        self.t2m_cfg = tcfg

    def _t2m(self, part: int, name: str):
        tc = getattr(self, "t2m_cfg", None)
        if tc is None or not tc.parts & part:
            raise RuntimeError(f"the T2M {name} encoder was not configured (t2m_configure) before finalize()")
        return tc

    def _t2m_lengths(self, lengths, B: int, L: int) -> torch.Tensor:
        ln = torch.as_tensor(lengths).reshape(-1)
        if ln.numel() != B:
            raise ValueError(f"lengths must hold {B} values, got {ln.numel()}")
        if ln.dtype.is_floating_point or ln.dtype == torch.bool:
            raise ValueError("lengths must be integers")
        if B and (int(ln.min()) < 1 or int(ln.max()) > L):
            raise ValueError(f"lengths must lie in [1, {L}]")
        return ln.to(device=self.device, dtype=torch.int32).contiguous()

    def t2m_movement(self, x: torch.Tensor) -> torch.Tensor:
        tc = self._t2m(_lib.T2M_MOVEMENT, "movement")
        if x.dim() != 3 or x.shape[2] != tc.dim_pose or x.shape[0] < 1 or x.shape[1] < 4:
            raise ValueError(f"x must be [B >= 1, T >= 4, {tc.dim_pose}], got {tuple(x.shape)}")
        x = x.to(device=self.device, dtype=torch.float32)
        if x.stride(2) != 1 or x.stride(0) != x.shape[1] * x.stride(1):
            x = x.contiguous()
        B, T = x.shape[:2]
        out = torch.empty((B, T // 2 // 2, tc.dim_move_latent), dtype=torch.float32, device=self.device)
        check(self.lib.mldb_t2m_movement(self._h, _ptr(x), x.stride(1), B, T, _ptr(out), self._stream()),
              "mldb_t2m_movement")
        return out

    def t2m_motion(self, x: torch.Tensor, lengths) -> torch.Tensor:
        tc = self._t2m(_lib.T2M_MOTION, "motion")
        if x.dim() != 3 or x.shape[2] != tc.dim_move_latent or x.shape[0] < 1 or x.shape[1] < 1:
            raise ValueError(f"x must be [B >= 1, L >= 1, {tc.dim_move_latent}], got {tuple(x.shape)}")
        xd = _f32c(x, self.device)
        B, L = xd.shape[:2]
        ln = self._t2m_lengths(lengths, B, L)
        out = torch.empty((B, tc.dim_motion_latent), dtype=torch.float32, device=self.device)
        check(self.lib.mldb_t2m_motion(self._h, _ptr(xd), _ptr(ln), B, L, _ptr(out), self._stream()), "mldb_t2m_motion")
        return out

    def t2m_text(self, word_embs: torch.Tensor, pos_ohot: torch.Tensor, lengths) -> torch.Tensor:
        tc = self._t2m(_lib.T2M_TEXT, "text")
        if word_embs.dim() != 3 or word_embs.shape[2] != tc.dim_word or word_embs.shape[0] < 1 or word_embs.shape[1] < 1:
            raise ValueError(f"word_embs must be [B >= 1, L >= 1, {tc.dim_word}], got {tuple(word_embs.shape)}")
        if tuple(pos_ohot.shape) != (*word_embs.shape[:2], tc.dim_pos_ohot):
            raise ValueError(f"pos_ohot must be [{word_embs.shape[0]}, {word_embs.shape[1]}, {tc.dim_pos_ohot}], "
                             f"got {tuple(pos_ohot.shape)}")
        w, p = _f32c(word_embs, self.device), _f32c(pos_ohot, self.device)
        B, L = w.shape[:2]
        ln = self._t2m_lengths(lengths, B, L)
        out = torch.empty((B, tc.dim_coemb_hidden), dtype=torch.float32, device=self.device)
        check(self.lib.mldb_t2m_text(self._h, _ptr(w), _ptr(p), _ptr(ln), B, L, _ptr(out), self._stream()),
              "mldb_t2m_text")
        return out

    def kernel_stats(self, reset: bool = False) -> Dict[str, int]:
        arr = (C.c_int64 * len(_lib.KSTAT_NAMES))()
        check(self.lib.mldb_kernel_stats(self._h, arr, len(_lib.KSTAT_NAMES)), "mldb_kernel_stats")
        if reset:
            check(self.lib.mldb_reset_kernel_stats(self._h), "mldb_reset_kernel_stats")
        return {k: int(v) for k, v in zip(_lib.KSTAT_NAMES, arr)}

    @property
    def launch_count(self) -> int:
        return int(self.lib.mldb_launch_count(self._h))

    def _stream(self):
        return C.c_void_p(torch.cuda.current_stream(self.device).cuda_stream)

    def set_timesteps(self, n: int) -> torch.Tensor:
        ts = torch.empty(n, dtype=torch.int64)
        check(self.lib.mldb_scheduler_set_timesteps(self._h, n, _ptr(ts)), "mldb_scheduler_set_timesteps")
        self.timesteps = ts
        return ts

    def scheduler_step(self, model_output: torch.Tensor, timestep: int, sample: torch.Tensor,
                       noise: Optional[torch.Tensor] = None) -> torch.Tensor:
        mo, sa = _f32c(model_output, self.device), _f32c(sample, self.device)
        nz = None if noise is None else _f32c(noise, self.device)
        out = torch.empty_like(sa)
        check(self.lib.mldb_scheduler_step(self._h, _ptr(mo), int(timestep), _ptr(sa), _ptr(nz),
                                           sa.numel(), _ptr(out), self._stream()), "mldb_scheduler_step")
        return out

    @property
    def cfg_on(self) -> bool:
        return self.cfg.guidance_scale > 1.0

    def _check_cond(self, c: torch.Tensor, Bx: int):
        if self.cfg.cond_kind == _lib.COND_TEXT:
            if c.dim() != 3 or c.shape[0] != Bx or c.shape[2] != self.cfg.text_dim or c.shape[1] < 1:
                raise ValueError(f"condition must be [{Bx}, S, {self.cfg.text_dim}] (uncond half first when guidance "
                                 f"is on), got {tuple(c.shape)}")
        elif c.numel() != Bx:
            raise ValueError(f"action condition must hold {Bx} class ids ([{Bx}, 1]), got {tuple(c.shape)}")

    def _check_latent(self, x: torch.Tensor, rows: int, what: str):
        cfg = self.cfg
        want = (rows, x.shape[1], cfg.nfeats) if cfg.diffusion_only else (rows, cfg.n_lat, cfg.latent_dim)
        if x.dim() != 3 or tuple(x.shape) != want:
            raise ValueError(f"{what} must be {list(want)}, got {tuple(x.shape)}")

    def _check_lengths(self, ln: Optional[torch.Tensor], B: int, T: Optional[int] = None):
        if ln is None:
            return
        if ln.numel() != B:
            raise ValueError(f"lengths must have {B} entries, got {ln.numel()}")
        if T is not None and not isinstance(T, bool):
            host = ln if ln.device.type == "cpu" else None
            if host is not None and (int(host.max()) > T or int(host.min()) < 1):
                raise ValueError(f"lengths must lie in [1, {T}]")

# ... 228 lines not shown
```

Measured before the change: 813.5.

## Fuse attention out-projection and LayerNorm into the tensor-core FFN kernel

Adds a transformer-layer 'tail' path that folds the attention out-projection GEMM, its residual LayerNorm, the two FFN GEMMs and the final LayerNorm into one persistent wgmma kernel. The first LayerNorm now runs in place on the shared-memory X tile, and the output is written back with a TMA bulk store. The fused path is taken only for small M (at most two 128-row tiles) unless forced. The aim is to remove one kernel launch and a global round trip of the intermediate activation per layer, at the cost of more register pressure and extra TMA descriptors. A debug entry point and profiling ops are added alongside.

```diff
diff --git a/include/mldb.h b/include/mldb.h
--- a/include/mldb.h
+++ b/include/mldb.h
@@ -137,6 +137,11 @@
                    const float* b2, const float* gamma, const float* beta, int32_t M, int32_t d, int32_t ff,
                    int32_t mode, float* out, void* stream);
 
+int mldb_debug_tail(mldb_handle* h, const float* att, const float* X, const float* Wo, const float* bo,
+                    const float* gamma1, const float* beta1, const float* W1, const float* b1, const float* W2,
+                    const float* b2, const float* gamma2, const float* beta2, int32_t M, int32_t d, int32_t ff,
+                    int32_t mode, int32_t out_rows, float* out, void* stream);
+
 int mldb_debug_attention(mldb_handle* h, const float* Q, const float* KV, const int32_t* lengths, int32_t kv_prefix,
                          int32_t nseq, int32_t Lq, int32_t Lk, int32_t heads, int32_t hd, int32_t mode, float* out,
                          void* stream);
diff --git a/mld_b200/_lib.py b/mld_b200/_lib.py
--- a/mld_b200/_lib.py
+++ b/mld_b200/_lib.py
@@ -80,6 +80,7 @@
     "mldb_debug_gemm": (C.c_int, [_P, _P, _P, _P, _P, _P, _P, C.c_int32, C.c_int32, C.c_int32, C.c_int32,
                                   C.c_int32, C.c_int32, C.c_int32, _P, _P]),
     "mldb_debug_ffn": (C.c_int, [_P, _P, _P, _P, _P, _P, _P, _P, C.c_int32, C.c_int32, C.c_int32, C.c_int32, _P, _P]),
+    "mldb_debug_tail": (C.c_int, [_P] * 13 + [C.c_int32] * 5 + [_P, _P]),
     "mldb_debug_attention": (C.c_int, [_P, _P, _P, _P, C.c_int32, C.c_int32, C.c_int32, C.c_int32, C.c_int32, C.c_int32,
                                        C.c_int32, _P, _P]),
     "mldb_debug_attention_causal": (C.c_int, [_P, _P, _P, _P, C.c_int32, C.c_int32, C.c_int32, C.c_int32, C.c_int32,
diff --git a/mld_b200/csrc/engine.cu b/mld_b200/csrc/engine.cu
--- a/mld_b200/csrc/engine.cu
+++ b/mld_b200/csrc/engine.cu
@@ -418,16 +418,39 @@
     kcount(h, MLDB_KSTAT_ATTN_SIMT);
   }
 }
+static int ffn_scratch_slot(const mldb_handle* h, cudaStream_t st) {
+  int k = 0;
+  for (int i = 0; i < mldb_handle::MAX_BRANCHES - 1; ++i) if (st == h->br_stream[i]) k = i + 1;
+  return k;
+}
 static void op_ffn(mldb_handle* h, const GemmArgs& g1, const GemmArgs& g2, const LnArgs& l2, float* cf32, cudaStream_t st) {
   if (h->use_tc && tc_ffn_supported(h->tc, g1, g2, l2)) {
-    int k = 0;
-    for (int i = 0; i < mldb_handle::MAX_BRANCHES - 1; ++i) if (st == h->br_stream[i]) k = i + 1;
+    const int k = ffn_scratch_slot(h, st);
     if (!tc_ffn(h->tc, g1, g2, l2, h->ffn_scratch[k], h->ffn_flags[k], st)) h->op_failed = true;
     kcount(h, MLDB_KSTAT_FFN_TC);
     return;
   }
   op_gemm(h, g1, st);
   op_gemm_ln(h, g2, l2, cf32, st);
+}
+static void op_tail(mldb_handle* h, const LinW& wo, const LnW& n1, const LinW& l1, const LinW& l2, const LnW& n2,
+                    ActBuf att, ActBuf x, ActBuf x1, ActBuf hbuf, ActBuf xout, int M, int d, int ff, float* cf32,
+                    cudaStream_t st, int fuse = 1) {
+  GemmArgs go; go.a1 = att; go.K1 = d; go.M = M; go.w = wo;
+  LnArgs ln1; ln1.res = x; ln1.gamma = n1.g; ln1.beta = n1.b; ln1.M = M; ln1.d = d; ln1.out = x1;
+  GemmArgs g1; g1.a1 = x1; g1.K1 = d; g1.M = M; g1.w = l1; g1.act = ACT_GELU; g1.out = hbuf;
+  GemmArgs g2; g2.a1 = hbuf; g2.K1 = ff; g2.M = M; g2.w = l2;
+  LnArgs ln2; ln2.res = x1; ln2.gamma = n2.g; ln2.beta = n2.b; ln2.M = M; ln2.d = d; ln2.out = xout;
+  constexpr int FUSE_MAX_TILES = 2;
+  const bool small = (M + 127) / 128 <= FUSE_MAX_TILES;
+  if (fuse && (fuse == 2 || small) && h->use_tc && tc_tail_supported(h->tc, go, ln1, g1, g2, ln2)) {
+    const int k = ffn_scratch_slot(h, st);
+    if (!tc_tail(h->tc, go, ln1, g1, g2, ln2, h->ffn_scratch[k], h->ffn_flags[k], st)) h->op_failed = true;
+    kcount(h, MLDB_KSTAT_FFN_TC);
+    return;
+  }
+  op_gemm_ln(h, go, ln1, cf32, st);
+  op_ffn(h, g1, g2, ln2, cf32, st);
 }
 
 static int alloc_act(mldb_handle* h, int rows, int cols, ActBuf* out) {
@@ -504,9 +527,8 @@
   LnArgs l; l.res = res; l.gamma = n.g; l.beta = n.b; l.M = M; l.d = d; l.out = xout;
   op_gemm_ln(h, g, l, cf32, st);
 }
-static void self_attn_block(mldb_handle* h, const LinW& in_proj, const LinW& out_proj, const LnW& n,
-                            ActBuf xin, ActBuf xout, StackWs& ws, const SeqInfo& si, int heads,
-                            cudaStream_t st) {
+static void self_attn(mldb_handle* h, const LinW& in_proj, ActBuf xin, StackWs& ws, const SeqInfo& si, int heads,
+                      cudaStream_t st) {
   const int d = ws.d;
   GemmArgs g; g.a1 = xin; g.K1 = d; g.M = ws.M; g.w = in_proj; g.out = ws.qkv;
   op_gemm(h, g, st);
@@ -514,7 +536,12 @@
   a.Lk = ws.L; a.nseq = ws.nseq; a.heads = heads; a.hd = d / heads;
   a.lengths = si.lengths; a.kv_prefix = si.kv_prefix; a.len_mod = si.len_mod; a.seq0 = 0; a.out = ws.att;
   op_attn(h, a, st);
-  out_proj_ln(h, out_proj, n, ws.att, xin, xout, ws.M, d, ws.cf32, st);
+}
+static void self_attn_block(mldb_handle* h, const LinW& in_proj, const LinW& out_proj, const LnW& n,
+                            ActBuf xin, ActBuf xout, StackWs& ws, const SeqInfo& si, int heads,
+                            cudaStream_t st) {
+  self_attn(h, in_proj, xin, ws, si, heads, st);
+  out_proj_ln(h, out_proj, n, ws.att, xin, xout, ws.M, ws.d, ws.cf32, st);
 }
 static void ffn_block(mldb_handle* h, const LinW& l1, const LinW& l2, const LnW& n, ActBuf xin,
                       ActBuf xout, StackWs& ws, int act, cudaStream_t st) {
@@ -525,8 +552,8 @@
 }
 static void enc_layer(mldb_handle* h, const StackW& sw, const EncW& w, ActBuf xin, ActBuf xout,
                       StackWs& ws, const SeqInfo& si, cudaStream_t st) {
-  self_attn_block(h, w.in_proj, w.out_proj, w.n1, xin, ws.x1, ws, si, sw.heads, st);
-  ffn_block(h, w.l1, w.l2, w.n2, ws.x1, xout, ws, ACT_GELU, st);
+  self_attn(h, w.in_proj, xin, ws, si, sw.heads, st);
+  op_tail(h, w.out_proj, w.n1, w.l1, w.l2, w.n2, ws.att, xin, ws.x1, ws.h, xout, ws.M, ws.d, ws.ff, ws.cf32, st);
 }
 static void dec_layer(mldb_handle* h, const StackW& sw, const DecW& w, ActBuf xin, ActBuf xout,
                       ActBuf mem, StackWs& ws, const SeqInfo& si, cudaStream_t st) {
@@ -585,11 +612,7 @@
   a.Lk = ws.L; a.nseq = ws.nseq; a.heads = sw.heads; a.hd = d / sw.heads; a.lengths = si.lengths;
   a.kv_prefix = si.kv_prefix; a.len_mod = si.len_mod; a.out = ws.satt;
   op_attn(h, a, st);
-  out_proj_ln(h, w.out_proj, w.n1, ws.satt, ws.sx, ws.sx1, R, d, ws.cf32, st);
-  GemmArgs g1; g1.a1 = ws.sx1; g1.K1 = d; g1.M = R; g1.w = w.l1; g1.act = ACT_GELU; g1.out = ws.sh;
-  GemmArgs g2; g2.a1 = ws.sh; g2.K1 = ws.ff; g2.M = R; g2.w = w.l2;
-  LnArgs l2; l2.res = ws.sx1; l2.gamma = w.n2.g; l2.beta = w.n2.b; l2.M = R; l2.d = d; l2.out = ws.sout;
-  op_ffn(h, g1, g2, l2, ws.cf32, st);
+  op_tail(h, w.out_proj, w.n1, w.l1, w.l2, w.n2, ws.satt, ws.sx, ws.sx1, ws.sh, ws.sout, R, d, ws.ff, ws.cf32, st);
   return ws.sout;
 }
 
@@ -1807,6 +1830,10 @@
       op_gemm_ln(h, g, l, ws.cf32, st);
     } else if (!strcmp(op, "ffn")) {
       ffn_block(h, w.l1, w.l2, w.n2, ws.x1, ws.cur[0], ws, ACT_GELU, st);
+    } else if (!strcmp(op, "tail")) {
+      op_tail(h, w.out_proj, w.n1, w.l1, w.l2, w.n2, ws.att, ws.x0, ws.x1, ws.h, ws.cur[0], ws.M, d, ws.ff, ws.cf32, st);
+    } else if (!strcmp(op, "tail_fused")) {
+      op_tail(h, w.out_proj, w.n1, w.l1, w.l2, w.n2, ws.att, ws.x0, ws.x1, ws.h, ws.cur[0], ws.M, d, ws.ff, ws.cf32, st, 2);
     } else if (!strcmp(op, "layer")) {
       enc_layer(h, h->den, w, ws.x0, ws.cur[0], ws, si, st);
     } else {
@@ -2237,6 +2264,50 @@
   return MLDB_OK;
 }
 
+extern "C" int mldb_debug_tail(mldb_handle* h, const float* att, const float* X, const float* Wo, const float* bo,
+                               const float* gamma1, const float* beta1, const float* W1, const float* b1,
+                               const float* W2, const float* b2, const float* gamma2, const float* beta2, int32_t M,
+                               int32_t d, int32_t ff, int32_t mode, int32_t out_rows, float* out, void* stream) {
+  if (!h || !att || !X || !Wo || !gamma1 || !beta1 || !W1 || !W2 || !gamma2 || !beta2 || !out || M <= 0 || d <= 0 ||
+      ff <= 0 || out_rows < M)
+    FAIL(MLDB_ERR_INVALID, "bad argument");
+  DeviceGuard guard(h->device);
+  cudaStream_t st = (cudaStream_t)stream;
+  const size_t n_alloc0 = h->allocs.size();
+  LinW wo, l1, l2;
+  LnW n1, n2;
+  TRY(pack_linear(h, Wo, d, d, bo, &wo));
+  TRY(pack_linear(h, W1, ff, d, b1, &l1));
+  TRY(pack_linear(h, W2, d, ff, b2, &l2));
+  TRY(upload_f32(h, gamma1, d, &n1.g));
+  TRY(upload_f32(h, beta1, d, &n1.b));
+  TRY(upload_f32(h, gamma2, d, &n2.g));
+  TRY(upload_f32(h, beta2, d, &n2.b));
+  ActBuf a, x, x1, hb, o;
+  float* cf32 = nullptr;
+  TRY(alloc_act(h, M, d, &a));
+  TRY(alloc_act(h, M, d, &x));
+  TRY(alloc_act(h, M, d, &x1));
+  TRY(alloc_act(h, M, ff, &hb));
+  TRY(alloc_act(h, out_rows, d, &o));
+  TRY(dev_alloc(h, (void**)&cf32, (size_t)M * d * sizeof(float)));
+  k_rows_to_split<<<nblk((int64_t)out_rows * d), 256, 0, st>>>(o, out, d, out_rows, d, 1 << 30, 0, 0, 0, nullptr);
+  k_rows_to_split<<<nblk((int64_t)M * d), 256, 0, st>>>(a, att, d, M, d, 1 << 30, 0, 0, 0, nullptr);
+  k_rows_to_split<<<nblk((int64_t)M * d), 256, 0, st>>>(x, X, d, M, d, 1 << 30, 0, 0, 0, nullptr);
+  const bool saved = h->use_tc;
+  h->use_tc = mode != 0;
+  const int saved_fused = tc_set_ffn_fused(h->tc, 1);
+  op_tail(h, wo, n1, l1, l2, n2, a, x, x1, hb, o, M, d, ff, cf32, st, mode == 2 ? 2 : 0);
+  h->use_tc = saved;
+  tc_set_ffn_fused(h->tc, saved_fused);
+  k_split_to_f32<<<nblk((int64_t)out_rows * d), 256, 0, st>>>(o, out, (int64_t)out_rows * d);
+  cudaError_t e = cudaStreamSynchronize(st);
+  if (e == cudaSuccess) e = cudaGetLastError();
+  while (h->allocs.size() > n_alloc0) { cudaFree(h->allocs.back()); h->allocs.pop_back(); }
+  if (e != cudaSuccess) FAIL(MLDB_ERR_CUDA, "debug tail: %s", cudaGetErrorString(e));
+  return MLDB_OK;
+}
+
 static int debug_attention(mldb_handle* h, const float* Q, const float* KV, const int32_t* lengths, int32_t kv_prefix,
                            int32_t nseq, int32_t Lq, int32_t Lk, int32_t heads, int32_t hd, int32_t mode, int causal,
                            float* out, void* stream) {
diff --git a/mld_b200/csrc/gemm_tc.cu b/mld_b200/csrc/gemm_tc.cu
--- a/mld_b200/csrc/gemm_tc.cu
+++ b/mld_b200/csrc/gemm_tc.cu
@@ -81,33 +81,19 @@
   }
 }
 
-__device__ __forceinline__ void ln_epilogue(float (&d)[128], float sc, const float* bias, const __half* res_hi,
-                                            const __half* res_lo, int ld_res, const float* gamma, const float* beta,
-                                            __half* out_hi, __half* out_lo, int ld_out, int r_lo, int M, int cp) {
-  const bool ok0 = r_lo < M, ok1 = r_lo + 8 < M;
+template <class Res, class Out>
+__device__ __forceinline__ void ln_rows(float (&d)[128], float sc, const float* bias, const float* gamma,
+                                        const float* beta, int cp, Res&& res, Out&& out) {
   float s0 = 0.0f, s1 = 0.0f;
 #pragma unroll
   for (int j = 0; j < 32; ++j) {
     const int n = 8 * j + cp;
     const float2 b = bias ? __ldg(reinterpret_cast<const float2*>(bias + n)) : make_float2(0.0f, 0.0f);
-    float x0 = fmaf(d[4 * j], sc, b.x), x1 = fmaf(d[4 * j + 1], sc, b.y);
-    float x2 = fmaf(d[4 * j + 2], sc, b.x), x3 = fmaf(d[4 * j + 3], sc, b.y);
-    if (res_hi) {
-      if (ok0) {
-        const int64_t o = (int64_t)r_lo * ld_res + n;
-        const float2 h = __half22float2(*reinterpret_cast<const __half2*>(res_hi + o));
-        const float2 l = __half22float2(*reinterpret_cast<const __half2*>(res_lo + o));
-        x0 = (x0 + h.x) + l.x; x1 = (x1 + h.y) + l.y;
-      }
-      if (ok1) {
-        const int64_t o = (int64_t)(r_lo + 8) * ld_res + n;
-        const float2 h = __half22float2(*reinterpret_cast<const __half2*>(res_hi + o));
-        const float2 l = __half22float2(*reinterpret_cast<const __half2*>(res_lo + o));
-        x2 = (x2 + h.x) + l.x; x3 = (x3 + h.y) + l.y;
-      }
-    }
-    d[4 * j] = x0; d[4 * j + 1] = x1; d[4 * j + 2] = x2; d[4 * j + 3] = x3;
-    s0 += x0 + x1; s1 += x2 + x3;
+    float x[4] = {fmaf(d[4 * j], sc, b.x), fmaf(d[4 * j + 1], sc, b.y), fmaf(d[4 * j + 2], sc, b.x),
+                  fmaf(d[4 * j + 3], sc, b.y)};
+    res(j, x);
+    d[4 * j] = x[0]; d[4 * j + 1] = x[1]; d[4 * j + 2] = x[2]; d[4 * j + 3] = x[3];
+    s0 += x[0] + x[1]; s1 += x[2] + x[3];
   }
   const float mean0 = quad_sum(s0) * (1.0f / 256), mean1 = quad_sum(s1) * (1.0f / 256);
   float q0 = 0.0f, q1 = 0.0f;
@@ -123,13 +109,64 @@
   for (int j = 0; j < 32; ++j) {
     const int n = 8 * j + cp;
     const float2 g = __ldg(reinterpret_cast<const float2*>(gamma + n)), be = __ldg(reinterpret_cast<const float2*>(beta + n));
-    if (ok0)
-      store_split2(out_hi, out_lo, (int64_t)r_lo * ld_out + n, fmaf(d[4 * j] * rstd0, g.x, be.x),
-                   fmaf(d[4 * j + 1] * rstd0, g.y, be.y));
-    if (ok1)
-      store_split2(out_hi, out_lo, (int64_t)(r_lo + 8) * ld_out + n, fmaf(d[4 * j + 2] * rstd1, g.x, be.x),
-                   fmaf(d[4 * j + 3] * rstd1, g.y, be.y));
-  }
+    const float y[4] = {fmaf(d[4 * j] * rstd0, g.x, be.x), fmaf(d[4 * j + 1] * rstd0, g.y, be.y),
+                        fmaf(d[4 * j + 2] * rstd1, g.x, be.x), fmaf(d[4 * j + 3] * rstd1, g.y, be.y)};
+    out(j, y);
+  }
+}
+
+__device__ __forceinline__ void ln_epilogue(float (&d)[128], float sc, const float* bias, const __half* res_hi,
+                                            const __half* res_lo, int ld_res, const float* gamma, const float* beta,
+                                            __half* out_hi, __half* out_lo, int ld_out, int r_lo, int M, int cp) {
+  const bool ok0 = r_lo < M, ok1 = r_lo + 8 < M;
+  ln_rows(d, sc, bias, gamma, beta, cp,
+          [&](int j, float (&x)[4]) {
+            if (!res_hi) return;
+            const int n = 8 * j + cp;
+            if (ok0) {
+              const int64_t o = (int64_t)r_lo * ld_res + n;
+              const float2 h = __half22float2(*reinterpret_cast<const __half2*>(res_hi + o));
+              const float2 l = __half22float2(*reinterpret_cast<const __half2*>(res_lo + o));
+              x[0] = (x[0] + h.x) + l.x; x[1] = (x[1] + h.y) + l.y;
+            }
+            if (ok1) {
+              const int64_t o = (int64_t)(r_lo + 8) * ld_res + n;
+              const float2 h = __half22float2(*reinterpret_cast<const __half2*>(res_hi + o));
+              const float2 l = __half22float2(*reinterpret_cast<const __half2*>(res_lo + o));
+              x[2] = (x[2] + h.x) + l.x; x[3] = (x[3] + h.y) + l.y;
+            }
+          },
+          [&](int j, const float (&y)[4]) {
+            const int n = 8 * j + cp;
+            if (ok0) store_split2(out_hi, out_lo, (int64_t)r_lo * ld_out + n, y[0], y[1]);
+            if (ok1) store_split2(out_hi, out_lo, (int64_t)(r_lo + 8) * ld_out + n, y[2], y[3]);
+          });
+}
+
+__device__ __forceinline__ void ln_tile(float (&d)[128], float sc, const float* bias, const float* gamma,
+                                        const float* beta, uint8_t* tile, int rl, int lane, int cp) {
+  uint8_t* const row0 = tile + rl * 128 + cp * 2;
+  const int sw = lane >> 2;
+  auto at = [&](int j, int h, int plane) {
+    return reinterpret_cast<__half2*>(row0 + plane * 65536 + h * 1024 + (j >> 3) * 16384 + (((j & 7) ^ sw) << 4));
+  };
+  ln_rows(d, sc, bias, gamma, beta, cp,
+          [&](int j, float (&x)[4]) {
+#pragma unroll
+            for (int h = 0; h < 2; ++h) {
+              const float2 hi = __half22float2(*at(j, h, 0)), lo = __half22float2(*at(j, h, 1));
+              x[2 * h] = (x[2 * h] + hi.x) + lo.x; x[2 * h + 1] = (x[2 * h + 1] + hi.y) + lo.y;
+            }
+          },
+          [&](int j, const float (&y)[4]) {
+#pragma unroll
+            for (int h = 0; h < 2; ++h) {
+              uint32_t hi, lo;
+              split2(y[2 * h], y[2 * h + 1], hi, lo);
+              *reinterpret_cast<uint32_t*>(at(j, h, 0)) = hi;
+              *reinterpret_cast<uint32_t*>(at(j, h, 1)) = lo;
+            }
+          });
 }
 
 template <int BN, int EPI, int ACT = ACT_NONE>
@@ -322,11 +359,11 @@
   float* scratch;
   int* flags;
   int reverse;
+  int prefix;
   long long* tl;
-  float inv_s1, inv_s2;
+  float inv_s0, inv_s1, inv_s2;
+  const float* b0; const float* gamma1; const float* beta1;
   const float* b1; const float* b2; const float* gamma; const float* beta;
-  const __half* res_hi; const __half* res_lo; int ld_res;
-  __half* out_hi; __half* out_lo; int ld_out;
 };
 struct FfnCfg {
   static constexpr int CHUNK = 64;
@@ -339,7 +376,10 @@
 __global__ void __launch_bounds__(MMA_THREADS, 1)
 k_ffn_tc(const __grid_constant__ CUtensorMap tmXh, const __grid_constant__ CUtensorMap tmXl,
          const __grid_constant__ CUtensorMap tmW1h, const __grid_constant__ CUtensorMap tmW1l,
-         const __grid_constant__ CUtensorMap tmW2h, const __grid_constant__ CUtensorMap tmW2l, const FfnParams p) {
+         const __grid_constant__ CUtensorMap tmW2h, const __grid_constant__ CUtensorMap tmW2l,
+         const __grid_constant__ CUtensorMap tmAh, const __grid_constant__ CUtensorMap tmAl,
+         const __grid_constant__ CUtensorMap tmWoh, const __grid_constant__ CUtensorMap tmWol,
+         const __grid_constant__ CUtensorMap tmYh, const __grid_constant__ CUtensorMap tmYl, const FfnParams p) {
   using Cfg = FfnCfg;
   constexpr int STAGES = Cfg::STAGES;
   extern __shared__ uint8_t smem_raw[];
@@ -348,7 +388,7 @@
   uint64_t* bar_full = reinterpret_cast<uint64_t*>(ring + STAGES * Cfg::STAGE_BYTES);
   uint64_t* bar_empty = bar_full + STAGES;
   uint64_t* bar_xfull = bar_empty + STAGES;
-  uint64_t* bar_xempty = bar_xfull + 1;
+  uint64_t* bar_xempty = bar_xfull + 4;
 
   const int warp = __shfl_sync(0xffffffffu, (int)(threadIdx.x >> 5), 0), lane = threadIdx.x & 31;
   int tl_n = 0;
@@ -366,23 +406,30 @@
     return Item{rev(p.full * ncta + t), c0, c1, p.parts == 1 ? 0 : (part == p.parts - 1 ? 2 : 1),
                 p.parts == 1 ? 0 : slot0 + (part == p.parts - 1 ? 0 : part)};
   };
-  const int per_tile = 4 * NC;
+  const int PRE = p.prefix ? 8 : 0;
+  const int per_tile = PRE + 4 * NC;
   int total = p.full * per_tile;
   if (nlocal > p.full) {
     const Item it = item(p.full);
-    total += 4 * (it.c1 - it.c0);
-  }
+    total += PRE + 4 * (it.c1 - it.c0);
+  }
+  const int XG = p.prefix ? 2 : 1;
+  const int xtotal = nlocal * 4 * XG;
 
   if (threadIdx.x == 0) {
     for (int s = 0; s < STAGES; ++s) {
       mbar_init(smem_u32(&bar_full[s]), 1);
       mbar_init(smem_u32(&bar_empty[s]), CONSUMER_WARPS);
     }
-    mbar_init(smem_u32(bar_xfull), 1);
-    mbar_init(smem_u32(bar_xempty), CONSUMER_WARPS);
+    for (int kb = 0; kb < 4; ++kb) {
+      mbar_init(smem_u32(&bar_xfull[kb]), 1);
+      mbar_init(smem_u32(&bar_xempty[kb]), CONSUMER_WARPS);
+    }
     asm volatile("fence.mbarrier_init.release.cluster;" ::: "memory");
     tma_prefetch_desc(&tmXh); tma_prefetch_desc(&tmXl); tma_prefetch_desc(&tmW1h);
     tma_prefetch_desc(&tmW1l); tma_prefetch_desc(&tmW2h); tma_prefetch_desc(&tmW2l);
+    tma_prefetch_desc(&tmYh); tma_prefetch_desc(&tmYl);
+    if (p.prefix) { tma_prefetch_desc(&tmAh); tma_prefetch_desc(&tmAl); tma_prefetch_desc(&tmWoh); tma_prefetch_desc(&tmWol); }
   }
   pdl_trigger();
   __syncthreads();
@@ -393,52 +440,56 @@
   auto load_slot = [&](int q) {
     const int j = min(q / per_tile, p.full);
     const Item it = item(j);
-    const int r = q - j * per_tile, c = it.c0 + (r >> 2), k = r & 3;
+    const int r = q - j * per_tile;
     if (elect_one()) {
       const uint32_t full = smem_u32(&bar_full[q % STAGES]);
       const uint32_t dst = smem_u32(ring + (q % STAGES) * Cfg::STAGE_BYTES);
       mbar_expect_tx(full, Cfg::STAGE_BYTES);
-      if (k < 2) {
-        for (int kk = 0; kk < 2; ++kk) {
-          tma_load_2d(dst + kk * 8192, &tmW1h, full, (2 * k + kk) * BK, c * Cfg::CHUNK);
-          tma_load_2d(dst + 16384 + kk * 8192, &tmW1l, full, (2 * k + kk) * BK, c * Cfg::CHUNK);
-        }
+      if (r < PRE) {
+        tma_load_2d(dst, (r & 1) ? &tmWol : &tmWoh, full, (r >> 1) * BK, 0);
       } else {
-        tma_load_2d(dst, k == 3 ? &tmW2l : &tmW2h, full, c * Cfg::CHUNK, 0);
+        const int c = it.c0 + ((r - PRE) >> 2), k = (r - PRE) & 3;
+        if (k < 2) {
+          for (int kk = 0; kk < 2; ++kk) {
+            tma_load_2d(dst + kk * 8192, &tmW1h, full, (2 * k + kk) * BK, c * Cfg::CHUNK);
+            tma_load_2d(dst + 16384 + kk * 8192, &tmW1l, full, (2 * k + kk) * BK, c * Cfg::CHUNK);
+          }
+        } else {
+          tma_load_2d(dst, k == 3 ? &tmW2l : &tmW2h, full, c * Cfg::CHUNK, 0);
+        }
       }
     }
     __syncwarp();
   };
-  auto load_x = [&](int j) {
+  auto load_x = [&](int v) {
     if (elect_one()) {
+      const int j = v / (4 * XG), kb = v & 3;
+      const bool att = p.prefix && (v >> 2) == j * XG;
       const int m0 = item(j).mt * BM;
-      const uint32_t full = smem_u32(bar_xfull);
-      mbar_expect_tx(full, Cfg::X_BYTES);
-      for (int kb = 0; kb < 4; ++kb) {
-        tma_load_2d(smem_u32(smem + kb * 16384), &tmXh, full, kb * BK, m0);
-        tma_load_2d(smem_u32(smem + 65536 + kb * 16384), &tmXl, full, kb * BK, m0);
-      }
-      if (j + 1 < nlocal) {
+      const uint32_t full = smem_u32(&bar_xfull[kb]);
+      mbar_expect_tx(full, 2 * BM * 128);
+      tma_load_2d(smem_u32(smem + kb * 16384), att ? &tmAh : &tmXh, full, kb * BK, m0);
+      tma_load_2d(smem_u32(smem + 65536 + kb * 16384), att ? &tmAl : &tmXl, full, kb * BK, m0);
+      if (att && kb == 0)
+        for (int k2 = 0; k2 < 4; ++k2) { tma_prefetch_2d(&tmXh, k2 * BK, m0); tma_prefetch_2d(&tmXl, k2 * BK, m0); }
+      if (v % (4 * XG) == 0 && j + 1 < nlocal) {
         const int m1 = item(j + 1).mt * BM;
-        for (int k2 = 0; k2 < 4; ++k2) { tma_prefetch_2d(&tmXh, k2 * BK, m1); tma_prefetch_2d(&tmXl, k2 * BK, m1); }
+        for (int k2 = 0; k2 < 4; ++k2) {
+          tma_prefetch_2d(&tmXh, k2 * BK, m1); tma_prefetch_2d(&tmXl, k2 * BK, m1);
+          if (p.prefix) { tma_prefetch_2d(&tmAh, k2 * BK, m1); tma_prefetch_2d(&tmAl, k2 * BK, m1); }
+        }
       }
     }
     __syncwarp();
   };
-  auto produce = [&](int need) {
+  auto produce = [&](int need, int need_x) {
+    ring_produce(x_next, xtotal, need_x, bar_xempty, 4, load_x);
     ring_produce(q_next, total, need, bar_empty, STAGES, load_slot);
-    if (x_next < nlocal && __shfl_sync(0xffffffffu, (int)mbar_test(smem_u32(bar_xempty), ((uint32_t)x_next & 1u) ^ 1u), 0))
-      load_x(x_next++);
-  };
-  auto produce_x = [&](int j) {
-    while (x_next <= j) {
-      mbar_wait(smem_u32(bar_xempty), ((uint32_t)x_next & 1u) ^ 1u);
-      load_x(x_next++);
-    }
   };
 
   const int cw = warp >> 2;
   const int cp = 2 * (lane & 3);
+  const int rl = cw * 64 + (warp & 3) * 16 + (lane >> 2);
   const uint32_t sX = smem_u32(smem) + cw * (64 * 128);
   float acc2[128];
   float acc1[32];
@@ -446,17 +497,48 @@
   int rc = 0;
   auto slot_full = [&](int r) { mbar_wait(smem_u32(&bar_full[r % STAGES]), ((uint32_t)(r / STAGES)) & 1u); };
   auto slot_free = [&](int r) { if (lane == 0) mbar_arrive(smem_u32(&bar_empty[r % STAGES])); };
+  auto x_full = [&](int kb, uint32_t par) { mbar_wait(smem_u32(&bar_xfull[kb]), par); };
+  auto x_free = [&](int kb) { if (lane == 0) mbar_arrive(smem_u32(&bar_xempty[kb])); };
   for (int j = 0; j < nlocal; ++j) {
     const Item it = item(j);
     const int m0 = it.mt * BM;
-    if (warp == 0) produce_x(j);
-    mbar_wait(smem_u32(bar_xfull), (uint32_t)j & 1u);
+    const uint32_t xpar = (uint32_t)(j * XG) & 1u;
+    if (warp == 0) produce(-1, 4 * j * XG + 3);
+    if (p.prefix) {
+#pragma unroll
+      for (int kb = 0; kb < 4; ++kb) {
+        if (warp == 0) produce(rc + 1, -1);
+        x_full(kb, xpar);
+        slot_full(rc); slot_full(rc + 1);
+        const uint32_t wh = smem_u32(ring + (rc % STAGES) * Cfg::STAGE_BYTES);
+        const uint32_t wl = smem_u32(ring + ((rc + 1) % STAGES) * Cfg::STAGE_BYTES);
+        wg_fence();
+        kblock_ss<256>(acc2, sX + kb * 16384, sX + 65536 + kb * 16384, wh, wl, kb == 0);
+        wg_commit();
+        wg_wait<0>();
+        slot_free(rc); slot_free(rc + 1); x_free(kb);
+        rc += 2;
+        if (warp == 0) produce(-1, -1);
+        tl_event(p.tl, tl_n, 60, kb);
+      }
+      acc_fence(acc2);
+      if (warp == 0) produce(-1, 4 * j * XG + 7);
+#pragma unroll
+      for (int kb = 0; kb < 4; ++kb) x_full(kb, xpar ^ 1u);
+      ln_tile(acc2, p.inv_s0, p.b0, p.gamma1, p.beta1, smem, rl, lane, cp);
+      fence_async_smem();
+      named_bar_sync(2 + cw, 128);
+      tl_event(p.tl, tl_n, 61, j);
+    } else {
+#pragma unroll
+      for (int kb = 0; kb < 4; ++kb) x_full(kb, xpar);
+    }
     tl_event(p.tl, tl_n, 2, j);
     int pend = -1;
     for (int c = it.c0; c < it.c1; ++c) {
 #pragma unroll
       for (int half = 0; half < 2; ++half) {
-        if (warp == 0) produce(rc + half);
+        if (warp == 0) produce(rc + half, -1);
         slot_full(rc + half);
         tl_event(p.tl, tl_n, 10 + half, c);
         const uint32_t w = smem_u32(ring + ((rc + half) % STAGES) * Cfg::STAGE_BYTES);
@@ -474,8 +556,9 @@
       if (pend >= 0) slot_free(pend);
       slot_free(rc); slot_free(rc + 1);
       rc += 2;
-      if (c == it.c1 - 1 && lane == 0) mbar_arrive(smem_u32(bar_xempty));
-      if (warp == 0) produce(-1);
+      if (c == it.c1 - 1 && it.mode == 1)
+        for (int kb = 0; kb < 4; ++kb) x_free(kb);
+      if (warp == 0) produce(-1, -1);
 #pragma unroll
       for (int ks = 0; ks < 4; ++ks) {
 #pragma unroll
@@ -489,7 +572,7 @@
         }
       }
       tl_event(p.tl, tl_n, 14, c);
-      if (warp == 0) produce(rc);
+      if (warp == 0) produce(rc, -1);
       slot_full(rc);
       tl_event(p.tl, tl_n, 12, c);
       wg_fence();
@@ -502,7 +585,7 @@
         }
       }
       wg_commit();
-      if (warp == 0) produce(rc + 1);
+      if (warp == 0) produce(rc + 1, -1);
       slot_full(rc + 1);
       {
         const uint64_t wd = make_desc(smem_u32(ring + ((rc + 1) % STAGES) * Cfg::STAGE_BYTES));
@@ -514,14 +597,13 @@
       slot_free(rc);
       pend = rc + 1;
       rc += 2;
-      if (warp == 0) produce(-1);
+      if (warp == 0) produce(-1, -1);
     }
     wg_wait<0>();
     acc_fence(acc2);
     if (pend >= 0) slot_free(pend);
-    if (warp == 0) produce(-1);
+    if (warp == 0) produce(-1, -1);
     tl_event(p.tl, tl_n, 4, j);
-    const int rl = cw * 64 + (warp & 3) * 16 + (lane >> 2);
     if (it.mode == 1) {
       float* const dst = p.scratch + (size_t)it.piece0 * (BM * 256);
 #pragma unroll
@@ -561,9 +643,28 @@
       if (threadIdx.x == 0)
         for (int pp = 0; pp < nparts; ++pp) p.flags[it.piece0 + pp] = 0;
     }
-    ln_epilogue(acc2, p.inv_s2, p.b2, p.res_hi, p.res_lo, p.ld_res, p.gamma, p.beta, p.out_hi, p.out_lo, p.ld_out,
-                m0 + rl, p.M, cp);
-    tl_event(p.tl, tl_n, 5, j);
+    ln_tile(acc2, p.inv_s2, p.b2, p.gamma, p.beta, smem, rl, lane, cp);
+    fence_async_smem();
+    named_bar_sync(2 + cw, 128);
+    tl_event(p.tl, tl_n, 62, j);
+    if ((warp & 3) == 0) {
+      if (elect_one()) {
+        if (m0 + cw * 64 < p.M) {
+#pragma unroll
+          for (int kb = 0; kb < 4; ++kb) {
+            const uint32_t src = smem_u32(smem + kb * 16384 + cw * 8192);
+            tma_store_2d(&tmYh, src, kb * BK, m0 + cw * 64);
+            tma_store_2d(&tmYl, src + 65536, kb * BK, m0 + cw * 64);
+          }
+          bulk_commit();
+          bulk_wait_read<0>();
+        }
+#pragma unroll
+        for (int kb = 0; kb < 4; ++kb) mbar_arrive_cnt(smem_u32(&bar_xempty[kb]), 4);
+      }
+      __syncwarp();
+      tl_event(p.tl, tl_n, 63, j);
+    }
   }
   tl_event(p.tl, tl_n, 42);
 }
@@ -894,6 +995,8 @@
   c->ffn_fused = on;
   return old;
 }
+static bool planes_aligned16(const ActBuf& b) { return ((uintptr_t)b.hi & 15) == 0 && ((uintptr_t)b.lo() & 15) == 0; }
+
 bool tc_ffn_supported(const TcCtx* c, const GemmArgs& g1, const GemmArgs& g2, const LnArgs& l2) {
   if (!c || !c->ffn_fused) return false;
   if (!tc_gemm_supported(c, g1) || !tc_gemm_ln_supported(c, g2, l2)) return false;
@@ -901,24 +1004,43 @@
   if (g1.w.N % FfnCfg::CHUNK || g1.w.N > MAX_N || g1.w.N != g2.K1) return false;
   if (g1.act != ACT_GELU || g1.out_f32 || g1.addtab || g1.zero_lengths) return false;
   if (g1.in_group < g1.M || g1.out_group != 0 || g1.out_off != 0) return false;
+  if (l2.res.hi != g1.a1.hi || l2.res.plane_stride != g1.a1.plane_stride) return false;
+  if (!planes_aligned16(g1.a1) || !planes_aligned16(l2.out)) return false;
   return true;
 }
-bool tc_ffn(TcCtx* c, const GemmArgs& g1, const GemmArgs& g2, const LnArgs& l2, float* scratch, int* flags, cudaStream_t st) {
-  CUtensorMap mXh, mXl, mW1h, mW1l, mW2h, mW2l;
-  const int m_tiles = (g1.M + BM - 1) / BM;
-  const bool ok = make_map(&mXh, g1.a1.hi, g1.M, g1.K1, BM) && make_map(&mXl, g1.a1.lo(), g1.M, g1.K1, BM) &&
-                  make_map(&mW1h, g1.w.w, g1.w.N, g1.w.K, FfnCfg::CHUNK) &&
-                  make_map(&mW1l, g1.w.w + g1.w.plane_stride, g1.w.N, g1.w.K, FfnCfg::CHUNK) &&
-                  make_map(&mW2h, g2.w.w, g2.w.N, g2.w.K, 256) &&
-                  make_map(&mW2l, g2.w.w + g2.w.plane_stride, g2.w.N, g2.w.K, 256);
+bool tc_tail_supported(const TcCtx* c, const GemmArgs& go, const LnArgs& l1, const GemmArgs& g1, const GemmArgs& g2,
+                       const LnArgs& l2) {
+  if (!tc_gemm_ln_supported(c, go, l1) || !tc_ffn_supported(c, g1, g2, l2)) return false;
+  if (go.K1 != 256 || go.K2 > 0 || go.M != g1.M || !l1.res.hi) return false;
+  if (g1.a1.hi != l1.out.hi || g1.a1.plane_stride != l1.out.plane_stride) return false;
+  return planes_aligned16(go.a1) && planes_aligned16(l1.res);
+}
+
+static bool launch_ffn(TcCtx* c, const GemmArgs* go, const LnArgs* l1, const GemmArgs& g1, const GemmArgs& g2,
+                       const LnArgs& l2, float* scratch, int* flags, cudaStream_t st) {
+  CUtensorMap mXh, mXl, mW1h, mW1l, mW2h, mW2l, mAh, mAl, mWoh, mWol, mYh, mYl;
+  const int M = g1.M, m_tiles = (M + BM - 1) / BM;
+  const ActBuf x = go ? l1->res : g1.a1;
+  bool ok = make_map(&mXh, x.hi, M, 256, BM) && make_map(&mXl, x.lo(), M, 256, BM) &&
+            make_map(&mW1h, g1.w.w, g1.w.N, g1.w.K, FfnCfg::CHUNK) &&
+            make_map(&mW1l, g1.w.w + g1.w.plane_stride, g1.w.N, g1.w.K, FfnCfg::CHUNK) &&
+            make_map(&mW2h, g2.w.w, g2.w.N, g2.w.K, 256) &&
+            make_map(&mW2l, g2.w.w + g2.w.plane_stride, g2.w.N, g2.w.K, 256) &&
+            make_map(&mYh, l2.out.hi, M, 256, 64) && make_map(&mYl, l2.out.lo(), M, 256, 64);
+  if (go) {
+    ok = ok && make_map(&mAh, go->a1.hi, M, 256, BM) && make_map(&mAl, go->a1.lo(), M, 256, BM) &&
+         make_map(&mWoh, go->w.w, go->w.N, go->w.K, 256) && make_map(&mWol, go->w.w + go->w.plane_stride, go->w.N, go->w.K, 256);
+  } else {
+    mAh = mXh; mAl = mXl; mWoh = mW2h; mWol = mW2l;
+  }
   if (!ok) return false;
   FfnParams p{};
-  p.M = g1.M; p.m_tiles = m_tiles; p.n_chunks = g1.w.N / FfnCfg::CHUNK;
+  p.M = M; p.m_tiles = m_tiles; p.n_chunks = g1.w.N / FfnCfg::CHUNK;
   p.tl = tc::mldb_timeline_buffer();
+  p.prefix = go ? 1 : 0;
+  if (go) { p.inv_s0 = go->w.inv_scale; p.b0 = go->w.bias; p.gamma1 = l1->gamma; p.beta1 = l1->beta; }
   p.inv_s1 = g1.w.inv_scale; p.inv_s2 = g2.w.inv_scale;
   p.b1 = g1.w.bias; p.b2 = g2.w.bias; p.gamma = l2.gamma; p.beta = l2.beta;
-  p.res_hi = l2.res.hi; p.res_lo = l2.res.hi ? l2.res.lo() : nullptr; p.ld_res = l2.res.cols;
-  p.out_hi = l2.out.hi; p.out_lo = l2.out.lo(); p.ld_out = l2.out.cols;
   const int ncta_max = c->sm_count;
   p.full = m_tiles / ncta_max; p.left = m_tiles % ncta_max; p.parts = 1;
   p.scratch = scratch; p.flags = flags;
@@ -928,6 +1050,14 @@
   }
   const int ncta = p.full > 0 ? ncta_max : p.left * p.parts;
   p.reverse = tc::snake_order();
-  launch_pdl(k_ffn_tc, dim3(ncta), dim3(MMA_THREADS), FfnCfg::SMEM_BYTES, st, mXh, mXl, mW1h, mW1l, mW2h, mW2l, p);
+  launch_pdl(k_ffn_tc, dim3(ncta), dim3(MMA_THREADS), FfnCfg::SMEM_BYTES, st, mXh, mXl, mW1h, mW1l, mW2h, mW2l, mAh,
+             mAl, mWoh, mWol, mYh, mYl, p);
   return true;
 }
+bool tc_ffn(TcCtx* c, const GemmArgs& g1, const GemmArgs& g2, const LnArgs& l2, float* scratch, int* flags, cudaStream_t st) {
+  return launch_ffn(c, nullptr, nullptr, g1, g2, l2, scratch, flags, st);
+}
+bool tc_tail(TcCtx* c, const GemmArgs& go, const LnArgs& l1, const GemmArgs& g1, const GemmArgs& g2, const LnArgs& l2,
+             float* scratch, int* flags, cudaStream_t st) {
+  return launch_ffn(c, &go, &l1, g1, g2, l2, scratch, flags, st);
+}
diff --git a/mld_b200/csrc/gemm_tc.h b/mld_b200/csrc/gemm_tc.h
--- a/mld_b200/csrc/gemm_tc.h
+++ b/mld_b200/csrc/gemm_tc.h
@@ -10,5 +10,9 @@
 bool tc_ffn_supported(const TcCtx* c, const GemmArgs& g1, const GemmArgs& g2, const LnArgs& l2);
 constexpr size_t TC_FFN_SCRATCH_BYTES = (size_t)160 * 128 * 256 * 4, TC_FFN_FLAG_BYTES = 160 * 4;
 bool tc_ffn(TcCtx* c, const GemmArgs& g1, const GemmArgs& g2, const LnArgs& l2, float* scratch, int* flags, cudaStream_t st);
+bool tc_tail_supported(const TcCtx* c, const GemmArgs& go, const LnArgs& l1, const GemmArgs& g1, const GemmArgs& g2,
+                       const LnArgs& l2);
+bool tc_tail(TcCtx* c, const GemmArgs& go, const LnArgs& l1, const GemmArgs& g1, const GemmArgs& g2, const LnArgs& l2,
+             float* scratch, int* flags, cudaStream_t st);
 int tc_set_ffn_split(TcCtx* c, int on);
 int tc_set_ffn_fused(TcCtx* c, int on);
diff --git a/mld_b200/csrc/tc_common.cuh b/mld_b200/csrc/tc_common.cuh
--- a/mld_b200/csrc/tc_common.cuh
+++ b/mld_b200/csrc/tc_common.cuh
@@ -21,6 +21,9 @@
 }
 __device__ __forceinline__ void mbar_arrive(uint32_t bar) {
   asm volatile("mbarrier.arrive.shared::cta.b64 _, [%0];" ::"r"(bar) : "memory");
+}
+__device__ __forceinline__ void mbar_arrive_cnt(uint32_t bar, uint32_t n) {
+  asm volatile("mbarrier.arrive.shared::cta.b64 _, [%0], %1;" ::"r"(bar), "r"(n) : "memory");
 }
 __device__ __forceinline__ void mbar_wait(uint32_t bar, uint32_t parity) {
   uint32_t done = 0, spins = 0;
@@ -71,6 +74,15 @@
 __device__ __forceinline__ void tma_prefetch_desc(const CUtensorMap* map) {
   asm volatile("prefetch.tensormap [%0];" ::"l"(reinterpret_cast<uint64_t>(map)) : "memory");
 }
+__device__ __forceinline__ void tma_store_2d(const CUtensorMap* map, uint32_t src, int c0, int c1) {
+  asm volatile("cp.async.bulk.tensor.2d.global.shared::cta.bulk_group [%0, {%2, %3}], [%1];"
+               ::"l"(reinterpret_cast<uint64_t>(map)), "r"(src), "r"(c0), "r"(c1) : "memory");
+}
+__device__ __forceinline__ void bulk_commit() { asm volatile("cp.async.bulk.commit_group;" ::: "memory"); }
+template <int N> __device__ __forceinline__ void bulk_wait_read() {
+  asm volatile("cp.async.bulk.wait_group.read %0;" ::"n"(N) : "memory");
+}
+__device__ __forceinline__ void fence_async_smem() { asm volatile("fence.proxy.async.shared::cta;" ::: "memory"); }
 
 __device__ __forceinline__ bool elect_one() {
   uint32_t pred;
diff --git a/mld_b200/engine.py b/mld_b200/engine.py
--- a/mld_b200/engine.py
+++ b/mld_b200/engine.py
@@ -100,6 +100,19 @@
         out = torch.empty((M, d), dtype=torch.float32, device=self.device)
         check(self.lib.mldb_debug_ffn(self._h, _ptr(X), *[_ptr(t) for t in host], M, d, ff, int(mode), _ptr(out),
                                       self._stream()), "mldb_debug_ffn")
+        return out
+
+    def debug_tail(self, att, X, Wo, bo, g1, be1, W1, b1, W2, b2, g2, be2, mode=2, pad=None):
+        att, X = _f32c(att, self.device), _f32c(X, self.device)
+        host = [None if t is None else t.detach().float().contiguous().cpu()
+                for t in (Wo, bo, g1, be1, W1, b1, W2, b2, g2, be2)]
+        M, d = X.shape
+        ff = host[4].shape[0]
+        out = torch.empty((M, d), dtype=torch.float32, device=self.device)
+        if pad is not None:
+            out = torch.cat([out, _f32c(pad, self.device)]).contiguous()
+        check(self.lib.mldb_debug_tail(self._h, _ptr(att), _ptr(X), *[_ptr(t) for t in host], M, d, ff, int(mode),
+                                       out.shape[0], _ptr(out), self._stream()), "mldb_debug_tail")
         return out
 
     def debug_attention(self, q, nseq, Lq, heads, lengths=None, mode=2, kv=None, Lk=None, kv_prefix=0,
```

New measurement: 850.7, median of 6. 1.05x the previous value.
